# tencent-ailab/PCDMs

Measured on AMD Instinct MI355X. Metric: images/sec (50-step DDIM, 352x512 stage2), higher is better.
Workload: dtype bf16; 1 GPU; stage2 inpaint, 352x512 (canvas 704x512, latent 64x88), batch=4 per GPU, 50 DDIM steps, guidance 2.0 (UNet batch 8), 868.9M-param UNet, 258 context tokens, bf16 MFMA / fp32 accumulate; global_batch=4, parallelism=dp1, hipgraph=True, rccl_world_size=1, attention=bf16

## Files before the change

### include/pcdm.h

```cpp
#ifndef PCDM_H
#define PCDM_H
#include <stdint.h>
#ifdef __cplusplus
extern "C" {
#endif

typedef void* pcdm_stream_t;

#define PCDM_ABI_VERSION 5
int pcdm_version(void);
int pcdm_is_emulator(void);

int64_t pcdm_groupnorm_ws_floats(int B, int C);
int pcdm_groupnorm_cluster_timeouts(const float* ws, unsigned* count_out, pcdm_stream_t s);
int pcdm_groupnorm(const void* x1, int C1, const void* x2, int C2, int B, int HW, int groups, float eps,
                   const float* gamma, const float* beta, int fuse_silu, void* y, float* ws, pcdm_stream_t s);

typedef struct pcdm_gn_splitk_src {
    const float* part;
    int32_t split_k, M, N, Npad;
    const float* bias;
    const float* rowvec;
    int64_t ldrv;
    const int32_t* rowvec_step;
    int64_t rowvec_step_stride;
    const void* residual;
    int64_t ldr;
    void* pre_out;
    int32_t store_pre;
    int32_t rowvec_step_count;
    int32_t* step_error;
} pcdm_gn_splitk_src;
int pcdm_groupnorm_splitk(const pcdm_gn_splitk_src* src, const void* x2, int C2, int B, int HW, int groups, float eps,
                          const float* gamma, const float* beta, int fuse_silu, void* y, float* ws, pcdm_stream_t s);

int pcdm_layernorm(const void* x, void* y, int rows, int C, float eps, const float* gamma, const float* beta,
                   pcdm_stream_t s);

enum { PCDM_EPI_STORE = 0, PCDM_EPI_GEGLU = 1, PCDM_EPI_SPLIT_VT = 2, PCDM_EPI_NCHW_F32 = 3 };
enum { PCDM_ACT_NONE = 0, PCDM_ACT_SILU = 1, PCDM_ACT_GELU = 2 };
typedef struct pcdm_gemm_params {
    uint32_t struct_size;
    const void* a;
    const void* a2;
    int64_t lda, lda2;
    int32_t c1;
    int32_t conv;
    int32_t B, Hi, Wi, Ho, Wo, stride, upsample, cin;
    const void* w;
    int32_t M, N, K, Npad;
    const float* bias;
    const float* rowvec;
    int64_t ldrv;
    int32_t rows_per_batch;
    const void* residual;
    int64_t ldr;
    int32_t res_mod;
    int32_t epilogue;
    int32_t vt_col0;
    void* out;
    int64_t ldo;
    void* out2;
    int64_t ldo2;
    int32_t split_k;
    float* ws;
    int64_t ws_floats;
    int64_t ldw;
    int32_t no_pad_lo;
    int32_t tile;
    int32_t act;
    int32_t zero_rows;
    const float* ln_wsum;
    float ln_eps;
    int32_t defer_reduce;
    const int32_t* rowvec_step;
    int64_t rowvec_step_stride;
    int32_t dup_rows;
    const float* ln_row_stats;
    float* row_stats_out;
    int32_t rowvec_step_count;
    int32_t* step_error;
    const void* a3;
    int64_t lda3;
    uint64_t tap_lut;
    int32_t tap_group_n;
} pcdm_gemm_params;
int pcdm_gemm(const pcdm_gemm_params* p, pcdm_stream_t s);

int pcdm_flash_attn(const void* q, int64_t ldq, const void* k, int64_t ldk, const void* vt, int64_t ldvt,
                    void* o, int64_t ldo, int B, int H, int Lq, int Lk, float scale, pcdm_stream_t s);
#define PCDM_ATTN_DEFAULT_THR 8.0f
int pcdm_flash_attn_thr(const void* q, int64_t ldq, const void* k, int64_t ldk, const void* vt, int64_t ldvt,
                        void* o, int64_t ldo, int B, int H, int Lq, int Lk, float scale, float thr_log2, pcdm_stream_t s);

int pcdm_quantize_fp8(const void* x, void* y, int64_t rows, int cols, int cols_pad, int64_t ldx, int64_t ldy, float scale, pcdm_stream_t s);
int pcdm_flash_attn_fp8(const void* q, int64_t ldq, const void* k8, int64_t ldk, const void* vt8, int64_t ldvt, void* o, int64_t ldo,
                        int B, int H, int Lq, int Lk, float scale, float k_descale, float v_descale, float thr_log2, pcdm_stream_t s);

int pcdm_attn_wide(const void* q, int64_t ldq, const void* k, int64_t ldk, const void* vt, int64_t ldvt, void* o, int64_t ldo,
                   int B, int Lq, int Lk, int d, float scale, pcdm_stream_t s);

int pcdm_timestep_embedding(const int64_t* t_dev, const int32_t* step_dev, float* out, int B, int dim,
                            int flip_sin_to_cos, float shift, pcdm_stream_t s);
int pcdm_small_linear(const float* x, const void* w, const float* bias, const float* add, float* y, int B, int K,
                      int N, int act_in, int act_out, pcdm_stream_t s);
int pcdm_timestep_embedding_rows(const int64_t* t_dev, int n, float* out, int dim, int flip_sin_to_cos, float shift, pcdm_stream_t s);
int pcdm_time_class_combine(const float* emb_t, const float* cls, void* out_bf16, int n, int B, int D, pcdm_stream_t s);

int pcdm_assemble_input(const float* latents, int N, int rep, const float* mask, int mask_b, const float* masked,
                        int masked_b, void* out, int h, int w, int cpad, pcdm_stream_t s);
int pcdm_nchw_f32_to_nhwc_bf16(const float* x, void* y, int B, int C, int Cpad, int HW, pcdm_stream_t s);
int pcdm_nhwc_bf16_to_nchw_f32(const void* x, float* y, int B, int C, int HW, pcdm_stream_t s);
int pcdm_f32_to_bf16(const float* x, void* y, int64_t n, pcdm_stream_t s);

int pcdm_cfg_step(const float* eps, int cfg, float g, const float* x, const float* noise, float* x_prev,
                  float* eps_out, const float* coef, const int32_t* step_dev, int64_t n, pcdm_stream_t s);
int pcdm_unipc_step(const float* eps, int cfg, float g, float* x, float* m1, float* m2, float* last, const float* coef,
                    const int32_t* step_dev, int64_t n, pcdm_stream_t s);
int pcdm_dpmpp_step(const float* eps, int cfg, float g, float* x, float* m1, const float* noise_all, const float* coef,
                    const int32_t* step_dev, int64_t n, pcdm_stream_t s);
int pcdm_unclip_step(const float* pred, int cfg, float g, const float* x, const float* noise, float* x_prev,
                     const float* c8, int64_t n, pcdm_stream_t s);
int pcdm_unclip_step_dev(const float* pred, int cfg, float g, float* x, const float* noise_all, const float* coef,
                         const int32_t* step_dev, int64_t n, pcdm_stream_t s);
int pcdm_rescale_noise_cfg(const float* cfg_eps, const float* text_eps, float* out, int N, int64_t n,
                           float guidance_rescale, pcdm_stream_t s);
int pcdm_softmax_rows(const float* s_in, void* p_out, int rows, int cols, int64_t ld_s, int64_t ld_p, float scale,
                      pcdm_stream_t s);
int pcdm_gaussian_sample(const float* moments, const float* noise, float* out, int B, int zc, int HW, float scale,
                         pcdm_stream_t s);
int pcdm_image_to_uint8(const float* x, void* out, int B, int cstride, int HW, pcdm_stream_t s);
int pcdm_lincomb(float* y, int nin, const float* const* xs, const float* c, int64_t n, pcdm_stream_t s);
int pcdm_advance_step(int32_t* step_dev, pcdm_stream_t s);
int pcdm_pixel_shuffle2(const void* in, void* out, int B, int H, int W, int C, pcdm_stream_t s);

int64_t pcdm_metrics_ws_bytes(int N, int ref_n, int W, int H, float sigma);
int pcdm_ssim(const void* cand, int N, int Hc, int Wc, const int32_t* cand_win, const void* ref, int ref_n, int Hr, int Wr, const int32_t* ref_win,
              int channels, int is_f32, float sigma, float data_range, float* scores, int32_t* argmax, void* ws, int64_t ws_bytes, pcdm_stream_t s);
int pcdm_psnr(const void* cand, int N, int Hc, int Wc, const int32_t* cand_win, const void* ref, int ref_n, int Hr, int Wr, const int32_t* ref_win,
              int channels, int is_f32, float data_range, float* mse, float* psnr, void* ws, int64_t ws_bytes, pcdm_stream_t s);
int pcdm_select_image(const void* cand_u8, int N, int Hc, int Wc, const int32_t* win, int channels, const int32_t* index_dev, void* out, int normalized,
                      pcdm_stream_t s);

typedef struct pcdm_lpips_weights {
    const float* conv_w[5];
    const float* conv_b[5];
    const float* lin[5];
} pcdm_lpips_weights;
int pcdm_pack_lpips_conv(const float* w, const float* bias, int Cout, int Cin, int kh, int kw, float* out_w, float* out_bias, int* K_out, int* cin_out);
int pcdm_conv2d_f32(const float* x, int B, int Hi, int Wi, int Cin, const float* w_packed, const float* bias, int Cout, int kh, int kw, int stride, int pad,
                    int relu, float* out, pcdm_stream_t s);
int pcdm_maxpool3s2_f32(const float* x, int B, int Hi, int Wi, int C, float* out, pcdm_stream_t s);
int64_t pcdm_lpips_ws_bytes(int N, int ref_n, int H, int W);
int pcdm_lpips(const void* img0, int N, int H0, int W0, const int32_t* win0, const void* img1, int ref_n, int H1, int W1, const int32_t* win1, int is_f32,
               int normalize, const pcdm_lpips_weights* wts, float* out, float* layers, int32_t* argmin, void* ws, int64_t ws_bytes, pcdm_stream_t s);

typedef struct pcdm_inception_weights {
    const float* w[94];
    const float* bias[94];
} pcdm_inception_weights;
int pcdm_conv2d_f32_ex(const float* x, int B, int Hi, int Wi, int Cin, const float* w_packed, const float* bias, int Cout, int kh, int kw, int stride,
                       int pad_h, int pad_w, int relu, float* out, int out_pitch, int out_offset, pcdm_stream_t s);
int pcdm_maxpool3s2_f32_ex(const float* x, int B, int Hi, int Wi, int C, float* out, int out_pitch, int out_offset, pcdm_stream_t s);
int pcdm_avgpool3_f32(const float* x, int B, int H, int W, int C, float* out, pcdm_stream_t s);
int pcdm_global_avgpool_f32(const float* x, int B, int P, int C, float* out, pcdm_stream_t s);
int pcdm_inception_input(const void* img, int N, int Hi, int Wi, const int32_t* win, int is_f32, int resize, int normalize, float* out, pcdm_stream_t s);
int64_t pcdm_inception_ws_bytes(int B, int H, int W, int dims);
int pcdm_inception_features(const void* img, int N, int Hi, int Wi, const int32_t* win, int is_f32, int resize, int normalize, int dims,
                            const pcdm_inception_weights* wts, float* out, void* ws, int64_t ws_bytes, pcdm_stream_t s);
int pcdm_fid_accumulate(const float* feat, int B, int D, double* sum, double* gram, pcdm_stream_t s);
int pcdm_fid_finalize(const double* sum, const double* gram, int64_t n, int D, double* mu, double* sigma, pcdm_stream_t s);

int64_t pcdm_resample_ws_bytes(int Hs, int Ws, int Hd, int Wd, int channels, int ky);
int pcdm_resample_u8(const void* src, int Hs, int Ws, int channels, const int32_t* xtab, int kx, const int32_t* ytab, int ky, void* dst, int Hd, int Wd,
                     int64_t dst_pitch, int x0, int y0, void* ws, int64_t ws_bytes, pcdm_stream_t s);
int pcdm_u8_to_nchw(const void* src_u8, int Hs, int Ws, int channels, const int32_t* win, int mode, double scale, const float* mean, const float* std_,
                    float* out, pcdm_stream_t s);

int pcdm_resize_cubic_f32(const void* src, int src_is_f32, int Hs, int Ws, int channels, float* dst, int N, int Hd, int Wd, int index, int nchw,
                          float divisor, pcdm_stream_t s);
int pcdm_absdiff(const void* cand, int N, int Hc, int Wc, const int32_t* cand_win, const void* ref, int ref_n, int Hr, int Wr, const int32_t* ref_win,
                 int channels, int is_f32, float* l1, float* mae, void* ws, int64_t ws_bytes, pcdm_stream_t s);
int64_t pcdm_ssim_box_ws_bytes(int N, int ref_n, int W, int H, int win_size);
int pcdm_ssim_box(const void* cand, int N, int Hc, int Wc, const int32_t* cand_win, const void* ref, int ref_n, int Hr, int Wr, const int32_t* ref_win,
                  int channels, int is_f32, int win_size, float data_range, float* scores, void* ws, int64_t ws_bytes, pcdm_stream_t s);

int pcdm_pose_tables(int32_t* tables, int count);
int64_t pcdm_pose_ws_bytes(int M, int P);
int pcdm_pose_draw(const float* keypoints, const float* scores, int M, int P, int Hd, int Wd, int hands, int faces, const int32_t* tables, void* out,
                   void* ws, int64_t ws_bytes, pcdm_stream_t s);
int pcdm_resize_linear_u8(const void* src, int M, int Hs, int Ws, void* dst, int Hd, int Wd, pcdm_stream_t s);

typedef struct pcdm_unet pcdm_unet;
typedef struct pcdm_unet_config {
    int32_t out_channels;
    int32_t n_levels;
    int32_t block_out_channels[8];
    int32_t heads[8];
    int32_t cross_attn[8];
    int32_t layers_per_block;
    int32_t cross_attention_dim;
    int32_t norm_groups;
    float norm_eps;
    int32_t class_embed;
    int32_t flip_sin_to_cos;
    float freq_shift;
} pcdm_unet_config;
pcdm_unet* pcdm_unet_create(const pcdm_unet_config* cfg);
void pcdm_unet_destroy(pcdm_unet* u);
const char* pcdm_unet_last_error(const pcdm_unet* u);
int pcdm_unet_set_weight(pcdm_unet* u, const char* name, const void* w_bf16, const float* bias, const float* wsum, int N, int K, int Npad, int cin);
int pcdm_unet_set_vector(pcdm_unet* u, const char* name, const float* v, int n);
int pcdm_unet_set_tile(pcdm_unet* u, int ln, int M, int Npad, int K, int conv, int stride, int upsample, int epilogue, int two_source, int residual,
                       int zero_rows, int tile, int split_k);
int pcdm_unet_set_attention_fp8(pcdm_unet* u, int on);
int pcdm_unet_get_tile(const pcdm_unet* u, int ln, int M, int Npad, int K, int conv, int stride, int upsample, int epilogue, int two_source, int residual,
// ... 20 lines not shown
```

### pcdms_amd/_lib.py

```python
from __future__ import annotations

import ctypes as C
import os
from pathlib import Path
from typing import Optional

import torch

_HERE = Path(__file__).resolve().parent
LIB_PATH = Path(os.environ.get("PCDM_LIB") or _HERE / "lib" / "libpcdm.so")

_lib: Optional[C.CDLL] = None
_is_emu = False


class GemmParams(C.Structure):

    _fields_ = [
        ("struct_size", C.c_uint32),
        ("a", C.c_void_p), ("a2", C.c_void_p), ("lda", C.c_int64), ("lda2", C.c_int64),
        ("c1", C.c_int32), ("conv", C.c_int32),
        ("B", C.c_int32), ("Hi", C.c_int32), ("Wi", C.c_int32), ("Ho", C.c_int32), ("Wo", C.c_int32),
        ("stride", C.c_int32), ("upsample", C.c_int32), ("cin", C.c_int32),
        ("w", C.c_void_p),
        ("M", C.c_int32), ("N", C.c_int32), ("K", C.c_int32), ("Npad", C.c_int32),
        ("bias", C.c_void_p), ("rowvec", C.c_void_p), ("ldrv", C.c_int64), ("rows_per_batch", C.c_int32),
        ("residual", C.c_void_p), ("ldr", C.c_int64), ("res_mod", C.c_int32),
        ("epilogue", C.c_int32), ("vt_col0", C.c_int32),
        ("out", C.c_void_p), ("ldo", C.c_int64), ("out2", C.c_void_p), ("ldo2", C.c_int64),
        ("split_k", C.c_int32), ("ws", C.c_void_p), ("ws_floats", C.c_int64),
        ("ldw", C.c_int64), ("no_pad_lo", C.c_int32), ("tile", C.c_int32), ("act", C.c_int32),
        ("zero_rows", C.c_int32),
        ("ln_wsum", C.c_void_p), ("ln_eps", C.c_float), ("defer_reduce", C.c_int32),
        ("rowvec_step", C.c_void_p), ("rowvec_step_stride", C.c_int64), ("dup_rows", C.c_int32),
        ("ln_row_stats", C.c_void_p), ("row_stats_out", C.c_void_p), ("rowvec_step_count", C.c_int32), ("step_error", C.c_void_p),
        ("a3", C.c_void_p), ("lda3", C.c_int64), ("tap_lut", C.c_uint64), ("tap_group_n", C.c_int32),
    ]

    def __init__(self, *args, **kw):
        super().__init__(*args, **kw)
        self.struct_size = C.sizeof(GemmParams)


class GnSplitKSrc(C.Structure):

    _fields_ = [("part", C.c_void_p), ("split_k", C.c_int32), ("M", C.c_int32), ("N", C.c_int32), ("Npad", C.c_int32),
                ("bias", C.c_void_p), ("rowvec", C.c_void_p), ("ldrv", C.c_int64), ("rowvec_step", C.c_void_p), ("rowvec_step_stride", C.c_int64),
                ("residual", C.c_void_p), ("ldr", C.c_int64), ("pre_out", C.c_void_p), ("store_pre", C.c_int32),
                ("rowvec_step_count", C.c_int32), ("step_error", C.c_void_p)]


class UNetConfig(C.Structure):

    _fields_ = [("out_channels", C.c_int32), ("n_levels", C.c_int32), ("block_out_channels", C.c_int32 * 8), ("heads", C.c_int32 * 8),
                ("cross_attn", C.c_int32 * 8), ("layers_per_block", C.c_int32), ("cross_attention_dim", C.c_int32),
                ("norm_groups", C.c_int32), ("norm_eps", C.c_float), ("class_embed", C.c_int32), ("flip_sin_to_cos", C.c_int32),
                ("freq_shift", C.c_float)]


class LpipsWeights(C.Structure):

    _fields_ = [("conv_w", C.c_void_p * 5), ("conv_b", C.c_void_p * 5), ("lin", C.c_void_p * 5)]


class InceptionWeights(C.Structure):

    _fields_ = [("w", C.c_void_p * 94), ("bias", C.c_void_p * 94)]


_P, _I, _L, _F = C.c_void_p, C.c_int, C.c_int64, C.c_float
_W4 = C.POINTER(C.c_int32)
_SIGS = {
    "pcdm_version": ([], C.c_int),
    "pcdm_is_emulator": ([], C.c_int),
    "pcdm_groupnorm_ws_floats": ([_I, _I], _L),
    "pcdm_groupnorm_cluster_timeouts": ([_P, C.POINTER(C.c_uint), _P], C.c_int),
    "pcdm_groupnorm": ([_P, _I, _P, _I, _I, _I, _I, _F, _P, _P, _I, _P, _P, _P], C.c_int),
    "pcdm_groupnorm_splitk": ([C.POINTER(GnSplitKSrc), _P, _I, _I, _I, _I, _F, _P, _P, _I, _P, _P, _P], C.c_int),
    "pcdm_layernorm": ([_P, _P, _I, _I, _F, _P, _P, _P], C.c_int),
    "pcdm_gemm": ([C.POINTER(GemmParams), _P], C.c_int),
    "pcdm_flash_attn": ([_P, _L, _P, _L, _P, _L, _P, _L, _I, _I, _I, _I, _F, _P], C.c_int),
    "pcdm_flash_attn_thr": ([_P, _L, _P, _L, _P, _L, _P, _L, _I, _I, _I, _I, _F, _F, _P], C.c_int),
    "pcdm_quantize_fp8": ([_P, _P, _L, _I, _I, _L, _L, _F, _P], C.c_int),
    "pcdm_flash_attn_fp8": ([_P, _L, _P, _L, _P, _L, _P, _L, _I, _I, _I, _I, _F, _F, _F, _F, _P], C.c_int),
    "pcdm_attn_wide": ([_P, _L, _P, _L, _P, _L, _P, _L, _I, _I, _I, _I, _F, _P], C.c_int),
    "pcdm_timestep_embedding": ([_P, _P, _P, _I, _I, _I, _F, _P], C.c_int),
    "pcdm_timestep_embedding_rows": ([_P, _I, _P, _I, _I, _F, _P], C.c_int),
    "pcdm_time_class_combine": ([_P, _P, _P, _I, _I, _I, _P], C.c_int),
    "pcdm_small_linear": ([_P, _P, _P, _P, _P, _I, _I, _I, _I, _I, _P], C.c_int),
    "pcdm_assemble_input": ([_P, _I, _I, _P, _I, _P, _I, _P, _I, _I, _I, _P], C.c_int),
    "pcdm_nchw_f32_to_nhwc_bf16": ([_P, _P, _I, _I, _I, _I, _P], C.c_int),
    "pcdm_nhwc_bf16_to_nchw_f32": ([_P, _P, _I, _I, _I, _P], C.c_int),
    "pcdm_f32_to_bf16": ([_P, _P, _L, _P], C.c_int),
    "pcdm_cfg_step": ([_P, _I, _F, _P, _P, _P, _P, _P, _P, _L, _P], C.c_int),
    "pcdm_unipc_step": ([_P, _I, _F, _P, _P, _P, _P, _P, _P, _L, _P], C.c_int),
    "pcdm_dpmpp_step": ([_P, _I, _F, _P, _P, _P, _P, _P, _L, _P], C.c_int),
    "pcdm_unclip_step": ([_P, _I, _F, _P, _P, _P, C.POINTER(_F), _L, _P], C.c_int),
    "pcdm_unclip_step_dev": ([_P, _I, _F, _P, _P, _P, _P, _L, _P], C.c_int),
    "pcdm_lincomb": ([_P, _I, C.POINTER(_P), C.POINTER(_F), _L, _P], C.c_int),
    "pcdm_rescale_noise_cfg": ([_P, _P, _P, _I, _L, _F, _P], C.c_int),
    "pcdm_softmax_rows": ([_P, _P, _I, _I, _L, _L, _F, _P], C.c_int),
    "pcdm_gaussian_sample": ([_P, _P, _P, _I, _I, _I, _F, _P], C.c_int),
    "pcdm_image_to_uint8": ([_P, _P, _I, _I, _I, _P], C.c_int),
    "pcdm_advance_step": ([_P, _P], C.c_int),
    "pcdm_pixel_shuffle2": ([_P, _P, _I, _I, _I, _I, _P], C.c_int),
    "pcdm_metrics_ws_bytes": ([_I, _I, _I, _I, _F], _L),
    "pcdm_ssim": ([_P, _I, _I, _I, _W4, _P, _I, _I, _I, _W4, _I, _I, _F, _F, _P, _P, _P, _L, _P], C.c_int),
    "pcdm_psnr": ([_P, _I, _I, _I, _W4, _P, _I, _I, _I, _W4, _I, _I, _F, _P, _P, _P, _L, _P], C.c_int),
    "pcdm_select_image": ([_P, _I, _I, _I, _W4, _I, _P, _P, _I, _P], C.c_int),
    "pcdm_pack_lpips_conv": ([_P, _P, _I, _I, _I, _I, _P, _P, _P, _P], C.c_int),
    "pcdm_conv2d_f32": ([_P, _I, _I, _I, _I, _P, _P, _I, _I, _I, _I, _I, _I, _P, _P], C.c_int),
    "pcdm_maxpool3s2_f32": ([_P, _I, _I, _I, _I, _P, _P], C.c_int),
    "pcdm_lpips_ws_bytes": ([_I, _I, _I, _I], _L),
    "pcdm_lpips": ([_P, _I, _I, _I, _W4, _P, _I, _I, _I, _W4, _I, _I, C.POINTER(LpipsWeights), _P, _P, _P, _P, _L, _P], C.c_int),
    "pcdm_conv2d_f32_ex": ([_P, _I, _I, _I, _I, _P, _P, _I, _I, _I, _I, _I, _I, _I, _P, _I, _I, _P], C.c_int),
    "pcdm_maxpool3s2_f32_ex": ([_P, _I, _I, _I, _I, _P, _I, _I, _P], C.c_int),
    "pcdm_avgpool3_f32": ([_P, _I, _I, _I, _I, _P, _P], C.c_int),
    "pcdm_global_avgpool_f32": ([_P, _I, _I, _I, _P, _P], C.c_int),
    "pcdm_inception_input": ([_P, _I, _I, _I, _W4, _I, _I, _I, _P, _P], C.c_int),
    "pcdm_inception_ws_bytes": ([_I, _I, _I, _I], _L),
    "pcdm_inception_features": ([_P, _I, _I, _I, _W4, _I, _I, _I, _I, C.POINTER(InceptionWeights), _P, _P, _L, _P], C.c_int),
    "pcdm_fid_accumulate": ([_P, _I, _I, _P, _P, _P], C.c_int),
    "pcdm_fid_finalize": ([_P, _P, _L, _I, _P, _P, _P], C.c_int),
    "pcdm_resample_ws_bytes": ([_I, _I, _I, _I, _I, _I], _L),
    "pcdm_resample_u8": ([_P, _I, _I, _I, _P, _I, _P, _I, _P, _I, _I, _L, _I, _I, _P, _L, _P], C.c_int),
    "pcdm_u8_to_nchw": ([_P, _I, _I, _I, _W4, _I, C.c_double, C.POINTER(_F), C.POINTER(_F), _P, _P], C.c_int),
    "pcdm_resize_cubic_f32": ([_P, _I, _I, _I, _I, _P, _I, _I, _I, _I, _I, _F, _P], C.c_int),
    "pcdm_absdiff": ([_P, _I, _I, _I, _W4, _P, _I, _I, _I, _W4, _I, _I, _P, _P, _P, _L, _P], C.c_int),
    "pcdm_ssim_box_ws_bytes": ([_I, _I, _I, _I, _I], _L),
    "pcdm_ssim_box": ([_P, _I, _I, _I, _W4, _P, _I, _I, _I, _W4, _I, _I, _I, _F, _P, _P, _L, _P], C.c_int),
    "pcdm_pose_tables": ([C.POINTER(C.c_int32), _I], C.c_int),
    "pcdm_pose_ws_bytes": ([_I, _I], _L),
    "pcdm_pose_draw": ([_P, _P, _I, _I, _I, _I, _I, _I, _P, _P, _P, _L, _P], C.c_int),
    "pcdm_resize_linear_u8": ([_P, _I, _I, _I, _P, _I, _I, _P], C.c_int),
    "pcdm_unet_create":([C.POINTER(UNetConfig)], _P),
    "pcdm_unet_destroy": ([_P], None),
    "pcdm_unet_last_error": ([_P], C.c_char_p),
    "pcdm_unet_set_weight": ([_P, C.c_char_p, _P, _P, _P, _I, _I, _I, _I], C.c_int),
    "pcdm_unet_set_vector": ([_P, C.c_char_p, _P, _I], C.c_int),
    "pcdm_unet_set_tile": ([_P] + [_I] * 13, C.c_int),
    "pcdm_unet_set_attention_fp8": ([_P, _I], C.c_int),
    "pcdm_unet_get_tile": ([_P] + [_I] * 11 + [C.POINTER(C.c_int), C.POINTER(C.c_int)], C.c_int),
    "pcdm_unet_workspace_bytes": ([_P, _I, _I, _I, _I], _L),
    "pcdm_unet_workspace_init": ([_P, _I, _I, _I, _I, _P, _P], C.c_int),
    "pcdm_unet_prepare_conditioning": ([_P, _I, _I, _I, _I, _P, _P, _P, _I, _I, _P, _P], C.c_int),
    "pcdm_unet_time_table_bytes": ([_P, _I, _I], _L),
    "pcdm_unet_prepare_timesteps": ([_P, _P, _I, _P, _P, _P], C.c_int),
    "pcdm_unet_set_shared_cfg_input": ([_P, _P, _I], C.c_int),
    "pcdm_unet_forward": ([_P, _P, _P, _P, _I, _I, _I, _I, _I, _P, _P, _P], C.c_int),
    "pcdm_unet_step_overflow": ([_P, _P, C.POINTER(C.c_int), _P], C.c_int),
    "pcdm_pack_linear": ([_P, _P, _I, _I, _I, _P, _P], C.c_int),
    "pcdm_pack_conv3x3": ([_P, _P, _I, _I, _I, _P, _P, _P, _P], C.c_int),
    "pcdm_pack_geglu": ([_P, _P, _I, _I, _P, _P], C.c_int),
}
EXPORTS = tuple(_SIGS)


def _bind(lib: C.CDLL) -> C.CDLL:
    for name, (args, res) in _SIGS.items():
        fn = getattr(lib, name)
        fn.argtypes = args
        fn.restype = res
    return lib


def use_library(lib: C.CDLL) -> None:
    global _lib, _is_emu
    _lib = _bind(lib)
    _is_emu = bool(lib.pcdm_is_emulator())


def load(path: Optional[Path] = None) -> C.CDLL:
    global _lib, _is_emu
    p = Path(path) if path else LIB_PATH
    if not p.exists():
        raise RuntimeError(
            f"{p} not found: the HIP kernel library is not built.  Run `python -m pcdms_amd.build` "
            "(needs hipcc); pcdms_amd has no fallback implementation.")
    _lib = _bind(C.CDLL(str(p)))
    _is_emu = bool(_lib.pcdm_is_emulator())
    return _lib


def lib() -> C.CDLL:
    return _lib if _lib is not None else load()


# ... 4 lines not shown
```

### pcdms_amd/csrc/gemm.hip

```cpp
#include "gemm_kernel.inc"

namespace {
template <bool CONV>
int dispatch_tile(int tile, const GemmArgs& a, hipStream_t st) {
    switch (tile) {
#ifndef PCDM_DEV_NEW_TILES_ONLY
        case 1: return launch_gemm<256, 128, 4, 2, 3, CONV>(a, st);
        case 2: return launch_gemm<64, 64, 2, 2, 2, CONV>(a, st);
        case 3: return launch_gemm<256, 64, 4, 2, 2, CONV>(a, st);
        case 4: return launch_gemm<128, 128, 2, 2, 2, CONV>(a, st);
        case 5: return launch_gemm<128, 64, 2, 2, 2, CONV>(a, st);
        case 6: return launch_gemm<256, 64, 4, 2, 3, CONV>(a, st);
        case 7: return launch_gemm<128, 128, 2, 2, 3, CONV>(a, st);
        case 8: return launch_gemm<64, 64, 2, 2, 4, CONV>(a, st);
        case 9: return launch_gemm<256, 128, 4, 2, 2, CONV>(a, st);
        case 10: return launch_gemm<128, 64, 2, 2, 3, CONV>(a, st);
        case 11: return launch_gemm<256, 128, 4, 2, 3, CONV, true>(a, st);
        case 12: return launch_gemm<256, 64, 4, 2, 3, CONV, true>(a, st);
        case 13: return launch_gemm<256, 64, 4, 1, 2, CONV>(a, st);
        case 14: return launch_gemm<256, 64, 4, 1, 3, CONV>(a, st);
        case 15: return launch_gemm<128, 64, 2, 1, 2, CONV>(a, st);
        case 16: return launch_gemm<512, 64, 8, 1, 2, CONV>(a, st);
        case 17: return launch_gemm<256, 256, 2, 4, 2, CONV>(a, st);
        case 18: return launch_gemm<128, 128, 4, 2, 2, CONV>(a, st);
#endif
        case 21: return launch_gemm<192, 320, 2, 4, 2, CONV, false, 16>(a, st);
        case 22: return launch_gemm<176, 320, 2, 4, 2, CONV, false, 16>(a, st);
        case 23: return launch_gemm<176, 256, 2, 4, 2, CONV, false, 16>(a, st);
        case 26: return launch_gemm<192, 256, 2, 4, 2, CONV, false, 16>(a, st);
#ifdef PCDM_DEV_KB32
        case 27: return launch_gemm<192, 320, 2, 4, 4, CONV, false, 16, 32>(a, st);
        case 28: return launch_gemm<256, 256, 2, 4, 4, CONV, false, 16, 32>(a, st);
#endif
        default: return -1;
    }
}
}

extern "C" int pcdm_gemm(const pcdm_gemm_params* p, pcdm_stream_t s) {
    if (!p || p->struct_size != (uint32_t)sizeof(pcdm_gemm_params)) return -1;
    if (!p->a || !p->w || !p->out) return -1;
    if (p->M <= 0 || p->N <= 0 || p->K <= 0 || p->K % BK || p->Npad % 64 || p->Npad < p->N || p->N % 4) return -1;
    if (p->rows_per_batch <= 0) return -1;
    if (((uintptr_t)p->bias & 15) || (p->rowvec && (((uintptr_t)p->rowvec & 15) || (p->ldrv > 0 && p->ldrv % 4) || (p->rowvec_step && p->rowvec_step_stride % 4))))
        return -1;
    const int64_t lim = 0x7fffffffLL;
    if ((int64_t)p->Npad * (p->ldw > 0 ? p->ldw : p->K) * 2 >= lim) return -2;
    if (p->conv ? ((int64_t)p->B * p->Hi * p->Wi * p->cin * 2 + ((int64_t)p->Wi + 1) * p->cin * 2 >= lim ||
                   (p->a2 && (int64_t)p->M * p->lda2 * 2 >= lim) || (p->a3 && (int64_t)p->M * p->lda3 * 2 >= lim))
                : ((int64_t)p->M * p->lda * 2 >= lim || (p->a2 && (int64_t)p->M * p->lda2 * 2 >= lim))) return -2;
    const int64_t out_esz = p->epilogue == PCDM_EPI_NCHW_F32 ? 4 : 2;
    if ((int64_t)p->M * (p->ldo > 0 ? p->ldo : p->N) * out_esz >= lim || (p->residual && (int64_t)p->M * (p->ldr > 0 ? p->ldr : p->N) * 2 >= lim))
        return -2;
    GemmArgs a;
    a.a = (const u16*)p->a;
    a.a2 = (const u16*)p->a2;
    a.lda = p->lda;
    a.lda2 = p->lda2;
    a.c1 = p->a2 ? p->c1 : p->K;
    a.a3 = (const u16*)p->a3;
    a.lda3 = p->lda3;
    a.xinv = 0;
    a.tap_lut = 0;
    a.tap_group_n = 0;
    a.B = p->B; a.Hi = p->Hi; a.Wi = p->Wi; a.Ho = p->Ho; a.Wo = p->Wo;
    a.stride = p->stride; a.upsample = p->upsample; a.cin = p->cin;
    a.pad = p->no_pad_lo ? 0 : 1;
    a.w = (const u16*)p->w;
    a.ldw = p->ldw > 0 ? p->ldw : p->K;
    if (a.ldw < p->K || a.ldw % 8) return -1;
    a.M = p->M; a.N = p->N; a.K = p->K; a.Npad = p->Npad;
    a.bias = p->bias;
    a.rowvec = p->rowvec;
    a.rowvec_step = p->rowvec ? p->rowvec_step : nullptr;
    a.rowvec_step_stride = p->rowvec_step_stride;
    a.rowvec_step_count = a.rowvec_step ? p->rowvec_step_count : 0;
    a.step_error = a.rowvec_step ? p->step_error : nullptr;
    if (a.rowvec_step_count < 0 || ((uintptr_t)a.step_error & 3)) return -1;
    a.ldrv = p->ldrv > 0 ? (int)p->ldrv : p->N;
    a.rows_per_batch = p->rows_per_batch;
    a.residual = (const u16*)p->residual;
    a.ldr = p->ldr;
    a.res_mod = p->res_mod > 0 ? p->res_mod : p->M;
    a.epilogue = p->epilogue;
    a.vt_col0 = p->vt_col0;
    a.out = p->out;
    a.ldo = p->ldo;
    a.out2 = (u16*)p->out2;
    a.ldo2 = p->ldo2;
    a.tiles_m = a.tiles_n = 0;
    a.debug = p->tile >> 8;
    a.act = p->act;
    a.dup_rows = p->dup_rows;
    if (a.dup_rows) {
        if (a.dup_rows < 0 || !p->conv || p->epilogue != PCDM_EPI_STORE || p->act || p->split_k > 1 || (p->N & 7) || (p->ldo & 7)) return -1;
        if (p->residual && ((p->ldr & 7) || (p->res_mod > 0 && p->res_mod < p->M))) return -1;
        if (p->rowvec && (p->rows_per_batch < 32 || a.dup_rows % p->rows_per_batch)) return -1;
        if (((int64_t)p->M + a.dup_rows) * (p->ldo > 0 ? p->ldo : p->N) * 2 >= lim) return -2;
    }
    a.zero_rows = p->zero_rows;
    if (a.zero_rows < 0 || a.zero_rows > p->M || (a.zero_rows && p->conv)) return -1;
    if (a.act < 0 || a.act > PCDM_ACT_GELU || (a.act == PCDM_ACT_GELU && p->epilogue == PCDM_EPI_GEGLU)) return -1;
    a.ln_wsum = p->ln_wsum;
    a.ln_eps = p->ln_eps;
    a.split_k = p->split_k > 1 ? p->split_k : 1;
    a.defer_reduce = (p->defer_reduce && a.split_k > 1) ? 1 : 0;
    if (a.defer_reduce && (p->act || p->res_mod > 0 && p->res_mod < p->M)) return -1;
    a.ws = p->ws;
    if (a.split_k > 1) {
        if (p->epilogue != PCDM_EPI_STORE || !p->ws || a.split_k > p->K / BK || a.split_k > 64) return -1;
        if (p->ws_floats < (int64_t)a.split_k * p->M * p->Npad) return -1;
    }
    if (p->conv && p->tap_group_n > 0) {
        const int ntaps = p->cin > 0 ? p->K / p->cin : 0;
        if (p->cin <= 0 || p->cin % BK || p->K != ntaps * p->cin || ntaps < 1 || ntaps > 4 || p->stride != 1 || p->upsample || p->no_pad_lo || p->dup_rows ||
            p->a2 || p->a3 || p->Hi != p->Ho || p->Wi != p->Wo || p->N % p->tap_group_n || p->N / p->tap_group_n > 4 || p->tap_group_n % 64)
            return -1;
        uint64_t lut = 0;
        for (int g = 0; g < p->N / p->tap_group_n; ++g) {
            uint64_t grp = (p->tap_lut >> (16 * g)) & ((1ull << (4 * ntaps)) - 1);
            for (int t = 0; t < ntaps; ++t)
                if (((grp >> (4 * t)) & 15) > 8) return -1;
            if (grp == 0) {
                if (ntaps == 4) return -1;
                grp = 1ull << (4 * ntaps);
            }
            lut |= grp << (16 * g);
        }
        if (p->M != p->B * p->Ho * p->Wo) return -1;
        a.tap_lut = lut;
        a.tap_group_n = p->tap_group_n;
    } else if (p->conv) {
        const int cx = p->K - 9 * p->cin;
        if (p->cin <= 0 || p->cin % BK || cx < 0 || (p->stride != 1 && p->stride != 2)) return -1;
        if (cx == 0 ? (p->a2 || p->a3)
                    : (!p->a2 || p->stride != 1 || p->upsample || p->no_pad_lo || p->dup_rows || p->Hi != p->Ho || p->Wi != p->Wo || cx % BK ||
                       p->c1 <= 0 || p->c1 % BK || p->c1 > cx || (p->c1 < cx) != (p->a3 != nullptr) || p->lda2 < p->c1 || (p->lda2 & 7) ||
                       (p->a3 && (p->lda3 < cx - p->c1 || (p->lda3 & 7))) || (((uintptr_t)p->a2 | (uintptr_t)p->a3) & 15)))
            return -1;
        a.xinv = (uint32_t)(((1ull << 31) + (uint64_t)(p->cin / 64) - 1) / (uint64_t)(p->cin / 64));
        if (p->upsample && (p->stride != 1 || p->no_pad_lo || p->Ho < p->Hi || p->Wo < p->Wi)) return -1;
        if (p->M != p->B * p->Ho * p->Wo) return -1;
    } else {
        if (p->a3 || (p->a2 && (p->c1 % BK || p->c1 <= 0 || p->c1 >= p->K))) return -1;
    }
    if (p->epilogue == PCDM_EPI_GEGLU && (!p->bias || p->Npad % 128 || p->N * 2 > p->Npad)) return -1;
    if (p->epilogue == PCDM_EPI_SPLIT_VT && (!p->out2 || p->vt_col0 % 4)) return -1;
    hipStream_t st = (hipStream_t)s;
    int tile = p->tile & 0xff;
    if (tile >= pcdm_gemm_detail::kRowGemmTile0) {
        if ((a.debug & 4) && p->ws_floats < (int64_t)((p->M + 95) / 96) * 8 * 8 * 2) return -1;
        if (p->row_stats_out) return -1;
        return p->conv ? -1 : pcdm_gemm_detail::launch_rowgemm(tile, a, st);
    }
    a.ln_row_stats = p->ln_row_stats;
    a.row_stats_out = p->row_stats_out;
    if (a.ln_wsum) {
        if (p->conv || p->a2 || a.split_k > 1 || p->rowvec || p->residual || p->act || a.zero_rows || a.dup_rows || (p->N & 7) || (p->ldo & 7) ||
            ((uintptr_t)a.ln_wsum & 15) || p->row_stats_out)
            return -1;
        if (p->epilogue != PCDM_EPI_STORE && p->epilogue != PCDM_EPI_GEGLU && p->epilogue != PCDM_EPI_SPLIT_VT) return -1;
        if (p->epilogue == PCDM_EPI_SPLIT_VT && (p->vt_col0 % 64 || p->rows_per_batch % 32 || (p->ldo2 & 7) || p->M % 32)) return -1;
        if (p->epilogue == PCDM_EPI_GEGLU && (tile == 2 || tile == 8)) return -1;
        if (((tile == 4 || tile == 7 || tile == 18) && p->Npad % 128) || ((tile == 17 || tile == 26 || tile == 23) && p->Npad % 256)) return -1;
        if (a.ln_row_stats && ((p->K & 63) || p->K > 1280 || ((uintptr_t)a.ln_row_stats & 15))) return -1;
        return pcdm_gemm_detail::launch_gemm_ext(a.ln_row_stats ? 2 : 1, tile, a, st);
    }
    if (a.ln_row_stats) return -1;
    if (a.row_stats_out) {
        if (p->conv || a.split_k > 1 || p->act || a.dup_rows || p->epilogue != PCDM_EPI_STORE || (p->N & 31) || (p->ldo & 7) || ((uintptr_t)a.row_stats_out & 7) ||
            (p->residual && ((p->ldr & 7) || (p->res_mod > 0 && p->res_mod < p->M))) || (p->rowvec && p->rows_per_batch < 32))
            return -1;
        if ((tile == 4 || tile == 7 || tile == 18) && p->Npad % 128) return -1;
        return pcdm_gemm_detail::launch_gemm_ext(3, tile, a, st);
    }
    const bool n128 = p->Npad % 128 == 0 && (a.tap_group_n == 0 || a.tap_group_n % 128 == 0);
    const bool needs128 = tile == 1 || tile == 4 || tile == 7 || tile == 9 || tile == 11 || tile == 18;
    if (p->epilogue == PCDM_EPI_GEGLU && tile != 0 && !needs128 && tile < 13) return -1;
    if (tile == 0) {
        const int64_t t256 = (int64_t)((p->M + 255) / 256) * (p->Npad / 128);
        const int64_t t128 = (int64_t)((p->M + 127) / 128) * (p->Npad / 128);
        if (n128 && t256 >= 200) tile = 1;
        else if (n128 && (t128 >= 160 || p->epilogue == PCDM_EPI_GEGLU)) tile = 4;
        else if (!n128 && (int64_t)((p->M + 127) / 128) * (p->Npad / 64) >= 256) tile = 5;
        else tile = 2;
    } else if ((needs128 && !n128) || (tile == 17 && p->Npad % 256)) {
        return -1;
    }
    return p->conv ? dispatch_tile<true>(tile, a, st) : dispatch_tile<false>(tile, a, st);
}
```

### pcdms_amd/csrc/gemm_args.h

```cpp
#pragma once
#include "pcdm_device.h"
#include "../../include/pcdm.h"

namespace pcdm_gemm_detail {
struct GemmArgs {
    const u16* a;
    const u16* a2;
    int64_t lda, lda2;
    int c1;
    const u16* a3;
    int64_t lda3;
    uint64_t tap_lut;
    int tap_group_n;
    uint32_t xinv;
    int B, Hi, Wi, Ho, Wo, stride, upsample, cin;
    int pad;
    const u16* w;
    int64_t ldw;
    int M, N, K, Npad;
    const float* bias;
    const float* rowvec;
    const int32_t* rowvec_step;
    int64_t rowvec_step_stride;
    int rowvec_step_count;
    int32_t* step_error;
    int ldrv;
    int rows_per_batch;
    const u16* residual;
    int64_t ldr;
    int res_mod;
    int epilogue;
    int vt_col0;
    void* out;
    int64_t ldo;
    u16* out2;
    int64_t ldo2;
    int tiles_m, tiles_n;
    int split_k;
    float* ws;
    int act;
    int zero_rows;
    const float* ln_wsum;
    float ln_eps;
    const float* ln_row_stats;
    float* row_stats_out;
    int dup_rows;
    int defer_reduce;
    int debug;
};
}

namespace pcdm_gemm_detail {
__device__ __forceinline__ int bounded_step(const int32_t* step, int count, int32_t* err) {
    int st = *step;
    if (count > 0 && (st < 0 || st >= count)) {
        if (err) *err = 1;
        st = st < 0 ? 0 : count - 1;
    }
    return st;
}
__device__ __forceinline__ const float* rowvec_base(const GemmArgs& p) {
    return (p.rowvec && p.rowvec_step) ? p.rowvec + (int64_t)bounded_step(p.rowvec_step, p.rowvec_step_count, p.step_error) * p.rowvec_step_stride : p.rowvec;
}
__device__ __forceinline__ float apply_act(float v, int act) {
    return act == PCDM_ACT_SILU ? silu_f(v) : act == PCDM_ACT_GELU ? gelu_erf_f(v) : v;
}
__device__ __forceinline__ float gate_act(float g, int act) { return act == PCDM_ACT_SILU ? silu_f(g) : gelu_erf_f(g); }

constexpr int kRowGemmTile0 = 31;
int launch_rowgemm(int tile, const GemmArgs& a, hipStream_t st);
int launch_gemm_ext(int ext, int tile, const GemmArgs& a, hipStream_t st);
}
```

### pcdms_amd/csrc/gemm_kernel.inc

```
#include "gemm_args.h"

#include <type_traits>



namespace {
using pcdm_gemm_detail::GemmArgs;
using pcdm_gemm_detail::apply_act;
using pcdm_gemm_detail::gate_act;
constexpr int BK = 64;

__device__ __attribute__((aligned(32))) const unsigned int g_zero32[8] = {0, 0, 0, 0, 0, 0, 0, 0};

template <int WCOLS>
struct PassGeom {
    static constexpr int LPR = WCOLS / 8;
    static constexpr int RPI = 64 / LPR;
    static constexpr int NIT = (32 + RPI - 1) / RPI;
    static constexpr bool TAIL = NIT * RPI > 32;
};

template <int WCOLS>
__device__ __forceinline__ void lean_res_load(const GemmArgs& p, int lane, int mrow0, int ncol0, BufRsrc rs_r, u32x4 (&rv)[4]) {
    typedef PassGeom<WCOLS> G;
    constexpr uint32_t kOOB = 0x80000000u;
    const int rl = lane / G::LPR, c8 = (lane - rl * G::LPR) * 8;
    const int n = ncol0 + c8;
    const bool lane_ok = rl < G::RPI && n < p.N;
    const uint32_t vr0 = lane_ok ? (uint32_t)(((mrow0 + rl) * (int)p.ldr + n) * 2) : kOOB;
    const uint32_t sr = (uint32_t)(G::RPI * (int)p.ldr * 2);
#pragma unroll
    for (int it = 0; it < G::NIT; ++it) rv[it] = buf_load16_once(rs_r, (G::TAIL && it * G::RPI + rl >= 32) ? kOOB : vr0 + it * sr);
}

template <int WCOLS, int EPW, int RV, bool STATS = false>
__device__ __forceinline__ void lean_pass(const GemmArgs& p, float* ep, int lane, int mrow0, int ncol0, f32x4 b0, f32x4 b1,
                                          BufRsrc rs_o, BufRsrc rs_v, const u32x4 (&rv)[4], const float* rvec_w, int rv_pitch,
                                          int rv_col0, int rv_split_row) {
    static_assert(!STATS || WCOLS == 32 || WCOLS == 64, "row statistics: passes of 32 or 64 columns");
    typedef PassGeom<WCOLS> G;
    constexpr int LPR = G::LPR, RPI = G::RPI, NIT = G::NIT;
    constexpr bool TAIL = G::TAIL;
    constexpr uint32_t kOOB = 0x80000000u;
    const int rl = lane / LPR, c8 = (lane - rl * LPR) * 8;
    const int n = ncol0 + c8;
    const bool lane_ok = rl < RPI && n < p.N;
    const uint32_t vo0 = lane_ok ? (uint32_t)(((mrow0 + rl) * (int)p.ldo + n) * 2) : kOOB;
    const uint32_t so = (uint32_t)(RPI * (int)p.ldo * 2);
    f32x4 t0[2], t1[2];
    if constexpr (RV == 1) {
#pragma unroll
        for (int h = 0; h < 2; ++h) {
            t0[h] = *(const f32x4*)(rvec_w + h * rv_pitch + rv_col0 + c8);
            t1[h] = *(const f32x4*)(rvec_w + h * rv_pitch + rv_col0 + c8 + 4);
        }
    }
#pragma unroll
    for (int it = 0; it < NIT; ++it) {
        const int r = it * RPI + rl;
        const int rr = (TAIL && r >= 32) ? 0 : r;
        const f32x4 v0 = *(const f32x4*)(ep + rr * EPW + c8), v1 = *(const f32x4*)(ep + rr * EPW + c8 + 4);
        f32x4 a0 = v0 + b0, a1 = v1 + b1;
        if constexpr (RV == 1) {
            const bool hi = mrow0 + r >= rv_split_row;
            a0 += hi ? t0[1] : t0[0];
            a1 += hi ? t1[1] : t1[0];
        }
        if constexpr (RV == 2) {
            const int mb = mrow0 + it * RPI;
            const int b_lo = mb / p.rows_per_batch;
            const int bidx = b_lo + ((mb + rl) >= (b_lo + 1) * p.rows_per_batch ? 1 : 0);
            const uint32_t vv = lane_ok ? (uint32_t)((bidx * p.ldrv + n) * 4) : kOOB;
            a0 += __builtin_bit_cast(f32x4, buf_load16(rs_v, vv));
            a1 += __builtin_bit_cast(f32x4, buf_load16(rs_v, vv + 16));
        }
#pragma unroll
        for (int e = 0; e < 4; ++e) {
            a0[e] += __builtin_bit_cast(float, rv[it][e >> 1] << (e & 1 ? 0 : 16) & 0xffff0000u);
            a1[e] += __builtin_bit_cast(float, rv[it][2 + (e >> 1)] << (e & 1 ? 0 : 16) & 0xffff0000u);
        }
        u32x4 o;
        o[0] = pack2bf(a0[0], a0[1]);
        o[1] = pack2bf(a0[2], a0[3]);
        o[2] = pack2bf(a1[0], a1[1]);
        o[3] = pack2bf(a1[2], a1[3]);
        buf_store16(rs_o, (TAIL && r >= 32) ? kOOB : vo0 + it * so, o);
        if constexpr (STATS) {
            float v[8];
#pragma unroll
            for (int e = 0; e < 4; ++e) {
                v[2 * e] = __builtin_bit_cast(float, o[e] << 16);
                v[2 * e + 1] = __builtin_bit_cast(float, o[e] & 0xffff0000u);
            }
            float sv = ((v[0] + v[1]) + (v[2] + v[3])) + ((v[4] + v[5]) + (v[6] + v[7]));
            sv += __shfl_xor(sv, 1, 64);
            sv += __shfl_xor(sv, 2, 64);
            const float mu = sv * (1.0f / 32.0f);
            float qv = 0.f;
#pragma unroll
            for (int e = 0; e < 8; ++e) {
                const float d = v[e] - mu;
                qv += d * d;
            }
            qv += __shfl_xor(qv, 1, 64);
            qv += __shfl_xor(qv, 2, 64);
            const int m = mrow0 + r;
            if (((lane & 3) == 0) && lane_ok && m < p.M) {
                const f32x2 sq = {sv, qv};
                *((f32x2*)p.row_stats_out + (int64_t)m * (p.N >> 5) + (n >> 5)) = sq;
            }
        }
    }
}

template <int WCOLS, int EPW>
__device__ __forceinline__ void vt_pass(const GemmArgs& p, const float* ep, int lane, int mrow0, int ncol0, BufRsrc rs_vt,
                                        const float* bias_c ) {
    constexpr uint32_t kOOB = 0x80000000u;
    const int b = mrow0 / p.rows_per_batch, tok0 = mrow0 - b * p.rows_per_batch;
    const int cl = lane & 15, tg = lane >> 4;
    const int cv = p.N - p.vt_col0;
#pragma unroll
    for (int ii = 0; ii < WCOLS / 16; ++ii) {
        const int c = ii * 16 + cl, n = ncol0 + c;
        const bool ok = n < p.N;
        const float bias = bias_c[c];
        float v[8];
#pragma unroll
        for (int i = 0; i < 8; ++i) v[i] = ep[(8 * tg + i) * EPW + c] + bias;
        u32x4 o;
#pragma unroll
        for (int i = 0; i < 4; ++i) o[i] = pack2bf(v[2 * i], v[2 * i + 1]);
        const uint32_t vo = ok ? (uint32_t)((((int64_t)b * cv + (n - p.vt_col0)) * p.ldo2 + tok0 + 8 * tg) * 2) : kOOB;
        buf_store16(rs_vt, vo, o);
    }
}

template <int N>
__device__ __forceinline__ void wait_vm_then_barrier() {
#ifdef PCDM_EMU
    __syncthreads();
#else
    asm volatile("s_waitcnt vmcnt(%0)\n\ts_barrier" ::"n"(N) : "memory");
#endif
}

template <int N>
__device__ __forceinline__ void wait_vm_lds_then_barrier() {
#ifdef PCDM_EMU
    __syncthreads();
#else
    __builtin_amdgcn_sched_barrier(0);
    __builtin_amdgcn_s_waitcnt((N & 15) | (7 << 4) | (0 << 8) | ((N >> 4) << 14));
    __builtin_amdgcn_s_barrier();
    __builtin_amdgcn_sched_barrier(0);
#endif
}

__device__ __forceinline__ void wait_lds() {
#ifndef PCDM_EMU
    __builtin_amdgcn_s_waitcnt(15 | (7 << 4) | (0 << 8) | (3 << 14));
#endif
}

template <int N>
__device__ __forceinline__ void wait_vm() {
#ifndef PCDM_EMU
    asm volatile("s_waitcnt vmcnt(%0)" ::"n"(N) : "memory");
#endif
}
__device__ __forceinline__ void wait_lds_then_barrier() {
#ifdef PCDM_EMU
    __syncthreads();
#else
    asm volatile("s_waitcnt lgkmcnt(0)\n\ts_barrier" ::: "memory");
#endif
}

template <int BM, int BN, int WGM, int WGN, int STAGES, bool CONV, bool STAG = false, int F = 32, int KB = 64, int EXT = 0>
__global__ __launch_bounds__(WGM* WGN * 64) void gemm_kernel(const GemmArgs p) {
    constexpr bool LNF = EXT == 1 || EXT == 2, LNK = EXT == 1, LNP = EXT == 2, STATS = EXT == 3;
    static_assert(EXT == 0 || (!CONV && !STAG && KB == 64), "extended instances: linear tiles on the rotated schedule");
    static_assert(!STATS || F == 32, "row-statistics producer: 32- / 64-column epilogue passes");
    static_assert(!LNK || BM % (8 * WGM * WGN) == 0, "in-loop row statistics: 8 rows per wave instruction");
    constexpr int BK = KB;
    constexpr int NW = WGM * WGN;
    static_assert(BM % F == 0, "tile shape");
    constexpr int FMT = BM / F;
    constexpr int FM = (FMT + WGM - 1) / WGM;
    constexpr int FM_LAST = FMT - (WGM - 1) * FM;
    constexpr bool UNEVEN = FM_LAST != FM;
    constexpr int WM = FM * F, WN = BN / WGN, FN = WN / F;
    static_assert(FM_LAST >= 1 && (!UNEVEN || (F == 16 && !STAG && KB == 64 && (EXT == 0 || EXT == 2))), "uneven tiles: 16x16x32 fragments, rotated schedule, plain / folded-LayerNorm (partials) instances");
    constexpr int KS = 512 / F;
    constexpr int NKS = BK / KS;
    constexpr int CPK = KS / 8;
    constexpr int NQ = F == 32 ? 4 : 1;
    constexpr int LF = F == 32 ? 5 : 4;
    static_assert((F == 32 || F == 16) && (!STAG || F == 32), "fragment shape");
    static_assert(KB == 64 || (KB == 32 && F == 16 && STAGES == 4 && !STAG), "K-tile depth");
    typedef typename std::conditional<F == 32, f32x16, f32x4>::type acc_t;
    constexpr bool ROLES = KB == 32;
    constexpr int LPR = BK / 8;
    constexpr int RPI = 64 / LPR;
    constexpr int PW = ROLES ? (BM + BN) / (RPI * NW) : 0;
    constexpr int NWA = ROLES ? BM / (RPI * PW) : NW;
    constexpr int BMS = ROLES ? BM : (BM + 8 * NW - 1) / (8 * NW) * (8 * NW);
    constexpr int AI = ROLES ? PW : BMS / 8 / NW, BI = ROLES ? PW : BN / 8 / NW;
    constexpr int PWT = ROLES ? PW : AI + BI;
    constexpr int D = STAGES - 1;
    static_assert(ROLES || ((BM == BMS || UNEVEN) && BN % (8 * NW) == 0), "tile shape");
    static_assert(!ROLES || ((BM + BN) % (RPI * NW) == 0 && BM % (RPI * PW) == 0 && BN % (RPI * PW) == 0), "tile shape (roles)");
    static_assert(WM % 32 == 0 && WN % F == 0, "tile shape");
    PCDM_DYN_SMEM(smem);
    u16* As = (u16*)smem;
    u16* Bs = As + STAGES * BMS * BK;

    const int t = threadIdx.x, lane = t & 63;
    const int wave = __builtin_amdgcn_readfirstlane(t >> 6);
    const int wm = wave / WGN, wn = wave - wm * WGN;
#ifndef PCDM_EMU
    unsigned long long stamp[6] = {0, 0, 0, 0, 0, 0};
    const unsigned long long wall0 = (p.debug & 4) ? wall_clock64() : 0ull;
#define PCDM_STAMP(i) do { if (p.debug & 4) stamp[i] = __builtin_readcyclecounter(); } while (0)
#else
#define PCDM_STAMP(i) ((void)0)
#endif
    PCDM_STAMP(0);

    const int nwg = gridDim.x, bid = blockIdx.x;
    const int q8 = nwg >> 3, r8 = nwg & 7, xcd = bid & 7;
    const int wg = (xcd < r8 ? xcd * (q8 + 1) : r8 * (q8 + 1) + (xcd - r8) * q8) + (bid >> 3);
    const int ntiles = p.tiles_m * p.tiles_n;
    const int ksplit = wg / ntiles, tile_id = wg - ksplit * ntiles;
    const int tile_m = tile_id / p.tiles_n, tile_n = tile_id - tile_m * p.tiles_n;
    const int m0 = tile_m * BM, n0 = tile_n * BN;

    const int srow = lane / LPR, spos = lane % LPR;
    auto swz = [](int r) { return KB == 64 ? (r >> 1) & 7 : (0 - (r >> 2)) & 3; };
    const bool doA = !ROLES || wave < NWA, doB = !ROLES || wave >= NWA;
    const int wa = ROLES ? (wave < NWA ? wave : 0) : wave, wb = ROLES ? (wave >= NWA ? wave - NWA : 0) : wave;
    constexpr uint32_t kOOB = 0x80000000u;
    uint32_t a_off[AI], a_off2[AI];
    int a_mask[AI];
    int a_b[AI], a_y[AI], a_x[AI];
#pragma unroll
    for (int j = 0; j < AI; ++j) {
        const int rl = (wa * AI + j) * RPI + srow;
        int m = m0 + rl;
        const uint32_t ck = (uint32_t)(spos ^ swz(rl)) * 16u;
        const bool mvalid = m < p.M;
        if (!mvalid) m = p.M - 1;
        const bool ghost = BMS > BM && rl >= BM;
        a_off2[j] = 0; a_mask[j] = 0; a_b[j] = a_y[j] = a_x[j] = 0;
        if (ghost) {
            a_off[j] = a_off2[j] = kOOB;
        } else if (CONV) {
            const int hw = p.Ho * p.Wo;
            const int b = m / hw, rem = m - b * hw;
            const int y = rem / p.Wo, x = rem - y * p.Wo;
            a_b[j] = b; a_y[j] = y; a_x[j] = x;
            a_off[j] = (uint32_t)((((int64_t)b * p.Hi + y * p.stride) * p.Wi + x * p.stride) * p.cin * 2) + ck;
            const int Hv_ = p.upsample ? p.Ho : p.Hi, Wv_ = p.upsample ? p.Wo : p.Wi;
#pragma unroll
            for (int tp = 0; tp < 9; ++tp) {
                const int iy = y * p.stride + tp / 3 - p.pad, ix = x * p.stride + tp % 3 - p.pad;
                if (iy >= 0 && iy < Hv_ && ix >= 0 && ix < Wv_) a_mask[j] |= 1 << tp;
            }
        } else {
            a_off[j] = m < p.zero_rows ? kOOB : (uint32_t)((int64_t)m * p.lda * 2) + ck;
            a_off2[j] = m < p.zero_rows ? kOOB : (uint32_t)((int64_t)m * p.lda2 * 2) + ck;
        }
    }
    uint32_t b_off[BI];
#pragma unroll
    for (int j = 0; j < BI; ++j) {
// ... 323 lines not shown
                    mfma_block(B1());
                    PCDM_SCHED_BARRIER();
                }
            }
            const int left = nkt - 2 - kt;
            wait_landed(left < 0 ? 0 : (left < STAGES - 2 ? left : STAGES - 2));
            if (kt + STAGES < nkt && !(p.debug & 1)) issue_tile(kt + STAGES, cur);
            const int nx = cur + 1 == STAGES ? 0 : cur + 1;
            if (kt + 1 < nkt) load_frags(nx, 0, B0());
            PCDM_SCHED_BARRIER();
            mfma_block(B1());
            PCDM_SCHED_BARRIER();
            cur = nx;
        }
        };
        if constexpr (UNEVEN) {
            if (wm == WGM - 1) kloop(std::integral_constant<int, FM_LAST>());
            else kloop(std::integral_constant<int, FM>());
        } else {
            kloop(std::integral_constant<int, FM>());
        }
    }

    PCDM_STAMP(3);
    const int half = lane >> LF;
    const int prow = lane & (F - 1);
    constexpr int QS = F == 32 ? 8 : 0;
    const int mlim = UNEVEN ? (m0 + BM < p.M ? m0 + BM : p.M) : p.M;
    if (p.split_k > 1) {
#pragma unroll
        for (int j = 0; j < FM; ++j) {
            const int m = m0 + wm * WM + j * F + prow;
            if (m >= mlim) continue;
            float* wr = p.ws + ((int64_t)ksplit * p.M + m) * p.Npad + n0 + wn * WN + 4 * half;
#pragma unroll
            for (int i = 0; i < FN; ++i)
#pragma unroll
                for (int rg = 0; rg < NQ; ++rg) {
                    f32x4 v = {acc[i][j][4 * rg], acc[i][j][4 * rg + 1], acc[i][j][4 * rg + 2], acc[i][j][4 * rg + 3]};
                    *(f32x4*)(wr + i * F + QS * rg) = v;
                }
        }
        return;
    }
    constexpr bool GLU_OK = WN == 64;
    const bool geglu = p.epilogue == PCDM_EPI_GEGLU;
    const bool qk_tile = p.epilogue == PCDM_EPI_SPLIT_VT && n0 + wn * WN + WN <= p.vt_col0;
    const bool v_tile = p.epilogue == PCDM_EPI_SPLIT_VT && n0 + wn * WN >= p.vt_col0 && p.rows_per_batch % 32 == 0 && (p.ldo2 & 7) == 0 &&
                        p.act == 0 && !p.residual && !p.rowvec && p.M % 32 == 0;
    const bool lean = ((p.epilogue == PCDM_EPI_STORE && p.act == 0) || (geglu && GLU_OK) || qk_tile || v_tile) && (p.N & 7) == 0 &&
                      (p.ldo & 7) == 0 && (!p.residual || ((p.ldr & 7) == 0 && p.res_mod >= p.M)) && (!p.rowvec || p.rows_per_batch >= 32);
    __syncthreads();
    if constexpr (LNK) {
        const float inv_k = 1.0f / (float)p.K;
#pragma unroll
        for (int i = 0; i < LN_NR; ++i) {
            float sv = ln_s[i], qv = ln_q[i];
#pragma unroll
            for (int m = 1; m < 8; m <<= 1) {
                sv += __shfl_xor(sv, m, 64);
                qv += __shfl_xor(qv, m, 64);
            }
            const float ds = sv * inv_k;
            float var = qv * inv_k - ds * ds;
            var = var > 0.f ? var : 0.f;
            if ((lane & 7) == 0) {
                const int r = wave * LN_SROWS + i * 8 + (lane >> 3);
                lnstat[2 * r] = ln_p[i] + ds;
                lnstat[2 * r + 1] = 1.0f / sqrtf(var + p.ln_eps);
            }
        }
        __syncthreads();
    }
    if (lean) {
        constexpr int RB = 32 / F;
        constexpr int CGM = 64 / F;
        constexpr int CG = FN < CGM ? FN : CGM;
        constexpr int EPW = CG * F + 4;
        const bool has_res = p.residual != nullptr && !geglu, has_rv = p.rowvec != nullptr && !geglu;
        const int ncols_out = qk_tile ? p.vt_col0 : p.N;
        auto epilogue_rep = [&](auto rep_tag) {
        constexpr int REP = decltype(rep_tag)::value;
        const int64_t sh = REP ? (int64_t)p.dup_rows : 0;
        const BufRsrc rs_o = make_buf_rsrc((const char*)p.out + sh * p.ldo * 2, (uint32_t)((((int64_t)mlim - 1) * p.ldo + ncols_out) * 2));
        const BufRsrc rs_r = make_buf_rsrc(has_res ? (const void*)(p.residual + sh * p.ldr) : (const void*)p.out,
                                           has_res ? (uint32_t)((((int64_t)p.M - 1) * p.ldr + p.N) * 2) : 0u);
        const float* rowvec0 = pcdm_gemm_detail::rowvec_base(p);
        const float* rowvec_rep = (has_rv && REP) ? rowvec0 + (sh / p.rows_per_batch) * p.ldrv : rowvec0;
        const BufRsrc rs_v = make_buf_rsrc(has_rv ? (const void*)rowvec_rep : (const void*)p.out,
                                           has_rv ? (uint32_t)((((int64_t)(p.M - 1) / p.rows_per_batch) * p.ldrv + p.N) * 4) : 0u);
        const BufRsrc rs_vt = make_buf_rsrc(v_tile ? (const void*)p.out2 : (const void*)p.out,
                                            v_tile ? (uint32_t)((int64_t)(p.M / p.rows_per_batch) * (p.N - p.vt_col0) * p.ldo2 * 2) : 0u);
        float* ep = (float*)smem + wave * (32 * EPW);
        constexpr int WNP = (WN + 3) / 4 * 4;
        float* bias_w = (float*)smem + NW * (32 * EPW) + wave * (3 * WNP);
        float* rvec_w = bias_w + WNP;
        const int wrow0 = m0 + wm * WM, wcol0 = n0 + wn * WN;
        const int rv_blo = wrow0 / p.rows_per_batch;
        const bool rv_lds = has_rv && (wrow0 + WM - 1) / p.rows_per_batch <= rv_blo + 1;
        const int rv_split_row = (rv_blo + 1) * p.rows_per_batch;
        {
            if (REP) PCDM_WAVE_SYNC();
            if (lane * 4 < WN) {
                const f32x4 z4 = {0.f, 0.f, 0.f, 0.f};
                if (!REP) *(f32x4*)(bias_w + lane * 4) = p.bias ? *(const f32x4*)(p.bias + wcol0 + lane * 4) : z4;
                if constexpr (LNF) *(f32x4*)(rvec_w + lane * 4) = *(const f32x4*)(p.ln_wsum + wcol0 + lane * 4);
                if (rv_lds) {
                    const int c = wcol0 + lane * 4;
                    const int nb = (p.M - 1) / p.rows_per_batch;
#pragma unroll
                    for (int h = 0; h < 2; ++h) {
                        const int b = rv_blo + h < nb ? rv_blo + h : nb;
                        f32x4 v = z4;
#pragma unroll
                        for (int e = 0; e < 4; ++e)
                            if (c + e < p.N) v[e] = rowvec_rep[(int64_t)b * p.ldrv + c + e];
                        *(f32x4*)(rvec_w + h * WNP + lane * 4) = v;
                    }
                }
            }
            PCDM_WAVE_SYNC();
        }
        auto ln_quad = [&](f32x4 a, int col, int row) -> f32x4 {
            if constexpr (LNF) {
                const f32x4 w4 = *(const f32x4*)(rvec_w + col);
                const float mean_r = lnstat[2 * (wm * WM + row)], rstd_r = lnstat[2 * (wm * WM + row) + 1];
#pragma unroll
                for (int e = 0; e < 4; ++e) a[e] = rstd_r * (a[e] - mean_r * w4[e]);
            }
            return a;
        };
        constexpr int NCG = (FN + CG - 1) / CG, NJB = WM / 32;
        auto run_passes = [&](auto res_tag) {
        constexpr bool RES = decltype(res_tag)::value;
        u32x4 rv[RES ? NCG * NJB : 1][4];
        auto pass_cols = [&](int q) { const int i0 = (q / NJB) * CG; return geglu ? 32 : ((FN - i0) < CG ? (FN - i0) : CG) * F; };
        auto pass_ncol0 = [&](int q) { return geglu ? (n0 + wn * WN) / 2 : n0 + wn * WN + (q / NJB) * CG * F; };
        auto issue_res = [&](int q) {
            if constexpr (!RES) {
#pragma unroll
                for (int it = 0; it < 4; ++it) rv[0][it] = u32x4{0, 0, 0, 0};
                return;
            }
            const int mrow0 = m0 + wm * WM + (q % NJB) * 32, wc = pass_cols(q), nc = pass_ncol0(q);
            if (wc == 64) lean_res_load<64>(p, lane, mrow0, nc, rs_r, rv[q]);
            else if (wc == 32) lean_res_load<32>(p, lane, mrow0, nc, rs_r, rv[q]);
            else if (wc == 16) lean_res_load<16>(p, lane, mrow0, nc, rs_r, rv[q]);
            else lean_res_load<48>(p, lane, mrow0, nc, rs_r, rv[q]);
        };
        if constexpr (EARLY_RES && RES) {
            static_assert(E_NPASS == NCG * NJB, "pass geometry");
            if (early_res) {
#pragma unroll
                for (int q = 0; q < NCG * NJB; ++q)
#pragma unroll
                    for (int it = 0; it < 4; ++it) rv[q][it] = rv_early[q][it];
            } else {
#pragma unroll
                for (int q = 0; q < NCG * NJB; ++q) issue_res(q);
            }
        } else {
#pragma unroll
            for (int q = 0; q < (RES ? NCG * NJB : 1); ++q) issue_res(q);
        }
        const bool swiglu = p.act == PCDM_ACT_SILU;
        f32x4 b0 = {0.f, 0.f, 0.f, 0.f}, b1 = b0;
#pragma unroll
        for (int q = 0; q < NCG * NJB; ++q) {
            const int i0 = (q / NJB) * CG, jb = q % NJB;
            const int ng = (FN - i0) < CG ? (FN - i0) : CG;
            const int ncol0 = pass_ncol0(q), wc = pass_cols(q);
            if (jb == 0 && !geglu && !v_tile) {
                const int c8_ = (lane % (wc / 8)) * 8;
                const float* bp = bias_w + (ncol0 - wcol0) + c8_;
                b0 = *(const f32x4*)bp;
                b1 = *(const f32x4*)(bp + 4);
            }
            if (geglu) {
                if constexpr (GLU_OK) {
#pragma unroll
                    for (int jj = 0; jj < RB; ++jj)
#pragma unroll
                        for (int i = 0; i < FN / 2; ++i)
#pragma unroll
                            for (int rg = 0; rg < NQ; ++rg) {
                                const int nl = i * F + QS * rg + 4 * half;
                                const f32x4 bh = *(const f32x4*)(bias_w + nl);
                                const f32x4 bg = *(const f32x4*)(bias_w + nl + 32);
                                const acc_t& ah = acc[i][jb * RB + jj];
                                const acc_t& ag = acc[i + FN / 2][jb * RB + jj];
                                f32x4 hq = {ah[4 * rg], ah[4 * rg + 1], ah[4 * rg + 2], ah[4 * rg + 3]};
                                f32x4 gq = {ag[4 * rg], ag[4 * rg + 1], ag[4 * rg + 2], ag[4 * rg + 3]};
                                if constexpr (LNF) {
                                    hq = ln_quad(hq, nl, jb * 32 + jj * F + prow);
                                    gq = ln_quad(gq, nl + 32, jb * 32 + jj * F + prow);
                                }
                                f32x4 v;
                                if (swiglu) {
#pragma unroll
                                    for (int e = 0; e < 4; ++e) v[e] = (hq[e] + bh[e]) * silu_f(gq[e] + bg[e]);
                                } else {
                                    v = geglu_quad(hq + bh, gq + bg);
                                }
                                *(f32x4*)(ep + (jj * F + prow) * EPW + nl) = v;
                            }
                }
            } else {
#pragma unroll
                for (int jj = 0; jj < RB; ++jj)
#pragma unroll
                    for (int i = 0; i < CG; ++i) {
                        if (i0 + i >= FN) break;
#pragma unroll
                        for (int rg = 0; rg < NQ; ++rg) {
                            const acc_t& a_ = acc[i0 + i < FN ? i0 + i : 0][jb * RB + jj];
                            f32x4 v = {a_[4 * rg], a_[4 * rg + 1], a_[4 * rg + 2], a_[4 * rg + 3]};
                            if constexpr (LNF) v = ln_quad(v, (i0 + i) * F + QS * rg + 4 * half, jb * 32 + jj * F + prow);
                            *(f32x4*)(ep + (jj * F + prow) * EPW + i * F + QS * rg + 4 * half) = v;
                        }
                    }
            }
            PCDM_WAVE_SYNC();
            const int mrow0 = m0 + wm * WM + jb * 32;
            if (v_tile) {
                if (mrow0 < p.M) {
                    const float* bc = bias_w + (ncol0 - wcol0);
                    if (ng * F == 64) vt_pass<64, EPW>(p, ep, lane, mrow0, ncol0, rs_vt, bc);
                    else if (ng * F == 32) vt_pass<32, EPW>(p, ep, lane, mrow0, ncol0, rs_vt, bc);
                    else if (ng * F == 16) vt_pass<16, EPW>(p, ep, lane, mrow0, ncol0, rs_vt, bc);
                    else vt_pass<48, EPW>(p, ep, lane, mrow0, ncol0, rs_vt, bc);
                }
            } else {
                const int rc0 = ncol0 - wcol0;
#define PCDM_LEAN(W, RVK) lean_pass<W, EPW, RVK, STATS && (W == 32 || W == 64)>(p, ep, lane, mrow0, ncol0, b0, b1, rs_o, rs_v, rv[RES ? q : 0], rvec_w, WNP, rc0, rv_split_row)
#define PCDM_LEAN_W(RVK)                 \
    do {                                 \
        if (wc == 64) PCDM_LEAN(64, RVK);      \
        else if (wc == 32) PCDM_LEAN(32, RVK); \
        else if (wc == 16) PCDM_LEAN(16, RVK); \
        else PCDM_LEAN(48, RVK);               \
    } while (0)
                if (!has_rv) PCDM_LEAN_W(0);
                else if (rv_lds) PCDM_LEAN_W(1);
                else PCDM_LEAN_W(2);
#undef PCDM_LEAN_W
#undef PCDM_LEAN
            }
            PCDM_WAVE_SYNC();
        }
        };
        if (has_res) run_passes(std::true_type());
        else run_passes(std::false_type());
        };
        epilogue_rep(std::integral_constant<int, 0>());
        if constexpr (CONV) {
            if (p.dup_rows > 0) epilogue_rep(std::integral_constant<int, 1>());
        }
#ifndef PCDM_EMU
        if ((p.debug & 4) && p.ws) {
            PCDM_STAMP(4);
            asm volatile("s_waitcnt vmcnt(0)" ::: "memory");
            PCDM_STAMP(5);
            if (lane == 0) {
                unsigned long long* o = (unsigned long long*)p.ws + ((int64_t)blockIdx.x * NW + wave) * 8;
                for (int i = 0; i < 6; ++i) o[i] = stamp[i];
                o[6] = wg;
                o[7] = wall_clock64() - wall0;
            }
        }
#endif
        return;
    }
    const float* rowvec_g = pcdm_gemm_detail::rowvec_base(p);
#pragma unroll
    for (int j = 0; j < FM; ++j) {
        const int m = m0 + wm * WM + j * F + prow;
        if (m >= mlim) continue;
        const int bidx = m / p.rows_per_batch;
        const int tok = m - bidx * p.rows_per_batch;
        const int64_t rrow = p.residual ? (int64_t)(m % p.res_mod) * p.ldr : 0;
        if (p.epilogue == PCDM_EPI_GEGLU) {
            if constexpr (GLU_OK) {
#pragma unroll
                for (int i = 0; i < FN / 2; ++i)
#pragma unroll
                    for (int rg = 0; rg < NQ; ++rg) {
                        const int nl = i * F + QS * rg + 4 * half;
                        const int nh = n0 + wn * WN + nl;
                        const int ng = nh + 32;
                        const int no = (n0 + wn * WN) / 2 + nl;
                        if (no >= p.N) continue;
                        const f32x4 bh = *(const f32x4*)(p.bias + nh), bg = *(const f32x4*)(p.bias + ng);
                        u16x4 o;
#pragma unroll
                        for (int e = 0; e < 4; ++e) {
                            const float hval = acc[i][j][4 * rg + e] + bh[e];
                            const float gval = acc[i + FN / 2][j][4 * rg + e] + bg[e];
                            o[e] = f2bf(hval * gate_act(gval, p.act));
                        }
                        *(u16x4*)((u16*)p.out + (int64_t)m * p.ldo + no) = o;
                    }
            }
            continue;
        }
#pragma unroll
        for (int i = 0; i < FN; ++i) {
#pragma unroll
            for (int rg = 0; rg < NQ; ++rg) {
                const int n = n0 + wn * WN + i * F + QS * rg + 4 * half;
                if (n >= p.N) continue;
                const f32x4 bv = *(const f32x4*)(p.bias ? p.bias + n : (const float*)g_zero32);
                const f32x4 tv = *(const f32x4*)(rowvec_g ? rowvec_g + (int64_t)bidx * p.ldrv + n : (const float*)g_zero32);
                const u16x4 rv = *(const u16x4*)(p.residual ? p.residual + rrow + n : (const u16*)g_zero32);
                float v[4];
#pragma unroll
                for (int e = 0; e < 4; ++e) v[e] = acc[i][j][4 * rg + e] + bv[e] + tv[e];
                if (p.act) {
#pragma unroll
                    for (int e = 0; e < 4; ++e) v[e] = apply_act(v[e], p.act);
                }
#pragma unroll
                for (int e = 0; e < 4; ++e) v[e] += bf2f(rv[e]);
                if (p.epilogue == PCDM_EPI_NCHW_F32) {
                    float* o = (float*)p.out;
#pragma unroll
                    for (int e = 0; e < 4; ++e)
                        if (n + e < p.N) o[((int64_t)bidx * p.N + n + e) * p.rows_per_batch + tok] = v[e];
                } else if (p.epilogue == PCDM_EPI_SPLIT_VT && n >= p.vt_col0) {
                    const int cv = p.N - p.vt_col0;
#pragma unroll
                    for (int e = 0; e < 4; ++e)
                        p.out2[((int64_t)bidx * cv + (n + e - p.vt_col0)) * p.ldo2 + tok] = f2bf(v[e]);
                } else {
                    u16x4 o;
#pragma unroll
                    for (int e = 0; e < 4; ++e) o[e] = f2bf(v[e]);
                    *(u16x4*)((u16*)p.out + (int64_t)m * p.ldo + n) = o;
                }
            }
        }
    }
}

__global__ __launch_bounds__(256) void splitk_reduce_kernel(const GemmArgs p) {
    const int nq = p.N / 4;
    const int64_t i = (int64_t)blockIdx.x * blockDim.x + threadIdx.x;
    if (i >= (int64_t)p.M * nq) return;
    const int m = (int)(i / nq), n = (int)(i - (int64_t)m * nq) * 4;
    const f32x4 bv = *(const f32x4*)(p.bias ? p.bias + n : (const float*)g_zero32);
    const float* rowvec_g = pcdm_gemm_detail::rowvec_base(p);
    const f32x4 tv = *(const f32x4*)(rowvec_g ? rowvec_g + (int64_t)(m / p.rows_per_batch) * p.ldrv + n : (const float*)g_zero32);
    const u16x4 rv = *(const u16x4*)(p.residual ? p.residual + (int64_t)(m % p.res_mod) * p.ldr + n : (const u16*)g_zero32);
    f32x4 v = {0.f, 0.f, 0.f, 0.f};
    const float* wp = p.ws + (int64_t)m * p.Npad + n;
    const int64_t slab = (int64_t)p.M * p.Npad;
    int s = 0;
    for (; s + 4 <= p.split_k; s += 4) {
        const f32x4 t0 = *(const f32x4*)(wp + (s + 0) * slab), t1 = *(const f32x4*)(wp + (s + 1) * slab);
        const f32x4 t2 = *(const f32x4*)(wp + (s + 2) * slab), t3 = *(const f32x4*)(wp + (s + 3) * slab);
        v += t0;
        v += t1;
        v += t2;
        v += t3;
    }
    for (; s < p.split_k; ++s) v += *(const f32x4*)(wp + s * slab);
    v += bv;
    v += tv;
    if (p.act) {
#pragma unroll
        for (int e = 0; e < 4; ++e) v[e] = apply_act(v[e], p.act);
    }
#pragma unroll
    for (int e = 0; e < 4; ++e) v[e] += bf2f(rv[e]);
    u16x4 o;
#pragma unroll
    for (int e = 0; e < 4; ++e) o[e] = f2bf(v[e]);
    *(u16x4*)((u16*)p.out + (int64_t)m * p.ldo + n) = o;
}

template <int BM, int BN, int WGM, int WGN, int STAGES, bool CONV, bool STAG = false, int F = 32, int KB = 64, int EXT = 0>
int launch_gemm(const GemmArgs& a, hipStream_t st) {
    constexpr bool LNF = EXT == 1 || EXT == 2;
    constexpr int BK = KB;
    constexpr int BMS_ = KB == 32 ? BM : (BM + 8 * WGM * WGN - 1) / (8 * WGM * WGN) * (8 * WGM * WGN);
    constexpr bool UNEVEN_ = (BM / F) % WGM != 0;
    constexpr int smem_ops = STAGES * (BMS_ + BN) * BK * (int)sizeof(u16);
    constexpr int FN_ = BN / WGN / F, CGM_ = 64 / F;
    constexpr int WNP_ = (BN / WGN + 3) / 4 * 4;
    constexpr int smem_epi = WGM * WGN * (32 * ((FN_ < CGM_ ? FN_ : CGM_) * F + 4) + 3 * WNP_) * (int)sizeof(float);
    constexpr int smem0 = smem_ops > smem_epi ? smem_ops : smem_epi;
    constexpr int smem = smem0 + (LNF ? 2 * BMS_ * (int)sizeof(float) : 0);
    static bool attr_done = false;
    if (!attr_done) {
        (void)hipFuncSetAttribute((const void*)gemm_kernel<BM, BN, WGM, WGN, STAGES, CONV, STAG, F, KB, EXT>,
                                  hipFuncAttributeMaxDynamicSharedMemorySize, smem);
        attr_done = true;
    }
    if (a.Npad % BN) return -1;
    if (a.tap_group_n > 0 && (!CONV || a.tap_group_n % BN)) return -1;
    if (a.epilogue == PCDM_EPI_GEGLU && BN / WGN != 64) return -1;
    if (UNEVEN_ && a.epilogue == PCDM_EPI_SPLIT_VT) return -1;
    GemmArgs g = a;
    g.tiles_m = (a.M + BM - 1) / BM;
    g.tiles_n = a.Npad / BN;
    PCDM_LAUNCH(PCDM_KERNEL_NAME(gemm_kernel<BM, BN, WGM, WGN, STAGES, CONV, STAG, F, KB, EXT>), dim3(g.tiles_m * g.tiles_n * g.split_k),
                dim3(WGM * WGN * 64), smem, st, g);
    PCDM_CHECK_LAUNCH();
    if (g.split_k > 1 && !g.defer_reduce) {
        const int64_t n = (int64_t)g.M * (g.N / 4);
        PCDM_LAUNCH(splitk_reduce_kernel, dim3((unsigned)((n + 255) / 256)), dim3(256), 0, st, g);
        PCDM_CHECK_LAUNCH();
    }
    return 0;
}

}
```

### pcdms_amd/csrc/misc.hip

```cpp
#include "pcdm_device.h"
#include "../../include/pcdm.h"
#include "image_common.h"

namespace {
__global__ void timestep_embedding_kernel(const int64_t* __restrict__ t_dev, const int32_t* __restrict__ step_dev,
                                          float* __restrict__ out, int B, int dim, int flip, float shift) {
    const int i = blockIdx.x * blockDim.x + threadIdx.x;
    if (i >= B * dim) return;
    const int j = i % dim, half = dim / 2;
    const float tv = (float)t_dev[step_dev ? *step_dev : 0];
    const int kk = j < half ? j : j - half;
    const float f = expf(-9.210340371976184f * (float)kk / ((float)half - shift));
    const float a = tv * f;
    const bool is_cos = flip ? (j < half) : (j >= half);
    out[i] = is_cos ? cosf(a) : sinf(a);
}

__global__ void timestep_embedding_rows_kernel(const int64_t* __restrict__ t_dev, float* __restrict__ out, int n, int dim, int flip, float shift) {
    const int i = blockIdx.x * blockDim.x + threadIdx.x;
    if (i >= n * dim) return;
    const int j = i % dim, half = dim / 2;
    const float tv = (float)t_dev[i / dim];
    const int kk = j < half ? j : j - half;
    const float f = expf(-9.210340371976184f * (float)kk / ((float)half - shift));
// ... 247 lines not shown
    float* o = out + (int64_t)blockIdx.x * n;
    for (int64_t i = threadIdx.x; i < n; i += blockDim.x) o[i] = a[i] * f;
}

__global__ __launch_bounds__(256) void softmax_rows_kernel(const float* __restrict__ s, u16* __restrict__ p, int cols,
                                                           int64_t ld_s, int64_t ld_p, float scale_log2e) {
    __shared__ float red[4];
    const float* sr = s + (int64_t)blockIdx.x * ld_s;
    u16* pr = p + (int64_t)blockIdx.x * ld_p;
    const int t = threadIdx.x;
    float v[32];
    float mx = -1e30f;
#pragma unroll
    for (int i = 0; i < 32; ++i) {
        const int c = t + 256 * i;
        v[i] = c < cols ? sr[c] * scale_log2e : -1e30f;
        mx = fmaxf(mx, v[i]);
    }
    mx = wave_max(mx);
    if ((t & 63) == 0) red[t >> 6] = mx;
    __syncthreads();
    mx = fmaxf(fmaxf(red[0], red[1]), fmaxf(red[2], red[3]));
    __syncthreads();
    float sum = 0.f;
#pragma unroll
    for (int i = 0; i < 32; ++i) {
        v[i] = fast_exp2(v[i] - mx);
        sum += (t + 256 * i < cols) ? v[i] : 0.f;
    }
    sum = wave_sum(sum);
    if ((t & 63) == 0) red[t >> 6] = sum;
    __syncthreads();
    const float inv = 1.0f / (red[0] + red[1] + red[2] + red[3]);
#pragma unroll
    for (int i = 0; i < 32; ++i) {
        const int c = t + 256 * i;
        if (c < cols) pr[c] = f2bf(v[i] * inv);
    }
}

__global__ void gaussian_sample_kernel(const float* __restrict__ mom, const float* __restrict__ noise,
                                       float* __restrict__ out, int zc, int HW, float scale, int64_t total) {
    const int64_t i = (int64_t)blockIdx.x * blockDim.x + threadIdx.x;
    if (i >= total) return;
    const int64_t chw = (int64_t)zc * HW;
    const int64_t b = i / chw, r = i - b * chw;
    const float mean = mom[b * 2 * chw + r];
    float lv = mom[b * 2 * chw + chw + r];
    lv = fminf(fmaxf(lv, -30.0f), 20.0f);
    const float z = noise ? noise[i] : 0.f;
    out[i] = (mean + __expf(0.5f * lv) * z) * scale;
}

__global__ void image_to_uint8_kernel(const float* __restrict__ x, uint8_t* __restrict__ out, int cstride, int HW,
                                      int64_t total) {
    const int64_t i = (int64_t)blockIdx.x * blockDim.x + threadIdx.x;
    if (i >= total) return;
    const int64_t b = i / HW, pix = i - b * HW;
#pragma unroll
    for (int c = 0; c < 3; ++c) {
        float v = x[(b * cstride + c) * HW + pix] * 0.5f + 0.5f;
        v = fminf(fmaxf(v, 0.f), 1.f);
        out[i * 3 + c] = (uint8_t)rintf(v * 255.0f);
    }
}

__global__ void pixel_shuffle2_kernel(const u16* __restrict__ in, u16* __restrict__ out, int H, int W, int C8, int64_t total) {
    const int64_t i = (int64_t)blockIdx.x * blockDim.x + threadIdx.x;
    if (i >= total) return;
    const int c8 = (int)(i % C8);
    const int64_t px = i / C8;
    const int W2 = 2 * W;
    const int X = (int)(px % W2);
    const int64_t bY = px / W2;
    const int Y = (int)(bY % (2 * H));
    const int64_t b = bY / (2 * H);
    const int64_t src = (((b * H + (Y >> 1)) * W + (X >> 1)) * 4 + ((Y & 1) * 2 + (X & 1))) * C8 + c8;
    ((u32x4*)out)[i] = ((const u32x4*)in)[src];
}

__global__ void advance_step_kernel(int32_t* step) {
    if (threadIdx.x == 0 && blockIdx.x == 0) *step += 1;
}
}

extern "C" int pcdm_version(void) { return PCDM_ABI_VERSION; }
extern "C" int pcdm_is_emulator(void) {
#ifdef PCDM_EMU
    return 1;
#else
    return 0;
#endif
}

extern "C" int pcdm_timestep_embedding(const int64_t* t_dev, const int32_t* step_dev, float* out, int B, int dim,
                                       int flip_sin_to_cos, float shift, pcdm_stream_t s) {
    if (!t_dev || !out || B <= 0 || dim <= 0 || dim % 2) return -1;
    PCDM_LAUNCH(timestep_embedding_kernel, grid1d((int64_t)B * dim, 256), dim3(256), 0, (hipStream_t)s, t_dev, step_dev,
                out, B, dim, flip_sin_to_cos, shift);
    PCDM_CHECK_LAUNCH();
    return 0;
}

extern "C" int pcdm_timestep_embedding_rows(const int64_t* t_dev, int n, float* out, int dim, int flip_sin_to_cos, float shift, pcdm_stream_t s) {
    if (!t_dev || !out || n <= 0 || dim <= 0 || dim % 2) return -1;
    PCDM_LAUNCH(timestep_embedding_rows_kernel, grid1d((int64_t)n * dim, 256), dim3(256), 0, (hipStream_t)s, t_dev, out, n, dim, flip_sin_to_cos, shift);
    PCDM_CHECK_LAUNCH();
    return 0;
}

extern "C" int pcdm_time_class_combine(const float* emb_t, const float* cls, void* out_bf16, int n, int B, int D, pcdm_stream_t s) {
    if (!emb_t || !out_bf16 || n <= 0 || B <= 0 || D <= 0) return -1;
    PCDM_LAUNCH(time_class_combine_kernel, grid1d((int64_t)n * B * D, 256), dim3(256), 0, (hipStream_t)s, emb_t, cls, (u16*)out_bf16, n, B, D);
    PCDM_CHECK_LAUNCH();
    return 0;
}

extern "C" int pcdm_small_linear(const float* x, const void* w, const float* bias, const float* add, float* y, int B,
                                 int K, int N, int act_in, int act_out, pcdm_stream_t s) {
    if (!x || !w || !y || B <= 0 || B > 32 || K <= 0 || K % 8 || N <= 0) return -1;
    PCDM_LAUNCH(small_linear_kernel, dim3((N + 3) / 4), dim3(256), 0, (hipStream_t)s, x, (const u16*)w, bias, add, y,
                B, K, N, act_in, act_out);
    PCDM_CHECK_LAUNCH();
    return 0;
}

extern "C" int pcdm_assemble_input(const float* latents, int N, int rep, const float* mask, int mask_b,
                                   const float* masked, int masked_b, void* out, int h, int w, int cpad,
                                   pcdm_stream_t s) {
    if (!latents || !masked || !out || N <= 0 || rep <= 0 || cpad % 8 || cpad < 16) return -1;
    const int64_t total = (int64_t)N * rep * h * w * (cpad / 8);
    PCDM_LAUNCH(assemble_input_kernel, grid1d(total, 256), dim3(256), 0, (hipStream_t)s, latents, N, rep, mask, mask_b,
                masked, masked_b, (u16*)out, h * w, cpad);
    PCDM_CHECK_LAUNCH();
    return 0;
}

extern "C" int pcdm_nchw_f32_to_nhwc_bf16(const float* x, void* y, int B, int C, int Cpad, int HW, pcdm_stream_t s) {
    if (!x || !y || B <= 0 || C <= 0 || HW <= 0 || Cpad % 8 || Cpad < C) return -1;
    const int64_t total = (int64_t)B * HW * (Cpad / 8);
    PCDM_LAUNCH(nchw_to_nhwc_kernel, grid1d(total, 256), dim3(256), 0, (hipStream_t)s, x, (u16*)y, C, Cpad, HW, total);
    PCDM_CHECK_LAUNCH();
    return 0;
}

extern "C" int pcdm_nhwc_bf16_to_nchw_f32(const void* x, float* y, int B, int C, int HW, pcdm_stream_t s) {
    if (!x || !y || B <= 0 || C <= 0 || HW <= 0) return -1;
    const int64_t total = (int64_t)B * HW * C;
    PCDM_LAUNCH(nhwc_to_nchw_kernel, grid1d(total, 256), dim3(256), 0, (hipStream_t)s, (const u16*)x, y, C, HW, total);
    PCDM_CHECK_LAUNCH();
    return 0;
}

extern "C" int pcdm_f32_to_bf16(const float* x, void* y, int64_t n, pcdm_stream_t s) {
    if (!x || !y || n <= 0) return -1;
    PCDM_LAUNCH(f32_to_bf16_kernel, grid1d(n, 256), dim3(256), 0, (hipStream_t)s, x, (u16*)y, n);
    PCDM_CHECK_LAUNCH();
    return 0;
}

extern "C" int pcdm_cfg_step(const float* eps, int cfg, float g, const float* x, const float* noise, float* x_prev,
                             float* eps_out, const float* coef, const int32_t* step_dev, int64_t n, pcdm_stream_t s) {
    if (!eps || n <= 0 || (x_prev && (!x || !coef))) return -1;
    PCDM_LAUNCH(cfg_step_kernel, grid1d(n, 256), dim3(256), 0, (hipStream_t)s, eps, cfg, g, x, noise, x_prev, eps_out,
                coef, step_dev, n);
    PCDM_CHECK_LAUNCH();
    return 0;
}

extern "C" int pcdm_unipc_step(const float* eps, int cfg, float g, float* x, float* m1, float* m2, float* last, const float* coef,
                               const int32_t* step_dev, int64_t n, pcdm_stream_t s) {
    if (!eps || !x || !m1 || !m2 || !last || !coef || n <= 0) return -1;
    PCDM_LAUNCH(unipc_step_kernel, grid1d(n, 256), dim3(256), 0, (hipStream_t)s, eps, cfg, g, x, m1, m2, last, coef, step_dev, n);
    PCDM_CHECK_LAUNCH();
    return 0;
}

extern "C" int pcdm_dpmpp_step(const float* eps, int cfg, float g, float* x, float* m1, const float* noise_all, const float* coef,
                               const int32_t* step_dev, int64_t n, pcdm_stream_t s) {
    if (!eps || !x || !m1 || !coef || n <= 0) return -1;
    PCDM_LAUNCH(dpmpp_step_kernel, grid1d(n, 256), dim3(256), 0, (hipStream_t)s, eps, cfg, g, x, m1, noise_all, coef, step_dev, n);
    PCDM_CHECK_LAUNCH();
    return 0;
}

extern "C" int pcdm_unclip_step(const float* pred, int cfg, float g, const float* x, const float* noise, float* x_prev,
                                const float* c8, int64_t n, pcdm_stream_t s) {
    if (!pred || !x || !x_prev || !c8 || n <= 0) return -1;
    UnclipArgs a;
    for (int i = 0; i < 8; ++i) a.c[i] = c8[i];
    PCDM_LAUNCH(unclip_step_kernel, grid1d(n, 256), dim3(256), 0, (hipStream_t)s, pred, cfg, g, x, noise, x_prev, a, n);
    PCDM_CHECK_LAUNCH();
    return 0;
}

extern "C" int pcdm_unclip_step_dev(const float* pred, int cfg, float g, float* x, const float* noise_all, const float* coef,
                                    const int32_t* step_dev, int64_t n, pcdm_stream_t s) {
    if (!pred || !x || !coef || !step_dev || n <= 0) return -1;
    PCDM_LAUNCH(unclip_step_dev_kernel, grid1d(n, 256), dim3(256), 0, (hipStream_t)s, pred, cfg, g, x, noise_all, coef, step_dev, n);
    PCDM_CHECK_LAUNCH();
    return 0;
}

extern "C" int pcdm_lincomb(float* y, int nin, const float* const* xs, const float* c, int64_t n, pcdm_stream_t s) {
    if (!y || nin <= 0 || nin > 6 || !xs || !c || n <= 0) return -1;
    LinArgs a;
    for (int i = 0; i < 6; ++i) {
        a.x[i] = i < nin ? xs[i] : nullptr;
        a.c[i] = i < nin ? c[i] : 0.f;
    }
    PCDM_LAUNCH(lincomb_kernel, grid1d(n, 256), dim3(256), 0, (hipStream_t)s, y, nin, a, (const float*)nullptr, n);
    PCDM_CHECK_LAUNCH();
    return 0;
}

extern "C" int pcdm_rescale_noise_cfg(const float* cfg_eps, const float* text_eps, float* out, int N, int64_t n,
                                      float guidance_rescale, pcdm_stream_t s) {
    if (!cfg_eps || !text_eps || !out || N <= 0 || n <= 1) return -1;
    PCDM_LAUNCH(rescale_cfg_kernel, dim3(N), dim3(1024), 0, (hipStream_t)s, cfg_eps, text_eps, out, n, guidance_rescale);
    PCDM_CHECK_LAUNCH();
    return 0;
}

__global__ __launch_bounds__(256) void quantize_fp8_kernel(const u16* __restrict__ x, uint8_t* __restrict__ y, int64_t rows, int cols,
                                                           int cols_pad, int64_t ldx, int64_t ldy, float scale) {
    const int per_row = cols_pad / 8;
    const int64_t i = (int64_t)blockIdx.x * blockDim.x + threadIdx.x;
    if (i >= rows * per_row) return;
    const int64_t r = i / per_row;
    const int c = (int)(i - r * per_row) * 8;
    float v[8];
    if (c + 8 <= cols && (ldx & 7) == 0 && ((uintptr_t)x & 15) == 0) {
        const u16x8 a = *(const u16x8*)(x + r * ldx + c);
#pragma unroll
        for (int e = 0; e < 8; ++e) v[e] = bf2f(a[e]);
    } else {
#pragma unroll
        for (int e = 0; e < 8; ++e) v[e] = c + e < cols ? bf2f(x[r * ldx + c + e]) : 0.f;
    }
#pragma unroll
    for (int e = 0; e < 8; ++e) {
        const float t = v[e] * scale;
        v[e] = t > 448.f ? 448.f : (t < -448.f ? -448.f : t);
    }
    u32x2 o = {pack4_fp8(v[0], v[1], v[2], v[3]), pack4_fp8(v[4], v[5], v[6], v[7])};
    *(u32x2*)(y + r * ldy + c) = o;
}

extern "C" int pcdm_quantize_fp8(const void* x, void* y, int64_t rows, int cols, int cols_pad, int64_t ldx, int64_t ldy, float scale,
                                 pcdm_stream_t s) {
    if (!x || !y || rows <= 0 || cols <= 0 || cols_pad < cols || cols_pad % 8 || ldy % 8 || ldy < cols_pad || ldx < cols ||
        ((uintptr_t)y & 7)) return -1;
// ... 55 lines not shown
```

### pcdms_amd/csrc/unet_ctx.hip

```cpp
#include "pcdm_device.h"
#include "../../include/pcdm.h"

#include <algorithm>
#include <cstdio>
#include <cstdlib>
#include <cstring>
#include <map>
#include <string>
#include <tuple>
#include <vector>

namespace {
struct PW {
    const void* w = nullptr;
    const float* bias = nullptr;
    const float* wsum = nullptr;
    int N = 0, K = 0, Npad = 0, cin = 0;
};
struct Vec {
    const float* v = nullptr;
    int n = 0;
};
typedef std::tuple<int, int, int, int, int, int, int, int, int, int, int> TileKey;

// ... 117 lines not shown
        return it->second.v;
    }
    void chk(int r, const char* what) {
        if (r != 0 && rc == 0) {
            rc = r;
            u->err = std::string(what) + " failed";
        }
    }

    struct G {
        const void* a2 = nullptr;
        int64_t lda2 = 0;
        const void* a3 = nullptr;
        int64_t lda3 = 0;
        int c1 = 0;
        const float* rowvec = nullptr;
        int64_t ldrv = 0;
        int rows_per_batch = 0;
        const void* residual = nullptr;
        int64_t ldr = 0;
        int res_mod = 0;
        int epilogue = PCDM_EPI_STORE;
        void* out2 = nullptr;
        int64_t ldo2 = 0;
        int vt_col0 = 0;
        int conv = 0, B = 0, Hi = 0, Wi = 0, Ho = 0, Wo = 0, stride = 1, upsample = 0;
        uint64_t tap_lut = 0;
        int tap_group_n = 0;
        int zero_rows = 0;
        int64_t ldo = 0;
        const PW* ln = nullptr;
        float ln_eps = 0.f;
        int dup_rows = 0;
        const int32_t* rowvec_step = nullptr;
        int64_t rowvec_step_stride = 0;
        int rowvec_step_count = 0;
        int32_t* step_error = nullptr;
        int defer = 0;
        float* row_stats = nullptr;
    };
    bool stats_valid = false;
    pcdm_gn_splitk_src pend;
    const void* pend_out = nullptr;
    void gemm(const void* a, int64_t lda, int M, const PW* w, void* out, const G& g) {
        if (rc || !w) return;
        pcdm_gemm_params p;
        memset(&p, 0, sizeof(p));
        p.struct_size = (uint32_t)sizeof(p);
        p.a = a;
        p.lda = lda;
        p.c1 = g.c1 ? g.c1 : (g.a2 ? (int)lda : w->K);
        p.a2 = g.a2;
        p.lda2 = g.lda2;
        p.a3 = g.a3;
        p.lda3 = g.lda3;
        p.tap_lut = g.tap_lut;
        p.tap_group_n = g.tap_group_n;
        p.conv = g.conv;
        if (g.conv) {
            p.B = g.B; p.Hi = g.Hi; p.Wi = g.Wi; p.Ho = g.Ho; p.Wo = g.Wo;
            p.stride = g.stride; p.upsample = g.upsample; p.cin = w->cin;
        }
        p.w = w->w;
        p.M = M; p.N = w->N; p.K = w->K; p.Npad = w->Npad;
        p.bias = w->bias;
        p.rowvec = g.rowvec;
        p.ldrv = g.ldrv;
        p.rows_per_batch = g.rows_per_batch ? g.rows_per_batch : M;
        p.residual = g.residual;
        p.ldr = g.residual ? (g.ldr ? g.ldr : w->N) : 0;
        p.res_mod = g.res_mod;
        p.epilogue = g.epilogue;
        p.vt_col0 = g.vt_col0;
        p.out = out;
        p.ldo = g.ldo ? g.ldo : w->N;
        p.out2 = g.out2;
        p.ldo2 = g.ldo2;
        p.zero_rows = g.zero_rows;
        p.dup_rows = g.dup_rows;
        p.rowvec_step = g.rowvec ? g.rowvec_step : nullptr;
        p.rowvec_step_stride = g.rowvec_step_stride;
        p.rowvec_step_count = g.rowvec_step_count;
        p.step_error = g.step_error;
        const TileKey key{0, M, w->Npad, w->K, g.conv, g.conv ? g.stride + (g.tap_group_n ? 20 : 0) : 0, g.upsample, g.epilogue, g.a2 ? 1 : 0, g.residual ? 1 : 0, g.zero_rows ? 1 : (g.dup_rows ? 2 : 0)};
        auto it = u->tiles.find(key);
        if (it != u->tiles.end() && !(it->second.first >= 31  && (g.rowvec || (g.residual && g.res_mod < M)))) {
            p.tile = it->second.first;
            if (it->second.second > 1) {
                p.split_k = it->second.second;
                p.ws = buf<float>("splitk");
                p.ws_floats = kSplitKFloats;
                if ((int64_t)p.split_k * M * w->Npad > kSplitKFloats) { p.split_k = 0; p.tile = 0; p.ws = nullptr; p.ws_floats = 0; }
            }
        }
        if (g.row_stats) {
            const int tl = p.tile;
            stats_valid = (tl == 2 || tl == 4 || tl == 5 || tl == 6 || tl == 7 || tl == 8 || tl == 10 || tl == 18) && p.split_k <= 1 && !g.conv &&
                          g.epilogue == PCDM_EPI_STORE && w->N % 32 == 0;
            if (stats_valid) p.row_stats_out = g.row_stats;
        } else {
            stats_valid = false;
        }
        if (pend_out) { rc = -1; u->err = "a deferred split-K reduce was never consumed"; return; }
        if (g.defer && p.split_k > 1 && g.epilogue == PCDM_EPI_STORE && p.ldo == w->N && (!g.residual || g.res_mod == M || g.res_mod == 0) &&
            !getenv_off("PCDM_DEFER_SPLITK")) {
            p.defer_reduce = 1;
            memset(&pend, 0, sizeof(pend));
            pend.part = p.ws; pend.split_k = p.split_k; pend.M = M; pend.N = w->N; pend.Npad = w->Npad;
            pend.bias = p.bias; pend.rowvec = p.rowvec; pend.ldrv = g.rowvec ? (g.ldrv ? g.ldrv : w->N) : 0;
            pend.rowvec_step = p.rowvec_step; pend.rowvec_step_stride = p.rowvec_step_stride;
            pend.rowvec_step_count = p.rowvec_step_count; pend.step_error = p.step_error;
            pend.residual = p.residual; pend.ldr = p.ldr;
            pend.pre_out = out; pend.store_pre = g.defer == 1;
            pend_out = out;
        }
        chk(pcdm_gemm(&p, st), "pcdm_gemm");
    }
    bool ln_wants_stats(int M, const PW* w, const PW* w_ln, int epilogue) const {
        if (!w || !w_ln || !w_ln->wsum || w->K == 320 || w->K % 64 || w->K > 1280 || getenv_off("PCDM_LN_TILED")) return false;
        auto it = u->tiles.find(TileKey{1, M, w->Npad, w->K, 0, 0, 0, epilogue, 0, 0, 0});
        return it != u->tiles.end() && it->second.first > 0 && it->second.second == 2;
    }
    void gemm_ln(const void* a, int64_t lda, int M, const PW* w, const PW* w_ln, const float* gamma, const float* beta, float eps, void* ln_buf,
                 void* out, G g) {
        if (rc || !w) return;
        if (w_ln && w_ln->wsum && (w->K == 320 || !getenv_off("PCDM_LN_TILED"))) {
            auto it = u->tiles.find(TileKey{1, M, w->Npad, w->K, 0, 0, 0, g.epilogue, 0, 0, 0});
            if (it != u->tiles.end() && it->second.first > 0) {
                pcdm_gemm_params p;
                memset(&p, 0, sizeof(p));
        p.struct_size = (uint32_t)sizeof(p);
                p.a = a; p.lda = lda; p.c1 = w->K;
                p.w = w_ln->w; p.M = M; p.N = w_ln->N; p.K = w_ln->K; p.Npad = w_ln->Npad;
                p.bias = w_ln->bias;
                p.rows_per_batch = g.rows_per_batch ? g.rows_per_batch : M;
                p.epilogue = g.epilogue; p.vt_col0 = g.vt_col0;
                p.out = out; p.ldo = g.ldo ? g.ldo : w->N;
                p.out2 = g.out2; p.ldo2 = g.ldo2;
                p.ln_wsum = w_ln->wsum; p.ln_eps = eps;
                if (it->second.second == 2 && g.row_stats && stats_valid) p.ln_row_stats = g.row_stats;
                p.tile = it->second.first;
                const int rc_ = pcdm_gemm(&p, st);
                if (rc_ != -1) {
                    chk(rc_, "pcdm_gemm (LayerNorm folded)");
                    return;
                }
            }
        }
        chk(pcdm_layernorm(a, ln_buf, M, w->K, eps, gamma, beta, st), "pcdm_layernorm");
        g.row_stats = nullptr;
        gemm(ln_buf, w->K, M, w, out, g);
    }
    void groupnorm(const void* x1, int C1, const void* x2, int C2, int B, int HW, float eps, const float* gamma, const float* beta, int silu, void* y) {
        if (rc) return;
        if (pend_out) {
            if (pend_out != x1 || pend.N != C1) { rc = -1; u->err = "deferred split-K reduce: the next GroupNorm reads another tensor"; return; }
            pend_out = nullptr;
            chk(pcdm_groupnorm_splitk(&pend, x2, C2, B, HW, u->cfg.norm_groups, eps, gamma, beta, silu, y, buf<float>("gnws"), st), "pcdm_groupnorm_splitk");
            return;
        }
        chk(pcdm_groupnorm(x1, C1, x2, C2, B, HW, u->cfg.norm_groups, eps, gamma, beta, silu, y, buf<float>("gnws"), st), "pcdm_groupnorm");
    }
};

int64_t lp8(int64_t v) { return (v + 7) / 8 * 8; }
int64_t lp16(int64_t v) { return (v + 15) / 16 * 16; }

// ... 469 lines not shown
            g.a2 = R.buf("t0"); g.lda2 = cc;
            g.residual = x; g.ldr = cc; g.res_mod = M;
            R.gemm(R.buf("ff"), 4 * cc, M, R.pw(p + "ffo"), out, g);
            return out;
        }
        {
            Run::G g;
            g.residual = R.buf("t0"); g.ldr = cc; g.res_mod = M;
            R.gemm(R.buf("ff"), 4 * cc, M, R.pw(p + "ff2"), R.buf("t1"), g);
        }
        Run::G g;
        g.residual = x; g.ldr = cc; g.res_mod = M;
        R.gemm(R.buf("t1"), cc, M, R.pw(p + "proj_out"), out, g);
        return out;
    };

    const int HW = h * w;
    struct Skip { const void* p; int hh, ww, ch; };
    std::vector<Skip> skips;
    const void* x;
    {
        Run::G g;
        g.conv = 1; g.B = B; g.Hi = h; g.Wi = w; g.Ho = h; g.Wo = w;
        if (pose_b > 0) { g.residual = R.buf("pose"); g.ldr = C0; g.res_mod = B * HW; }
        if (shared) {
            g.B = B / 2; g.dup_rows = (B / 2) * HW;
            if (pose_b > 0) g.res_mod = g.dup_rows;
            R.gemm(x_in, 0, (B / 2) * HW, R.pw("conv_in"), R.buf("skip0"), g);
        } else
        R.gemm(x_in, 0, B * HW, R.pw("conv_in"), R.buf("skip0"), g);
        x = R.buf("skip0");
    }
    skips.push_back({x, h, w, C0});
    int hh = h, ww = w;
    for (int i = 0; i < n && !R.rc; ++i) {
        const int ci = c.block_out_channels[i];
        int cprev = i == 0 ? C0 : c.block_out_channels[i - 1];
        for (int j = 0; j < Lb; ++j) {
            const std::string nm = "d" + std::to_string(i) + "." + std::to_string(j), rp = "down_blocks." + std::to_string(i) + ".resnets." + std::to_string(j) + ".";
            if (has_cross(c, i)) {
                x = resnet(rp, x, j == 0 ? cprev : ci, nullptr, 0, hh * ww, hh, ww, "r", true, shared && i == 0 && j == 0);
                x = transformer("down_blocks." + std::to_string(i) + ".attentions." + std::to_string(j) + ".", x, ci, c.heads[i], hh * ww, nm);
            } else {
                x = resnet(rp, x, j == 0 ? cprev : ci, nullptr, 0, hh * ww, hh, ww, nm, j < Lb - 1 || i == n - 1, shared && i == 0 && j == 0);
            }
            skips.push_back({x, hh, ww, ci});
        }
        if (i != n - 1) {
            const int ho = (hh - 1) / 2 + 1, wo = (ww - 1) / 2 + 1;
            Run::G g;
            g.conv = 1; g.B = B; g.Hi = hh; g.Wi = ww; g.Ho = ho; g.Wo = wo; g.stride = 2;
            g.defer = 1;
            void* o = R.buf("ds" + std::to_string(i));
            R.gemm(x, 0, B * ho * wo, R.pw("down_blocks." + std::to_string(i) + ".downsamplers.0.conv"), o, g);
            x = o;
            hh = ho; ww = wo;
            skips.push_back({x, hh, ww, ci});
        }
    }
    const int cm = c.block_out_channels[n - 1];
    x = resnet("mid_block.resnets.0.", x, cm, nullptr, 0, hh * ww, hh, ww, "r", true);
    x = transformer("mid_block.attentions.0.", x, cm, c.heads[n - 1], hh * ww, "r2");
    x = resnet("mid_block.resnets.1.", x, cm, nullptr, 0, hh * ww, hh, ww, "r", true);
    int cx = cm;
    for (int i = 0; i < n && !R.rc; ++i) {
        const int co = c.block_out_channels[n - 1 - i];
        for (int j = 0; j < Lb + 1; ++j) {
            const Skip sk = skips.back();
            skips.pop_back();
            if (sk.hh != hh || sk.ww != ww) { u->err = "skip size mismatch"; return -1; }
            x = resnet("up_blocks." + std::to_string(i) + ".resnets." + std::to_string(j) + ".", x, cx, sk.p, sk.ch, hh * ww, hh, ww, (j + i) % 2 ? "r" : "rb",
                       has_cross(c, n - 1 - i) || j < Lb || i == n - 1);
            cx = co;
            if (has_cross(c, n - 1 - i))
                x = transformer("up_blocks." + std::to_string(i) + ".attentions." + std::to_string(j) + ".", x, co, c.heads[n - 1 - i], hh * ww, j % 2 ? "u" : "ub");
        }
        if (i != n - 1) {
            const int ho = skips.back().hh, wo = skips.back().ww;
            const std::string up4 = "up_blocks." + std::to_string(i) + ".upsamplers.0.conv4";
            if (u->w.count(up4) && ho == 2 * hh && wo == 2 * ww) {
                Run::G g4;
                g4.conv = 1; g4.B = B; g4.Hi = hh; g4.Wi = ww; g4.Ho = hh; g4.Wo = ww;
                g4.tap_lut = 0x8754764354214310ull; g4.tap_group_n = cx;
                R.gemm(x, 0, B * hh * ww, R.pw(up4), R.buf("c1"), g4);
                R.chk(pcdm_pixel_shuffle2(R.buf("c1"), R.buf("us"), B, hh, ww, cx, s), "pcdm_pixel_shuffle2");
                x = R.buf("us");
                hh = ho; ww = wo;
                continue;
            }
            Run::G g;
            g.conv = 1; g.B = B; g.Hi = hh; g.Wi = ww; g.Ho = ho; g.Wo = wo; g.upsample = 1;
            g.defer = 1;
            R.gemm(x, 0, B * ho * wo, R.pw("up_blocks." + std::to_string(i) + ".upsamplers.0.conv"), R.buf("us"), g);
            x = R.buf("us");
            hh = ho; ww = wo;
        }
    }
    R.groupnorm(x, C0, nullptr, 0, B, HW, eps, R.vec("conv_norm_out.weight"), R.vec("conv_norm_out.bias"), 1, R.buf("gn"));
    {
        Run::G g;
        g.conv = 1; g.B = B; g.Hi = h; g.Wi = w; g.Ho = h; g.Wo = w; g.rows_per_batch = HW; g.epilogue = PCDM_EPI_NCHW_F32;
        R.gemm(R.buf("gn"), 0, B * HW, R.pw("conv_out"), eps_out, g);
    }
    return R.rc;
}

namespace {
inline uint16_t host_f2bf(float f) {
    uint32_t x;
    memcpy(&x, &f, 4);
    if ((x & 0x7fffffffu) > 0x7f800000u) return (uint16_t)((x >> 16) | 0x40);
    x += 0x7fffu + ((x >> 16) & 1u);
    return (uint16_t)(x >> 16);
}
}

extern "C" int pcdm_pack_linear(const float* w, const float* bias, int N, int K, int pad_to, uint16_t* out_w, float* out_bias) {
    if (N <= 0 || K <= 0 || K % 64 || pad_to <= 0) return -1;
    const int Npad = (N + pad_to - 1) / pad_to * pad_to;
    if (out_w) {
        if (!w) return -1;
        for (int64_t n = 0; n < Npad; ++n)
            for (int64_t k = 0; k < K; ++k) out_w[n * K + k] = n < N ? host_f2bf(w[n * K + k]) : 0;
    }
    if (out_bias)
        for (int n = 0; n < Npad; ++n) out_bias[n] = (bias && n < N) ? bias[n] : 0.f;
    return Npad;
}

extern "C" int pcdm_pack_conv3x3(const float* w, const float* bias, int N, int Cin, int pad_to, uint16_t* out_w, float* out_bias, int* K_out,
                                 int* cin_out) {
    if (N <= 0 || Cin <= 0 || pad_to <= 0) return -1;
    const int Cp = (Cin + 63) / 64 * 64, K = 9 * Cp;
    const int Npad = (N + pad_to - 1) / pad_to * pad_to;
    if (K_out) *K_out = K;
    if (cin_out) *cin_out = Cp;
    if (out_w) {
        if (!w) return -1;
        memset(out_w, 0, (size_t)Npad * K * sizeof(uint16_t));
        for (int64_t n = 0; n < N; ++n)
            for (int c = 0; c < Cin; ++c)
                for (int t = 0; t < 9; ++t) out_w[n * K + t * Cp + c] = host_f2bf(w[(n * Cin + c) * 9 + t]);
    }
    if (out_bias)
        for (int n = 0; n < Npad; ++n) out_bias[n] = (bias && n < N) ? bias[n] : 0.f;
    return Npad;
}

extern "C" int pcdm_pack_geglu(const float* w, const float* bias, int D, int K, uint16_t* out_w, float* out_bias) {
    if (D <= 0 || K <= 0 || K % 64) return -1;
    const int Dp = (D + 63) / 64 * 64;
    for (int64_t r = 0; r < 2 * Dp && (out_w || out_bias); ++r) {
        const int blk = (int)(r / 64), in = (int)(r % 64);
        const int d = blk * 32 + (in & 31);
        const bool gate = in >= 32;
        const int64_t src = gate ? (int64_t)D + d : d;
        if (out_w) {
            if (!w) return -1;
            for (int64_t k = 0; k < K; ++k) out_w[r * K + k] = d < D ? host_f2bf(w[src * K + k]) : 0;
        }
        if (out_bias) out_bias[r] = (bias && d < D) ? bias[src] : 0.f;
    }
    return 2 * Dp;
}
```

### pcdms_amd/ops.py

```python
from __future__ import annotations

import ctypes as C
import json
import math
import os
from pathlib import Path
from dataclasses import dataclass
from typing import Optional, Sequence, Union

import torch

from . import _lib
from ._lib import GemmParams

EPI_STORE, EPI_GEGLU, EPI_SPLIT_VT, EPI_NCHW_F32 = 0, 1, 2, 3
ACT_NONE, ACT_SILU, ACT_GELU = 0, 1, 2
BF16 = torch.bfloat16
LAUNCH_LOG: Optional[list] = None
LAUNCH_KEYS: Optional[list] = None
LAUNCH_SPANS: Optional[list] = None
LN_REFUSED: Optional[set] = None
AUTOTUNE = True
DEFER_SPLITK = os.environ.get("PCDM_DEFER_SPLITK", "1") != "0"


def _stream(t: torch.Tensor) -> Optional[int]:
    if t.is_cuda:
        return torch.cuda.current_stream(t.device).cuda_stream
    if not _lib.is_emulator():
        raise RuntimeError("pcdms_amd ops need tensors on the MI355X (device 'cuda'); there is no CPU path")
    return None


def _ptr(t: Optional[torch.Tensor]) -> Optional[int]:
    return None if t is None else t.data_ptr()


def _chk(rc: int, name: str) -> None:
    if rc != 0:
        raise RuntimeError(f"{name} failed with code {rc}")


def _c(t: torch.Tensor, dtype) -> torch.Tensor:
    assert t.dtype == dtype and t.is_contiguous(), (t.dtype, dtype, t.is_contiguous())
    return t


ROWGEMM_TILES = (31, 32, 33, 34, 35, 36)
STATS_TILES = (2, 4, 5, 6, 7, 8, 10, 18)
_STATS_VALID: dict = {}
LN_TILED = os.environ.get("PCDM_LN_TILED", "1") != "0"
LN_TILED_TILES = (18, 4, 7, 17, 26, 8, 2)
LN_PARTIALS_TILES = (23,)
TILE_SHAPES = {1: (256, 128), 2: (64, 64), 3: (256, 64), 4: (128, 128), 5: (128, 64), 6: (256, 64), 7: (128, 128),
               8: (64, 64), 9: (256, 128), 10: (128, 64), 11: (256, 128), 12: (256, 64), 13: (256, 64), 14: (256, 64),
               15: (128, 64), 16: (512, 64), 17: (256, 256), 18: (128, 128),
               21: (192, 320), 26: (192, 256), 22: (176, 320), 23: (176, 256),
               31: (192, 128), 32: (192, 64), 33: (96, 128), 34: (192, 64), 35: (128, 64), 36: (64, 64)}
_TUNED: dict = {}
_WS: dict = {}
_WS_RETIRED: list = []
_WS_GEN: dict = {}
TUNE_ITERS = 3
TUNE_REPEATS = 1
TUNE_COLD = False
_FLUSH: dict = {}


def _launch(t: torch.Tensor, call, name: str, work: float, info: tuple, *extra, key=None) -> int:
    if LAUNCH_LOG is None or not t.is_cuda:
        return call()
    e0, e1 = torch.cuda.Event(enable_timing=True), torch.cuda.Event(enable_timing=True)
    e0.record()
    rc = call()
    if rc == 0:
        e1.record()
        LAUNCH_LOG.append((name, work, e0, e1, info, *extra))
        if LAUNCH_KEYS is not None and key is not None:
            LAUNCH_KEYS.append((len(LAUNCH_LOG) - 1, key))
    return rc


def _time_launches(fn, iters: int) -> float:
    e0, e1 = torch.cuda.Event(enable_timing=True), torch.cuda.Event(enable_timing=True)
    e0.record()
    for _ in range(iters):
        fn()
    e1.record()
    e1.synchronize()
    return e0.elapsed_time(e1)


def groupnorm_ws(B: int, C: int, device) -> torch.Tensor:
    n = _lib.lib().pcdm_groupnorm_ws_floats(B, C)
    return torch.zeros(n, dtype=torch.float32, device=device)


def groupnorm_cluster_timeouts(ws: torch.Tensor) -> int:
# ... 181 lines not shown
def pack_geglu_ln(w, bias, gamma, beta, device) -> PackedWeight:
    wf, bf = fold_layernorm(w, bias, gamma, beta)
    return _with_wsum(pack_geglu(wf, bf, device))


def gemm(a: torch.Tensor, pw: PackedWeight, out: torch.Tensor, *, a2: Optional[torch.Tensor] = None, a3: Optional[torch.Tensor] = None,
         rowvec: Optional[torch.Tensor] = None, rows_per_batch: Optional[int] = None,
         residual: Optional[torch.Tensor] = None, res_mod: int = 0, epilogue: int = EPI_STORE,
         out2: Optional[torch.Tensor] = None, vt_col0: int = 0, conv: Optional[dict] = None, tile: int = 0,
         use_bias: bool = True, split_k: int = 1, w_ld: int = 0, act: int = ACT_NONE, zero_rows: int = 0,
         ln: Optional[tuple] = None, ln_buf: Optional[torch.Tensor] = None, pw_ln: Optional[PackedWeight] = None,
         defer_reduce: Optional[bool] = None, dup_rows: int = 0, rowvec_step: Optional[torch.Tensor] = None,
         rowvec_step_stride: int = 0, row_stats: Optional[torch.Tensor] = None, rowvec_step_count: int = 0,
         step_error: Optional[torch.Tensor] = None, tap_lut: int = 0, tap_group_n: int = 0) -> Union[torch.Tensor, "DeferredGemm"]:
    if ln is not None and conv is None and a2 is None and ln_buf is not None:
        return _gemm_ln(a, pw, pw_ln, out, ln, ln_buf, rows_per_batch=rows_per_batch, epilogue=epilogue, out2=out2, vt_col0=vt_col0,
                        tile=tile, row_stats=row_stats)
    assert ln is None
    p = GemmParams()
    assert a.dtype == BF16 and a.stride(-1) == 1 and (conv is None or a.is_contiguous())
    p.a = _ptr(a)
    p.ldw = w_ld
    if conv is not None:
        p.conv = 1
        p.B, p.Hi, p.Wi, p.Ho, p.Wo = conv["B"], conv["Hi"], conv["Wi"], conv["Ho"], conv["Wo"]
        p.stride, p.upsample, p.cin = conv.get("stride", 1), conv.get("upsample", 0), pw.cin
        p.no_pad_lo = conv.get("no_pad_lo", 0)
        assert a.numel() == p.B * p.Hi * p.Wi * pw.cin, (a.shape, pw.cin)
        M = p.B * p.Ho * p.Wo
        if tap_group_n:
            assert a2 is None and a3 is None and pw.K % pw.cin == 0 and pw.K // pw.cin <= 4, (pw.K, pw.cin)
            p.tap_lut, p.tap_group_n = int(tap_lut), int(tap_group_n)
        elif a2 is not None:
            assert a2.dtype == BF16 and a2.dim() == 2 and a2.shape[0] == M and a2.stride(-1) == 1
            p.a2, p.lda2, p.c1 = _ptr(a2), a2.stride(0), a2.shape[1]
            cx = a2.shape[1]
            if a3 is not None:
                assert a3.dtype == BF16 and a3.dim() == 2 and a3.shape[0] == M and a3.stride(-1) == 1
                p.a3, p.lda3 = _ptr(a3), a3.stride(0)
                cx += a3.shape[1]
            assert pw.K == 9 * pw.cin + cx, (pw.K, pw.cin, cx)
        else:
            assert a3 is None and pw.K == 9 * pw.cin, (pw.K, pw.cin)
    else:
        M = a.shape[0]
        p.lda = a.stride(0)
        p.c1 = a.shape[1]
        assert a3 is None
        if a2 is not None:
            assert a2.dtype == BF16 and a2.stride(-1) == 1
            p.a2 = _ptr(a2)
            p.lda2 = a2.stride(0)
            assert a.shape[1] + a2.shape[1] == pw.K
        else:
            assert a.shape[1] == pw.K, (a.shape, pw.K)
    p.w = _ptr(pw.w)
    p.M, p.N, p.K, p.Npad = M, pw.N, pw.K, pw.Npad
    p.bias = _ptr(pw.bias) if (use_bias and pw.bias is not None) else None
    p.rows_per_batch = rows_per_batch or M
    if rowvec is not None:
        assert rowvec.dtype == torch.float32 and rowvec.shape[-1] == pw.N and rowvec.stride(-1) == 1
        p.rowvec = _ptr(rowvec)
        p.ldrv = rowvec.stride(0)
        if rowvec_step is not None:
            assert rowvec_step.dtype == torch.int32 and rowvec_step.device == rowvec.device
            p.rowvec_step, p.rowvec_step_stride = _ptr(rowvec_step), int(rowvec_step_stride)
            p.rowvec_step_count = int(rowvec_step_count)
            if step_error is not None:
                assert step_error.dtype == torch.int32 and step_error.device == rowvec.device
                p.step_error = _ptr(step_error)
    if residual is not None:
        _c(residual, BF16)
        p.residual = _ptr(residual)
        p.ldr = residual.stride(0) if residual.dim() == 2 else pw.N
        p.res_mod = res_mod
    p.epilogue = epilogue
    p.act = act
    p.zero_rows = zero_rows
    p.dup_rows = dup_rows
    assert not dup_rows or (conv is not None and out.shape[0] >= M + dup_rows)
    p.vt_col0 = vt_col0
    p.out = _ptr(out)
    p.ldo = out.stride(0) if (out.dim() == 2 and epilogue != EPI_NCHW_F32) else pw.N
    if out2 is not None:
        p.out2 = _ptr(out2)
        p.ldo2 = out2.shape[-1]
    stream = _stream(a)
    split = 1
    key = None
    if tile == 0 and AUTOTUNE:
        key = (M, pw.Npad, pw.K, p.conv, p.stride + (10 if p.no_pad_lo else 0) + (20 if tap_group_n else 0), p.upsample, epilogue,
               a2 is not None, residual is not None) + ((True,) if zero_rows else ((2,) if dup_rows else ()))
        tile, split = _TUNED.get(key, (0, 1))
        if tile in ROWGEMM_TILES and (rowvec is not None or act != ACT_NONE or (residual is not None and res_mod < M)):
            tile, split = 0, 1
        elif tile == 0 and a.is_cuda and not torch.cuda.is_current_stream_capturing():
            tile, split = _TUNED[key] = _autotune(p, stream, pw, epilogue, a.device, out)
    elif split_k > 1:
        split = split_k
    p.tile = tile
    if row_stats is not None:
        ok = tile in STATS_TILES and split == 1 and conv is None and epilogue == EPI_STORE and act == ACT_NONE and pw.N % 32 == 0
        _STATS_VALID[row_stats.untyped_storage().data_ptr()] = ok
        if ok:
            assert row_stats.dtype == torch.float32 and row_stats.is_contiguous() and row_stats.numel() >= M * (pw.N // 32) * 2
            p.row_stats_out = _ptr(row_stats)
    deferred = None
    if split > 1:
        ws = _splitk_ws(a.device, split * M * pw.Npad)
        p.split_k, p.ws, p.ws_floats = split, ws.data_ptr(), ws.numel()
        if defer_reduce is not None and DEFER_SPLITK and epilogue == EPI_STORE and act == ACT_NONE and (residual is None or res_mod in (0, M)) \
                and (rowvec is None or (rows_per_batch and M % rows_per_batch == 0)) and out.is_contiguous() and out.shape == (M, pw.N):
            p.defer_reduce = 1
            deferred = DeferredGemm(part=ws.data_ptr(), split_k=split, M=M, N=pw.N, Npad=pw.Npad, bias=p.bias, rowvec=p.rowvec,
                                    ldrv=p.ldrv if rowvec is not None else 0, rowvec_step=p.rowvec_step, rowvec_step_stride=p.rowvec_step_stride,
                                    rowvec_step_count=p.rowvec_step_count, step_error=p.step_error,
                                    rpb=p.rows_per_batch, residual=p.residual, ldr=p.ldr, out=out,
                                    store=bool(defer_reduce), keep=(ws, rowvec, residual, pw, rowvec_step, step_error))
    _chk(_launch(a, lambda: _lib.lib().pcdm_gemm(C.byref(p), stream), "gemm_kernel", 2.0 * M * pw.alg_nk,
                 (M, pw.N, pw.K, bool(conv), tile, split), 2.0 * (M - zero_rows) * (pw.exec_nk or pw.alg_nk), key=key), "pcdm_gemm")
    return out if deferred is None else deferred


def row_stats_valid(row_stats: Optional[torch.Tensor]) -> bool:
    return row_stats is not None and _STATS_VALID.get(row_stats.untyped_storage().data_ptr(), False)


def ln_wants_row_stats(M: int, pw: "PackedWeight", epilogue: int) -> bool:
    if not LN_TILED or pw.K == 320 or pw.K % 64 or pw.K > 1280:
        return False
    ch = _TUNED.get(("ln", M, pw.Npad, pw.K, epilogue))
    return ch is None or (len(ch) > 1 and ch[0] > 0 and ch[1] == 2)


def row_stats_reference(a: torch.Tensor) -> torch.Tensor:
    M, K = a.shape
    v = a.float().view(M, K // 32, 32)
    sm = v.sum(-1)
    return torch.stack([sm, ((v - sm.unsqueeze(-1) / 32) ** 2).sum(-1)], -1).contiguous()


def _gemm_ln(a, pw, pw_ln, out, ln, ln_buf, *, rows_per_batch, epilogue, out2, vt_col0, tile, row_stats=None):
    gamma, beta, eps = ln
    M = a.shape[0]
    assert a.dtype == BF16 and a.stride(1) == 1 and a.shape[1] == pw.K and ln_buf.shape[0] >= M
    key = ("ln", M, pw.Npad, pw.K, epilogue)
    span0 = len(LAUNCH_LOG) if (LAUNCH_SPANS is not None and LAUNCH_LOG is not None and not tile) else None
    have_stats = row_stats_valid(row_stats)
    choice = (tile, 2 if have_stats else 1) if tile else _TUNED.get(key)
    if not LN_TILED and not tile and pw.K != 320:
        pw_ln = None
    stream = _stream(a)

    def fused(t, stats=None):
        p = GemmParams()
        p.a, p.lda, p.c1 = _ptr(a), a.stride(0), a.shape[1]
        p.w, p.M, p.N, p.K, p.Npad = _ptr(pw_ln.w), M, pw_ln.N, pw_ln.K, pw_ln.Npad
        p.bias = _ptr(pw_ln.bias)
        p.rows_per_batch = rows_per_batch or M
        p.epilogue, p.vt_col0 = epilogue, vt_col0
        p.out = _ptr(out)
        p.ldo = out.stride(0)
        if out2 is not None:
            p.out2, p.ldo2 = _ptr(out2), out2.shape[-1]
        p.ln_wsum, p.ln_eps = _ptr(_c(pw_ln.wsum, torch.float32)), float(eps)
        if stats is not None:
            p.ln_row_stats = _ptr(stats)
        p.tile = t
        return _lib.lib().pcdm_gemm(C.byref(p), stream)

    def two_launches():
        n = layernorm(a, gamma, beta, eps, ln_buf[:M])
        return gemm(n, pw, out, rows_per_batch=rows_per_batch, epilogue=epilogue, out2=out2, vt_col0=vt_col0)

# ... 262 lines not shown
def cfg_step(eps: torch.Tensor, cfg: bool, g: float, x: Optional[torch.Tensor], x_prev: Optional[torch.Tensor],
             coef: Optional[torch.Tensor], step_dev: Optional[torch.Tensor] = None,
             noise: Optional[torch.Tensor] = None, eps_out: Optional[torch.Tensor] = None) -> None:
    n = eps.numel() // (2 if cfg else 1)
    _c(eps, torch.float32)
    _chk(_lib.lib().pcdm_cfg_step(_ptr(eps), int(cfg), g, _ptr(x), _ptr(noise), _ptr(x_prev), _ptr(eps_out),
                                  _ptr(coef), _ptr(step_dev), n, _stream(eps)), "pcdm_cfg_step")


def unipc_step(eps: torch.Tensor, cfg: bool, g: float, x: torch.Tensor, m1: torch.Tensor, m2: torch.Tensor, last: torch.Tensor,
               coef: torch.Tensor, step_dev: Optional[torch.Tensor] = None) -> None:
    n = x.numel()
    for t in (eps, x, m1, m2, last, coef):
        _c(t, torch.float32)
    assert eps.numel() == (2 * n if cfg else n) and m1.numel() == m2.numel() == last.numel() == n and coef.shape[-1] == 12
    _chk(_lib.lib().pcdm_unipc_step(_ptr(eps), int(cfg), float(g), _ptr(x), _ptr(m1), _ptr(m2), _ptr(last), _ptr(coef),
                                    _ptr(step_dev), n, _stream(x)), "pcdm_unipc_step")


def dpmpp_step(eps: torch.Tensor, cfg: bool, g: float, x: torch.Tensor, m1: torch.Tensor, noise_all: Optional[torch.Tensor],
               coef: torch.Tensor, step_dev: Optional[torch.Tensor] = None) -> None:
    n = x.numel()
    for t in (eps, x, m1, coef):
        _c(t, torch.float32)
    assert eps.numel() == (2 * n if cfg else n) and m1.numel() == n and coef.shape[-1] == 8
    if noise_all is not None:
        assert _c(noise_all, torch.float32).numel() == coef.shape[0] * n
    _chk(_lib.lib().pcdm_dpmpp_step(_ptr(eps), int(cfg), float(g), _ptr(x), _ptr(m1), _ptr(noise_all), _ptr(coef),
                                    _ptr(step_dev), n, _stream(x)), "pcdm_dpmpp_step")


def unclip_step(pred: torch.Tensor, cfg: bool, g: float, x: torch.Tensor, noise: Optional[torch.Tensor], out: torch.Tensor,
                coefs: Sequence[float]) -> torch.Tensor:
    _c(pred, torch.float32); _c(x, torch.float32); _c(out, torch.float32)
    n = x.numel()
    assert pred.numel() == (2 * n if cfg else n) and out.numel() == n and len(coefs) == 8
    if noise is not None:
        assert _c(noise, torch.float32).numel() == n
    carr = (C.c_float * 8)(*[float(c) for c in coefs])
    _chk(_lib.lib().pcdm_unclip_step(_ptr(pred), int(cfg), float(g), _ptr(x), _ptr(noise), _ptr(out), carr, n, _stream(x)),
         "pcdm_unclip_step")
    return out


def unclip_step_dev(pred: torch.Tensor, cfg: bool, g: float, x: torch.Tensor, noise_all: Optional[torch.Tensor], coef: torch.Tensor,
                    step_dev: torch.Tensor) -> None:
    _c(pred, torch.float32); _c(x, torch.float32); _c(coef, torch.float32)
    n = x.numel()
    assert pred.numel() == (2 * n if cfg else n) and coef.shape[-1] == 8
    if noise_all is not None:
        assert _c(noise_all, torch.float32).numel() == coef.shape[0] * n
    _chk(_lib.lib().pcdm_unclip_step_dev(_ptr(pred), int(cfg), float(g), _ptr(x), _ptr(noise_all), _ptr(coef), _ptr(step_dev), n,
                                         _stream(x)), "pcdm_unclip_step_dev")


def lincomb(out: torch.Tensor, xs: Sequence[torch.Tensor], cs: Sequence[float]) -> torch.Tensor:
    n = len(xs)
    assert 1 <= n <= 6 and len(cs) == n
    for t in xs:
        _c(t, torch.float32)
        assert t.numel() == out.numel()
    arr = (C.c_void_p * n)(*[t.data_ptr() for t in xs])
    carr = (C.c_float * n)(*[float(c) for c in cs])
    _chk(_lib.lib().pcdm_lincomb(_ptr(out), n, arr, carr, out.numel(), _stream(out)), "pcdm_lincomb")
    return out


def rescale_noise_cfg(cfg_eps: torch.Tensor, text_eps: torch.Tensor, out: torch.Tensor, guidance_rescale: float) -> torch.Tensor:
    _c(cfg_eps, torch.float32); _c(text_eps, torch.float32); _c(out, torch.float32)
    N = cfg_eps.shape[0]
    _chk(_lib.lib().pcdm_rescale_noise_cfg(_ptr(cfg_eps), _ptr(text_eps), _ptr(out), N, cfg_eps.numel() // N,
                                           float(guidance_rescale), _stream(out)), "pcdm_rescale_noise_cfg")
    return out


def softmax_rows(s: torch.Tensor, out: torch.Tensor, scale: float) -> torch.Tensor:
    assert s.dtype == torch.float32 and out.dtype == BF16 and s.stride(1) == 1 and out.stride(1) == 1
    rows, cols = s.shape
    _chk(_lib.lib().pcdm_softmax_rows(_ptr(s), _ptr(out), rows, cols, s.stride(0), out.stride(0), float(scale), _stream(s)),
         "pcdm_softmax_rows")
    return out


def advance_step(step_dev: torch.Tensor) -> None:
    _chk(_lib.lib().pcdm_advance_step(_ptr(step_dev), _stream(step_dev)), "pcdm_advance_step")


def _win(w: Sequence[int]):
    return (C.c_int32 * 4)(*[int(v) for v in w])


def _images(cand: torch.Tensor, ref: torch.Tensor) -> int:
    assert cand.dim() == 4 and ref.dim() == 4 and cand.dtype == ref.dtype and cand.dtype in (torch.uint8, torch.float32), (cand.shape, ref.shape, cand.dtype, ref.dtype)
    assert cand.is_contiguous() and ref.is_contiguous() and cand.device == ref.device
    return int(cand.dtype == torch.float32)


def metrics_ws_bytes(N: int, ref_n: int, W: int, H: int, sigma: float) -> int:
    return int(_lib.lib().pcdm_metrics_ws_bytes(N, ref_n, W, H, float(sigma)))


def ssim(cand: torch.Tensor, ref: torch.Tensor, cand_win: Sequence[int], ref_win: Sequence[int], scores: torch.Tensor, argmax: Optional[torch.Tensor],
         ws: torch.Tensor, *, sigma: float = 1.2, data_range: Optional[float] = None) -> torch.Tensor:
    f32 = _images(cand, ref)
    _c(scores, torch.float32)
    if argmax is not None:
        _c(argmax, torch.int32)
    _chk(_lib.lib().pcdm_ssim(_ptr(cand), cand.shape[0], cand.shape[1], cand.shape[2], _win(cand_win), _ptr(ref), ref.shape[0], ref.shape[1], ref.shape[2],
                              _win(ref_win), cand.shape[3], f32, float(sigma), -1.0 if data_range is None else float(data_range), _ptr(scores),
                              _ptr(argmax), _ptr(ws), ws.numel() * ws.element_size(), _stream(cand)), "pcdm_ssim")
    return scores


def psnr(cand: torch.Tensor, ref: torch.Tensor, cand_win: Sequence[int], ref_win: Sequence[int], mse: Optional[torch.Tensor], out: Optional[torch.Tensor],
         ws: torch.Tensor, *, data_range: float = 255.0) -> Optional[torch.Tensor]:
    f32 = _images(cand, ref)
    for t in (mse, out):
        if t is not None:
            _c(t, torch.float32)
    _chk(_lib.lib().pcdm_psnr(_ptr(cand), cand.shape[0], cand.shape[1], cand.shape[2], _win(cand_win), _ptr(ref), ref.shape[0], ref.shape[1], ref.shape[2],
                              _win(ref_win), cand.shape[3], f32, float(data_range), _ptr(mse), _ptr(out), _ptr(ws), ws.numel() * ws.element_size(),
                              _stream(cand)), "pcdm_psnr")
    return out


def absdiff(cand: torch.Tensor, ref: torch.Tensor, cand_win: Sequence[int], ref_win: Sequence[int], l1: Optional[torch.Tensor],
            mae: Optional[torch.Tensor], ws: torch.Tensor) -> None:
    f32 = _images(cand, ref)
    for t in (l1, mae):
        if t is not None:
            _c(t, torch.float32)
    N, W, H = cand.shape[0], int(cand_win[2]), int(cand_win[3])
    call = lambda: _lib.lib().pcdm_absdiff(_ptr(cand), N, cand.shape[1], cand.shape[2], _win(cand_win), _ptr(ref), ref.shape[0], ref.shape[1],
                                           ref.shape[2], _win(ref_win), cand.shape[3], f32, _ptr(l1), _ptr(mae), _ptr(ws),
                                           ws.numel() * ws.element_size(), _stream(cand))
    _chk(_launch(cand, call, "absdiff", 3.0 * N * W * H * 3, (N, H, W, f32)), "pcdm_absdiff")


def ssim_box_ws_bytes(N: int, ref_n: int, W: int, H: int, win_size: int) -> int:
    return int(_lib.lib().pcdm_ssim_box_ws_bytes(N, ref_n, W, H, int(win_size)))


def ssim_box(cand: torch.Tensor, ref: torch.Tensor, cand_win: Sequence[int], ref_win: Sequence[int], scores: torch.Tensor, ws: torch.Tensor, *,
             win_size: int = 51, data_range: Optional[float] = None) -> torch.Tensor:
    f32 = _images(cand, ref)
    _c(scores, torch.float32)
    N, W, H, w = cand.shape[0], int(cand_win[2]), int(cand_win[3]), int(win_size)
    call = lambda: _lib.lib().pcdm_ssim_box(_ptr(cand), N, cand.shape[1], cand.shape[2], _win(cand_win), _ptr(ref), ref.shape[0], ref.shape[1],
                                            ref.shape[2], _win(ref_win), cand.shape[3], f32, w, -1.0 if data_range is None else float(data_range),
                                            _ptr(scores), _ptr(ws), ws.numel() * ws.element_size(), _stream(cand))
    _chk(_launch(cand, call, "ssim_box", 10.0 * N * 3 * max(W - w + 1, 0) * max(H - w + 1, 0) * 2 * w, (N, H, W, w)), "pcdm_ssim_box")
    return scores


def select_image(cand: torch.Tensor, win: Sequence[int], index: torch.Tensor, out: torch.Tensor, normalized: bool) -> torch.Tensor:
    assert cand.dim() == 4
    _c(cand, torch.uint8); _c(index, torch.int32); _c(out, torch.float32 if normalized else torch.uint8)
    _chk(_lib.lib().pcdm_select_image(_ptr(cand), cand.shape[0], cand.shape[1], cand.shape[2], _win(win), cand.shape[3], _ptr(index), _ptr(out),
                                      int(normalized), _stream(cand)), "pcdm_select_image")
    return out


def pack_lpips_conv(w: torch.Tensor, bias: Optional[torch.Tensor], device) -> dict:
    assert w.dim() == 4, w.shape
    w = w.detach().to("cpu", torch.float32).contiguous()
    b = None if bias is None else bias.detach().to("cpu", torch.float32).contiguous()
# ... 224 lines not shown
```

### pcdms_amd/pipeline.py

```python
from __future__ import annotations

import inspect
from dataclasses import dataclass
from typing import Any, Callable, List, Optional, Union

import torch

from . import ops
from .schedulers import DDIMScheduler, DDPMScheduler, DPMSolverMultistepScheduler, UniPCMultistepScheduler, _step_noise
from .unet import Stage2_InapintUNet2DConditionModel


@dataclass
class Stage2_InpaintDiffusionPipelineOutput:
    images: Any
    nsfw_content_detected: Optional[List[bool]] = None
    latents: Optional[torch.Tensor] = None


def rescale_noise_cfg(noise_cfg, noise_pred_text, guidance_rescale=0.0):
    a, b = noise_cfg.float().contiguous(), noise_pred_text.float().contiguous()
    return ops.rescale_noise_cfg(a, b, torch.empty_like(a), guidance_rescale).to(noise_cfg.dtype)


def retrieve_timesteps(scheduler, num_inference_steps: Optional[int] = None, device=None, timesteps: Optional[List[int]] = None,
                       **kwargs):
    if timesteps is not None:
        if "timesteps" not in set(inspect.signature(scheduler.set_timesteps).parameters.keys()):
            raise ValueError(f"The current scheduler class {scheduler.__class__}'s `set_timesteps` does not support custom"
                             f" timestep schedules. Please check whether you are using the correct scheduler.")
        scheduler.set_timesteps(timesteps=timesteps, device=device, **kwargs)
        timesteps = scheduler.timesteps
        num_inference_steps = len(timesteps)
    else:
        scheduler.set_timesteps(num_inference_steps, device=device, **kwargs)
        timesteps = scheduler.timesteps
    return timesteps, num_inference_steps


class Stage2_InpaintDiffusionPipeline:
    use_prior_embed = True

    def __init__(self, unet: Stage2_InapintUNet2DConditionModel, scheduler, vae=None, c_schedule: bool = False):
        self.unet = unet
        self.scheduler = scheduler
        self.vae = vae
        self.vae_scale_factor = 8
        self.c_schedule = c_schedule
        self._ctx = None
        self._graph = None
        self._graph_key = None
        self._st = {}

    _unet_kwargs: dict = {}

    @classmethod
    def from_pretrained(cls, pretrained_model_name_or_path, torch_dtype=None, **kwargs):
        import json
        from pathlib import Path

        from . import schedulers as S
        from .unet import UNet2DConditionModel
        from .vae import AutoencoderKL
        root = Path(str(pretrained_model_name_or_path))
        vae = AutoencoderKL.from_pretrained(root, subfolder="vae", torch_dtype=torch_dtype) if (root / "vae").is_dir() else None
        unet = UNet2DConditionModel.from_pretrained(root, subfolder="unet", torch_dtype=torch_dtype, **cls._unet_kwargs)
        scfg = {}
        sj = root / "scheduler" / "scheduler_config.json"
        if sj.exists():
            scfg = json.loads(sj.read_text())
        sched_cls = getattr(S, str(scfg.get("_class_name", "")), None)
        if not (isinstance(sched_cls, type) and issubclass(sched_cls, S._Base)):
            sched_cls = S.DDIMScheduler
        return cls(unet, sched_cls.from_config(scfg), vae=vae)

    @property
    def device(self):
        return self.unet.device

    _execution_device = device

    def to(self, device):
        self.unet.to(device)
        if self.vae is not None and hasattr(self.vae, "to"):
            self.vae.to(device)
        return self

    def enable_xformers_memory_efficient_attention(self, attention_op=None):
        self.unet.set_use_memory_efficient_attention_xformers(True, attention_op)

    def prepare_extra_step_kwargs(self, generator, eta):
        params = set(inspect.signature(self.scheduler.step).parameters.keys())
        kw = {}
# ... 56 lines not shown
            feature_f = torch.cat([s_img_proj_f.to(**f32), pred_t_img_embed.to(**f32)], dim=1).repeat_interleave(N, 0)
            prior_embed = pred_t_img_embed.to(**f32).repeat_interleave(N, 0)
        else:
            feature_f = s_img_proj_f.to(**f32).repeat_interleave(N, 0)
            prior_embed = None
        if do_cfg:
            feature_f = torch.cat([torch.zeros_like(feature_f), feature_f], dim=0)
            if prior_embed is not None:
                prior_embed = torch.cat([torch.zeros_like(prior_embed), prior_embed], dim=0)
        feature_f = feature_f.contiguous()
        if prior_embed is not None:
            prior_embed = prior_embed.contiguous()

        self.scheduler.set_timesteps(num_inference_steps, device=device)
        timesteps = self.scheduler.timesteps
        lat = self.prepare_latents(bs * N, 4, height, width, torch.float32, device, generator, latents).contiguous()
        extra = self.prepare_extra_step_kwargs(generator, eta)

        lat = self._sample(lat, mask, masked, pose_cond, feature_f, prior_embed, timesteps, do_cfg, guidance_scale, guidance_rescale,
                           eta, extra, mode, use_graph, callback, callback_steps, zero_uncond=do_cfg,
                           shared_halves=do_cfg)

        images = self._postprocess(lat, output_type)
        if not return_dict:
            return (images, None)
        return Stage2_InpaintDiffusionPipelineOutput(images=images, nsfw_content_detected=None, latents=lat)

    def _sample(self, lat, mask, masked, pose_cond, feature_f, prior_embed, timesteps, do_cfg, guidance_scale, guidance_rescale, eta,
                extra, mode, use_graph, callback, callback_steps, zero_uncond=False, shared_halves=False):
        linear = isinstance(self.scheduler, (DDIMScheduler, DDPMScheduler)) and eta == 0.0 \
            and not isinstance(self.scheduler, DDPMScheduler)
        linear = linear or (isinstance(self.scheduler, UniPCMultistepScheduler) and self.scheduler.config.solver_order <= 2)
        linear = linear or isinstance(self.scheduler, DPMSolverMultistepScheduler)
        mode = mode or ("fused" if linear else "reference")
        if mode == "fused" and not linear:
            raise ValueError("mode='fused' needs a scheduler with one linear update per step (DDIM with eta=0, UniPC, DPM-Solver++)")

        if mode == "reference":
            self.unet.invalidate_caches()
            for i, t in enumerate(timesteps):
                x = torch.cat([lat] * 2) if do_cfg else lat
                x = self.scheduler.scale_model_input(x, t)
                B = x.shape[0]
                inp = torch.cat([x] + ([] if mask is None else [mask.expand(B, -1, -1, -1)]) + [masked.expand(B, -1, -1, -1)], dim=1)
                eps = self.unet(inp, t, class_labels=prior_embed, encoder_hidden_states=feature_f,
                                my_pose_cond=pose_cond, return_dict=False)[0]
                if do_cfg:
                    g = torch.empty_like(lat)
                    eps = eps.float().contiguous()
                    ops.cfg_step(eps, True, float(guidance_scale), None, None, None, eps_out=g)
                    if guidance_rescale > 0.0:
                        g = rescale_noise_cfg(g, eps[eps.shape[0] // 2:], guidance_rescale)
                    eps = g
                lat = self.scheduler.step(eps, t, lat, **extra, return_dict=False)[0]
                if callback is not None and i % callback_steps == 0:
                    callback(i, t, lat)
            self.unet.invalidate_caches()
        else:
            lat = self._run_fused(lat, mask, masked, pose_cond, feature_f, prior_embed, timesteps, do_cfg,
                                  float(guidance_scale), eta, use_graph, callback, callback_steps,
                                  float(guidance_rescale) if do_cfg else 0.0, zero_uncond, shared_halves and do_cfg,
                                  generator=extra.get("generator"))

        return lat

    def _postprocess(self, lat, output_type):
        if output_type == "latent" or self.vae is None:
            return lat
        z = lat / self.vae.config.scaling_factor
        if output_type == "pt":
            return (self.vae.decode(z, return_dict=False)[0] / 2 + 0.5).clamp(0, 1)
        u8 = self.vae.decode_to_uint8(z)
        if output_type == "uint8":
            return u8
        arr = u8.cpu().numpy()
        if output_type == "np":
            return arr.astype("float32") / 255.0
        from PIL import Image
        return [Image.fromarray(a) for a in arr]

    def _step_eager(self, st):
        unet = self.unet
        B, h, w = st["B"], st["h"], st["w"]
        x_in = ops.assemble_input(st["lat"], st["rep"], st["mask"], st["masked"], st["x_in"])
        if st.get("ctx") is not None:
            eps = st["ctx"].forward(x_in, st["timesteps"], st["step"], B, h, w, st["pose_b"], out=st["eps_c"])
        else:
            eps = unet._forward_nhwc(x_in, B, h, w, st["timesteps"], st["cond"], step_dev=st["step"])
        cfg, g, e = st["rep"] == 2, st["g"], eps
        if st["gr"] > 0.0:
            n = eps.shape[0] // 2
            ops.cfg_step(eps, True, st["g"], None, None, None, eps_out=st["eps_g"])
            ops.rescale_noise_cfg(st["eps_g"], eps[n:], st["eps_g"], st["gr"])
            cfg, g, e = False, 1.0, st["eps_g"]
        if st["unipc"]:
            ops.unipc_step(e, cfg, g, st["lat"], st["m1"], st["m2"], st["last"], st["coef"], st["step"])
        elif st["dpm"]:
            ops.dpmpp_step(e, cfg, g, st["lat"], st["m1"], st["noise"], st["coef"], st["step"])
        else:
            ops.cfg_step(e, cfg, g, st["lat"], st["lat"], st["coef"], st["step"])
        ops.advance_step(st["step"])

    @staticmethod
    def _zero_history(st):
        if st.get("unipc"):
            for k in ("m1", "m2", "last"):
                st[k].zero_()
        elif st.get("dpm"):
            st["m1"].zero_()

    def _run_fused(self, lat, mask, masked, pose_cond, feature_f, prior_embed, timesteps, do_cfg, g, eta, use_graph,
                   callback, callback_steps, guidance_rescale=0.0, zero_uncond=False, shared_halves=False, generator=None):
        unet, dev = self.unet, self.device
        if unet._w is None:
            unet._pack()
        n = len(timesteps)
        N, _, h, w = lat.shape
        rep = 2 if do_cfg else 1
        B = rep * N
        n0 = N if (do_cfg and zero_uncond) else 0
        unipc = isinstance(self.scheduler, UniPCMultistepScheduler)
        dpm = isinstance(self.scheduler, DPMSolverMultistepScheduler)
        sde = dpm and self.scheduler.stochastic
        kind = "unipc" if unipc else ("dpm_sde" if sde else "dpm") if dpm else "linear"
        key = (B, h, w, n, rep, n0, tuple(feature_f.shape), None if mask is None else tuple(mask.shape), tuple(masked.shape),
               None if pose_cond is None else tuple(pose_cond.shape), prior_embed is None, kind, bool(shared_halves))
        st = self._st if self._graph_key == key else {}
        if not st:
            st.update(B=B, h=h, w=w, rep=rep, unipc=unipc, dpm=dpm, noise=None,
                      lat=torch.empty_like(lat), mask=None if mask is None else torch.empty_like(mask), masked=torch.empty_like(masked),
                      eps_g=torch.empty_like(lat),
                      x_in=torch.empty(B, h, w, 64, dtype=ops.BF16, device=dev),
                      step=torch.zeros(1, dtype=torch.int32, device=dev),
                      timesteps=torch.empty(n, dtype=torch.int64, device=dev),
                      coef=torch.empty(n, 12 if unipc else 8 if dpm else 4, dtype=torch.float32, device=dev))
            if unipc:
                st.update(m1=torch.zeros_like(lat), m2=torch.zeros_like(lat), last=torch.zeros_like(lat))
            if dpm:
                st.update(m1=torch.zeros_like(lat), noise=torch.empty(n, lat.numel(), dtype=torch.float32, device=dev) if sde else None)
            self._graph = None
        st["lat"].copy_(lat)
        if mask is not None:
            st["mask"].copy_(mask)
        st["masked"].copy_(masked)
        st["timesteps"].copy_(timesteps.to(dev))
        st["cond"] = unet.prepare_conditioning(B, h, w, feature_f, prior_embed, pose_cond, zero_ctx_batches=n0, shared_cfg_input=shared_halves,
                                               timesteps=st["timesteps"])
        st["coef"].copy_(self.scheduler.coefficient_table(device=dev) if (unipc or dpm) else self.scheduler.coefficient_table(eta, device=dev))
        if sde:
            for i in range(n):
                st["noise"][i].copy_(_step_noise(lat.shape, generator, dev).reshape(-1))
        st["g"] = g
        if st.get("gr", guidance_rescale) != guidance_rescale:
            self._graph = None
        st["gr"] = guidance_rescale
        w_gen = (id(unet), getattr(unet, "_pack_gen", 0), ops.workspace_generation(dev))
        if st.get("w_gen") != w_gen:
            self._graph = None
        st["ctx"] = None
        if self.c_schedule:
            from .unet_ctx import UNetContext
            if self._ctx is None or self._ctx._pack_gen != unet._pack_gen or self._ctx.unet is not unet:
                self._ctx = UNetContext(unet)
                self._graph = None
            if st.get("c_tuned") != (id(self._ctx), w_gen) and dev.type == "cuda":
                lat0 = lat.clone()
                st["step"].zero_()
                self._zero_history(st)
                self._step_eager(st)
                st["lat"].copy_(lat0)
                st["step"].zero_()
                self._zero_history(st)
                self._ctx.sync_tiles()
                w_gen2 = (id(unet), getattr(unet, "_pack_gen", 0), ops.workspace_generation(dev))
                if w_gen2 != w_gen:
                    self._graph = None
                w_gen = w_gen2
                st["c_tuned"] = (id(self._ctx), w_gen)
            st["pose_b"] = self._ctx.prepare_conditioning(B, h, w, feature_f, prior_embed, pose_cond, zero_ctx_batches=n0,
                                                          shared_cfg_input=st["cond"].shared_halves)
            self._ctx.prepare_timesteps(st["timesteps"], B, h, w)
            st["eps_c"] = st.get("eps_c") if st.get("eps_c") is not None and st["eps_c"].shape[0] == B else \
                torch.empty(B, unet.config.out_channels, h, w, dtype=torch.float32, device=dev)
            st["ctx"] = self._ctx
        st["step"].zero_()
        self._zero_history(st)
        self._st, self._graph_key = st, key
        if use_graph and dev.type == "cuda":
            if self._graph is None or self._st.get("g_captured") != g:
                lat0 = st["lat"].clone()
                self._step_eager(st)
                torch.cuda.synchronize()
                st["lat"].copy_(lat0)
                st["step"].zero_()
                self._zero_history(st)
                graph = torch.cuda.CUDAGraph()
                with torch.cuda.graph(graph, capture_error_mode="thread_local"):
                    self._step_eager(st)
                st["lat"].copy_(lat0)
                st["step"].zero_()
                self._zero_history(st)
                self._graph = graph
                st["g_captured"] = g
                w_gen = (id(unet), getattr(unet, "_pack_gen", 0), ops.workspace_generation(dev))
            st["w_gen"] = w_gen
            for i in range(n):
                self._graph.replay()
                if callback is not None and i % callback_steps == 0:
                    callback(i, timesteps[i], st["lat"].clone())
        else:
            st["w_gen"] = w_gen
            for i in range(n):
                self._step_eager(st)
                if callback is not None and i % callback_steps == 0:
                    callback(i, timesteps[i], st["lat"])
        out = st["lat"].clone()
        if hasattr(unet, "step_overflow") and unet.step_overflow():
            raise RuntimeError("the device step counter left the time-embedding table of this sampling call (clamped on the device): "
                               "the schedule ran more steps than prepare_conditioning(timesteps=...) was given")
        return out


class Simple_Stage2_InpaintDiffusionPipeline(Stage2_InpaintDiffusionPipeline):

    use_prior_embed = False


class Stage3_RefinedDiffusionPipeline(Stage2_InpaintDiffusionPipeline):

    @torch.no_grad()
    def __call__(self, height: Optional[int] = None, width: Optional[int] = None, num_inference_steps: int = 50,
                 guidance_scale: float = 7.5, num_images_per_prompt: Optional[int] = 1, eta: float = 0.0, generator=None,
                 latents: Optional[torch.Tensor] = None, output_type: Optional[str] = "pil", return_dict: bool = True,
                 callback=None, callback_steps: int = 1, guidance_rescale: float = 0.0,
                 vae_gen_t_image: Optional[torch.Tensor] = None, s_img_proj_f: Optional[torch.Tensor] = None,
                 gen_t_img_latents: Optional[torch.Tensor] = None, mode: Optional[str] = None, use_graph: bool = True):
        device = self.device
        N = num_images_per_prompt
        f32 = dict(device=device, dtype=torch.float32)
        if gen_t_img_latents is None:
            if self.vae is None:
                raise ValueError("pass gen_t_img_latents=... (VAE encode is outside the hot path) or construct with vae=")
            gen_t_img_latents = self.vae.encode(vae_gen_t_image.to(device)).latent_dist.sample(generator=generator)
            gen_t_img_latents = gen_t_img_latents * self.vae.config.scaling_factor
        do_cfg = guidance_scale > 1.0
        feat = s_img_proj_f.to(**f32).repeat_interleave(N, 0)
        gl = gen_t_img_latents.to(**f32).repeat_interleave(N, 0)
        if do_cfg:
            feat = torch.cat([torch.zeros_like(feat), feat])
            gl = torch.cat([torch.zeros_like(gl), gl])
        feat, gl = feat.contiguous(), gl.contiguous()
        self.scheduler.set_timesteps(num_inference_steps, device=device)
        lat = self.prepare_latents(s_img_proj_f.shape[0] * N, 4, height, width, torch.float32, device, generator, latents).contiguous()
        extra = self.prepare_extra_step_kwargs(generator, eta)
        lat = self._sample(lat, None, gl, None, feat, None, self.scheduler.timesteps, do_cfg, guidance_scale, guidance_rescale, eta, extra,
                           mode, use_graph, callback, callback_steps, zero_uncond=do_cfg)
        images = self._postprocess(lat, output_type)
        if not return_dict:
            return (images, None)
        return Stage2_InpaintDiffusionPipelineOutput(images=images, nsfw_content_detected=None, latents=lat)


class PCDMsPipeline(Simple_Stage2_InpaintDiffusionPipeline):

    @torch.no_grad()
    def __call__(self, simg_mask_latents=None, mask=None, cond_pose=None, prompt=None, height: Optional[int] = None,
                 width: Optional[int] = None, num_inference_steps: int = 50, timesteps=None, guidance_scale: float = 7.5,
                 negative_prompt=None, num_images_per_prompt: Optional[int] = 1, eta: float = 0.0, generator=None,
                 latents: Optional[torch.Tensor] = None, prompt_embeds=None, negative_prompt_embeds=None, ip_adapter_image=None,
                 output_type: Optional[str] = "pil", return_dict: bool = True, cross_attention_kwargs=None,
                 guidance_rescale: float = 0.0, clip_skip=None, callback_on_step_end=None,
                 callback_on_step_end_tensor_inputs=("latents",), mode: Optional[str] = None, use_graph: bool = True, **kwargs):
        if prompt is not None or negative_prompt is not None or ip_adapter_image is not None or cross_attention_kwargs is not None \
                or clip_skip is not None:
            raise NotImplementedError("text prompts / IP-adapter / LoRA / clip_skip are not part of the PCDMs path")
        if prompt_embeds is None or simg_mask_latents is None or mask is None or cond_pose is None:
            raise ValueError("simg_mask_latents, mask, cond_pose and prompt_embeds are required")
        device = self.device
        N = num_images_per_prompt
        h, w = simg_mask_latents.shape[-2:]
        height, width = height or h * self.vae_scale_factor, width or w * self.vae_scale_factor
        if (height // self.vae_scale_factor, width // self.vae_scale_factor) != (h, w):
            raise ValueError("height / width do not match simg_mask_latents")
        f32 = dict(device=device, dtype=torch.float32)
# ... 32 lines not shown
```

### pcdms_amd/unet.py

```python
from __future__ import annotations

import os
from pathlib import Path
from types import SimpleNamespace
from typing import Any, Dict, Iterator, List, Optional, Tuple, Union

import torch

from . import ops
from ._module import Config, HipModel, default_init, read_checkpoint, read_config
from .ops import BF16, PackedWeight

SHARE_CFG_PREFIX = os.environ.get("PCDM_SHARE_CFG_PREFIX", "1") != "0"
TIME_TABLE = os.environ.get("PCDM_TIME_TABLE", "1") != "0"
FUSE_FF_OUT = os.environ.get("PCDM_FUSE_FF_OUT", "1") != "0"
FUSE_SHORTCUT = os.environ.get("PCDM_FUSE_SHORTCUT", "1") != "0"
PHASE_UPSAMPLE = os.environ.get("PCDM_PHASE_UPSAMPLE", "1") != "0"

_DEFAULT_CONFIG: Dict[str, Any] = dict(
    sample_size=None, in_channels=4, out_channels=4, center_input_sample=False, flip_sin_to_cos=True, freq_shift=0,
    down_block_types=("CrossAttnDownBlock2D", "CrossAttnDownBlock2D", "CrossAttnDownBlock2D", "DownBlock2D"),
    mid_block_type="UNetMidBlock2DCrossAttn",
    up_block_types=("UpBlock2D", "CrossAttnUpBlock2D", "CrossAttnUpBlock2D", "CrossAttnUpBlock2D"),
    only_cross_attention=False, block_out_channels=(320, 640, 1280, 1280), layers_per_block=2,
    downsample_padding=1, mid_block_scale_factor=1, act_fn="silu", norm_num_groups=32, norm_eps=1e-5,
    cross_attention_dim=1280, encoder_hid_dim=None, encoder_hid_dim_type=None, attention_head_dim=8,
    num_attention_heads=None, dual_cross_attention=False, use_linear_projection=False, class_embed_type=None,
    addition_embed_type=None, num_class_embeds=None, upcast_attention=False, resnet_time_scale_shift="default",
    resnet_skip_time_act=False, resnet_out_scale_factor=1.0, time_embedding_type="positional",
    time_embedding_dim=None, time_embedding_act_fn=None, timestep_post_act=None, time_cond_proj_dim=None,
    conv_in_kernel=3, conv_out_kernel=3, projection_class_embeddings_input_dim=None,
    class_embeddings_concat=False, mid_block_only_cross_attention=None, cross_attention_norm=None,
    addition_embed_type_num_heads=64,
)

SD21_BASE_UNET_CONFIG: Dict[str, Any] = dict(
    sample_size=64, in_channels=4, out_channels=4, block_out_channels=(320, 640, 1280, 1280), layers_per_block=2,
    attention_head_dim=(5, 10, 20, 20), cross_attention_dim=1024, use_linear_projection=True,
    norm_num_groups=32, norm_eps=1e-5, flip_sin_to_cos=True, freq_shift=0, act_fn="silu",
    _diffusers_version="0.24.0",
)

_REQUIRED = dict(center_input_sample=False, mid_block_type="UNetMidBlock2DCrossAttn", only_cross_attention=False,
                 act_fn="silu", encoder_hid_dim=None, encoder_hid_dim_type=None, dual_cross_attention=False,
                 addition_embed_type=None, num_class_embeds=None, resnet_time_scale_shift="default",
                 resnet_skip_time_act=False, time_embedding_type="positional", time_embedding_act_fn=None,
                 timestep_post_act=None, time_cond_proj_dim=None, conv_in_kernel=3, conv_out_kernel=3,
                 class_embeddings_concat=False, cross_attention_norm=None, downsample_padding=1)


class UNet2DConditionOutput:

    def __init__(self, sample: torch.Tensor):
        self.sample = sample

    def __getitem__(self, i):
        return (self.sample,)[i]

    def to_tuple(self):
        return (self.sample,)


def _as_tuple(v, n):
    return tuple(v) if isinstance(v, (list, tuple)) else (v,) * n


class Conditioning:

    __slots__ = ("gen", "B", "h", "w", "L", "n0", "cls_emb", "pose_nhwc", "kv", "shared_halves", "temb_all", "temb_steps", "step_error")

    def __init__(self, gen: int, B: int, h: int, w: int, L: int):
        self.gen, self.B, self.h, self.w, self.L = gen, B, h, w, L
        self.n0 = 0
        self.shared_halves = False
        self.temb_all: Optional[torch.Tensor] = None
        self.temb_steps: Optional[torch.Tensor] = None
        self.step_error: Optional[torch.Tensor] = None
        self.cls_emb: Optional[torch.Tensor] = None
        self.pose_nhwc: Optional[torch.Tensor] = None
        self.kv: Dict[str, Tuple[torch.Tensor, torch.Tensor]] = {}


class Stage2_InapintUNet2DConditionModel(HipModel):

    _pose_required = True

    def __init__(self, **kwargs):
        super().__init__()
        cfg = dict(_DEFAULT_CONFIG)
        unknown = [k for k in kwargs if k not in cfg and not k.startswith("_")]
        if unknown:
            raise TypeError(f"unexpected config keys: {unknown}")
        cfg.update(kwargs)
        for k, v in _REQUIRED.items():
            if cfg[k] != v and not (k == "only_cross_attention" and not any(_as_tuple(cfg[k], 1))):
                raise NotImplementedError(f"config {k}={cfg[k]!r} is outside the stage-2 hot path (supported: {v!r})")
        if cfg["class_embed_type"] not in (None, "projection"):
            raise NotImplementedError(f"class_embed_type={cfg['class_embed_type']!r}")
        if cfg["class_embed_type"] == "projection" and cfg["projection_class_embeddings_input_dim"] is None:
            raise ValueError("`class_embed_type`: 'projection' requires `projection_class_embeddings_input_dim` be set")
# ... 426 lines not shown
            t1 = ops.gemm(at, a["o1"], self._buf("t1", (M, c)), residual=t0, res_mod=M, row_stats=want(a.get("q2_ln"), M - r0, ops.EPI_STORE))
            k2, vt2 = kv[p]
            at2 = self._buf("at", (M, c))
            q2 = ops.gemm(t1[r0:], a["q2"], self._buf("q2", (M, c))[r0:], ln=(a["ln2"][0], a["ln2"][1], 1e-5),
                          ln_buf=self._buf("ln", (M, c))[r0:], pw_ln=a.get("q2_ln"), row_stats=None if rs is None else rs[r0:])
            (ops.flash_attn_fp8 if self._attn_fp8 else ops.flash_attn)(q2, k2, vt2, at2[r0:], B - nzero, H, HW_, L)
            if taps is not None:
                tap(p + "t1", t1), tap(p + "q2", q2), tap(p + "at2", at2[r0:])
            t2 = ops.gemm(at2, a["o2"], self._buf("t0", (M, c)), residual=t1, res_mod=M, zero_rows=r0,
                          row_stats=want(a.get("ff1_ln"), M, ops.EPI_GEGLU))
            ff = ops.gemm(t2, a["ff1"], self._buf("ff", (M, 4 * c)), epilogue=ops.EPI_GEGLU, ln=(a["ln3"][0], a["ln3"][1], 1e-5),
                          ln_buf=self._buf("ln", (M, c)), pw_ln=a.get("ff1_ln"), row_stats=rs)
            if taps is not None:
                tap(p + "t2", t2), tap(p + "ff", ff)
            if "ffo" in a:
                o = ops.gemm(ff, a["ffo"], self._buf(name, (M, c)), a2=t2, residual=x, res_mod=M)
            else:
                t3 = ops.gemm(ff, a["ff2"], self._buf("t1", (M, c)), residual=t2, res_mod=M)
                o = ops.gemm(t3, a["proj_out"], self._buf(name, (M, c)), residual=x, res_mod=M)
                if taps is not None:
                    tap(p + "t3", t3)
            if taps is not None:
                tap(p + "out", o)
            return o

        HW = h * w
        shared = cond.shared_halves
        if shared:
            Mh = (B // 2) * HW
            x = ops.gemm(x_in[: B // 2], W["conv_in"], self._buf("skip0", (B * HW, boc[0])), conv=dict(B=B // 2, Hi=h, Wi=w, Ho=h, Wo=w),
                         residual=None if pose_nhwc is None else pose_nhwc.view(-1, boc[0])[:Mh], res_mod=0 if pose_nhwc is None else Mh,
                         dup_rows=Mh)
        else:
            x = ops.gemm(x_in, W["conv_in"], self._buf("skip0", (B * HW, boc[0])), conv=dict(B=B, Hi=h, Wi=w, Ho=h, Wo=w),
                         residual=None if pose_nhwc is None else pose_nhwc.view(-1, boc[0]),
                         res_mod=0 if pose_nhwc is None else pose_nhwc.shape[0] * HW)
        if taps is not None:
            tap("conv_in.out", x)
        skips: List[Tuple[torch.Tensor, int, int]] = [(x, h, w)]
        hh, ww = h, w
        L_ = self._layers[0]

        def skip_of(t):
            return t.out if isinstance(t, ops.DeferredGemm) else t
        for i, typ in enumerate(cfg.down_block_types):
            for j in range(L_):
                nm = f"d{i}.{j}"
                first = shared and i == 0 and j == 0
                if typ == "CrossAttnDownBlock2D":
                    x = resnet(f"down_blocks.{i}.resnets.{j}.", x, None, hh * ww, hh, ww, "r", gn_next=True, shared=first)
                    x = transformer(f"down_blocks.{i}.attentions.{j}.", x, hh * ww, nm)
                else:
                    x = resnet(f"down_blocks.{i}.resnets.{j}.", x, None, hh * ww, hh, ww, nm, gn_next=j < L_ - 1 or i == nlev - 1, shared=first)
                skips.append((skip_of(x), hh, ww))
            if i != nlev - 1:
                ho, wo = (hh - 1) // 2 + 1, (ww - 1) // 2 + 1
                x = ops.gemm(x.view(B, hh, ww, boc[i]), W[f"down_blocks.{i}.downsamplers.0.conv."],
                             self._buf(f"ds{i}", (B * ho * wo, boc[i])),
                             conv=dict(B=B, Hi=hh, Wi=ww, Ho=ho, Wo=wo, stride=2), defer_reduce=True)
                if taps is not None:
                    tap(f"down_blocks.{i}.downsamplers.0.out", x)
                hh, ww = ho, wo
                skips.append((skip_of(x), hh, ww))
        all_skips = list(skips) if taps is not None else None
        x = resnet("mid_block.resnets.0.", x, None, hh * ww, hh, ww, "r", gn_next=True)
        x = transformer("mid_block.attentions.0.", x, hh * ww, "r2")
        x = resnet("mid_block.resnets.1.", x, None, hh * ww, hh, ww, "r", gn_next=True)
        rev = list(reversed(boc))
        for i, typ in enumerate(cfg.up_block_types):
            for j in range(L_ + 1):
                sk, sh, sw = skips.pop()
                assert (sh, sw) == (hh, ww)
                cross = typ == "CrossAttnUpBlock2D"
                x = resnet(f"up_blocks.{i}.resnets.{j}.", x, sk, hh * ww, hh, ww, "r" if (j + i) % 2 else "rb",
                           gn_next=cross or j < L_ or i == nlev - 1)
                if cross:
                    x = transformer(f"up_blocks.{i}.attentions.{j}.", x, hh * ww, "u" if j % 2 else "ub")
                    if taps is not None:
                        taps[f"up{i}.{j}"] = x.clone()
            if i != nlev - 1:
                ho, wo = skips[-1][1], skips[-1][2]
                w4 = W.get(f"up_blocks.{i}.upsamplers.0.conv4.")
                if w4 is not None and (ho, wo) == (2 * hh, 2 * ww):
                    ph = ops.gemm(x.view(B, hh, ww, rev[i]), w4, self._buf("usp", (B * hh * ww, 4 * rev[i])),
                                  conv=dict(B=B, Hi=hh, Wi=ww, Ho=hh, Wo=ww), tap_lut=ops.UPSAMPLE_TAP_LUT, tap_group_n=rev[i])
                    x = ops.pixel_shuffle2(ph, self._buf("us", (B * ho * wo, rev[i])), B, hh, ww, rev[i])
                    if taps is not None:
                        tap(f"up_blocks.{i}.upsamplers.0.ph", ph), tap(f"up_blocks.{i}.upsamplers.0.out", x)
                    hh, ww = ho, wo
                    continue
                x = ops.gemm(x.view(B, hh, ww, rev[i]), W[f"up_blocks.{i}.upsamplers.0.conv."],
                             self._buf("us", (B * ho * wo, rev[i])),
                             conv=dict(B=B, Hi=hh, Wi=ww, Ho=ho, Wo=wo, upsample=1), defer_reduce=True)
                if taps is not None:
                    tap(f"up_blocks.{i}.upsamplers.0.out", x)
                hh, ww = ho, wo
        ws = self._buf("gnws", (int(ops._lib.lib().pcdm_groupnorm_ws_floats(B, 4096)),), torch.float32, zero=True)
        n = ops.groupnorm(x, None, B, HW, G, eps, W["norm_out"][0], W["norm_out"][1], True, self._buf("gn", (B * HW, boc[0])), ws)
        out = self._buf("eps", (B, cfg.out_channels, h, w), torch.float32)
        ops.gemm(n, W["conv_out"], out, conv=dict(B=B, Hi=h, Wi=w, Ho=h, Wo=w), rows_per_batch=HW,
                 epilogue=ops.EPI_NCHW_F32)
        if taps is not None:
            tap_stored()
            tap("norm_out", n), tap("eps", out)
            names = ["conv_in"]
            for i in range(nlev):
                names += [f"down{i}.{j}" for j in range(L_)] + ([f"ds{i}"] if i != nlev - 1 else [])
            for nm_, (t_, _, _) in zip(names, all_skips):
                taps[nm_] = t_.clone()
        return out


def _resnets(m: Stage2_InapintUNet2DConditionModel) -> Iterator[Tuple[str, int, int, int]]:
    boc, L = m._boc, m._layers[0]
    out = boc[0]
    for i in range(len(boc)):
        cin, out = out, boc[i]
        for j in range(L):
            yield f"down_blocks.{i}.resnets.{j}.", (cin if j == 0 else out), out, i
    yield "mid_block.resnets.0.", boc[-1], boc[-1], len(boc) - 1
    yield "mid_block.resnets.1.", boc[-1], boc[-1], len(boc) - 1
    rev = list(reversed(boc))
    out = rev[0]
    for i in range(len(boc)):
        prev, out = out, rev[i]
        inc = rev[min(i + 1, len(boc) - 1)]
        for j in range(L + 1):
            skip = inc if j == L else out
            rin = prev if j == 0 else out
            yield f"up_blocks.{i}.resnets.{j}.", rin + skip, out, len(boc) - 1 - i


def _transformers(m: Stage2_InapintUNet2DConditionModel) -> Iterator[Tuple[str, int, int]]:
    boc, L = m._boc, m._layers[0]
    for i, typ in enumerate(m.config.down_block_types):
        if typ == "CrossAttnDownBlock2D":
            for j in range(L):
                yield f"down_blocks.{i}.attentions.{j}.", boc[i], m._heads[i]
        elif typ != "DownBlock2D":
            raise NotImplementedError(typ)
    yield "mid_block.attentions.0.", boc[-1], m._heads[-1]
    rev, rh = list(reversed(boc)), list(reversed(m._heads))
    for i, typ in enumerate(m.config.up_block_types):
        if typ == "CrossAttnUpBlock2D":
            for j in range(L + 1):
                yield f"up_blocks.{i}.attentions.{j}.", rev[i], rh[i]
        elif typ != "UpBlock2D":
            raise NotImplementedError(typ)


def _param_shapes(m: Stage2_InapintUNet2DConditionModel) -> Iterator[Tuple[str, Tuple[int, ...]]]:
    cfg, boc = m.config, m._boc
    temb, ctx = boc[0] * 4, cfg.cross_attention_dim
    yield "conv_in.weight", (boc[0], cfg.in_channels, 3, 3)
    yield "conv_in.bias", (boc[0],)
    for nm, din in (("time_embedding", boc[0]),) + ((("class_embedding", cfg.projection_class_embeddings_input_dim),)
                                                    if cfg.class_embed_type == "projection" else ()):
        yield f"{nm}.linear_1.weight", (temb, din)
        yield f"{nm}.linear_1.bias", (temb,)
        yield f"{nm}.linear_2.weight", (temb, temb)
        yield f"{nm}.linear_2.bias", (temb,)
    for p, cin, cout, _ in _resnets(m):
        yield p + "norm1.weight", (cin,)
        yield p + "norm1.bias", (cin,)
        yield p + "conv1.weight", (cout, cin, 3, 3)
        yield p + "conv1.bias", (cout,)
        yield p + "time_emb_proj.weight", (cout, temb)
        yield p + "time_emb_proj.bias", (cout,)
        yield p + "norm2.weight", (cout,)
# ... 49 lines not shown
```

Measured before the change: 6.398 images/s.

## Fuse pixel-shuffle into upsample GEMM store and fuse DDIM step with input assembly

Adds a SHUFFLE2 epilogue so the phase-decomposed upsample convolution writes its outputs directly at their pixel-shuffled positions. This removes the separate pixel_shuffle2 kernel and its intermediate buffer round-trip. It also adds a step_tail kernel that fuses the CFG/DDIM update, the step advance and the next step's UNet input assembly, cutting small kernel launches per step. The trade-off is scattered row stores in the GEMM epilogue and extra index arithmetic per lane.

```diff
diff --git a/include/pcdm.h b/include/pcdm.h
--- a/include/pcdm.h
+++ b/include/pcdm.h
@@ -37,7 +37,7 @@
 int pcdm_layernorm(const void* x, void* y, int rows, int C, float eps, const float* gamma, const float* beta,
                    pcdm_stream_t s);
 
-enum { PCDM_EPI_STORE = 0, PCDM_EPI_GEGLU = 1, PCDM_EPI_SPLIT_VT = 2, PCDM_EPI_NCHW_F32 = 3 };
+enum { PCDM_EPI_STORE = 0, PCDM_EPI_GEGLU = 1, PCDM_EPI_SPLIT_VT = 2, PCDM_EPI_NCHW_F32 = 3, PCDM_EPI_SHUFFLE2 = 4 };
 enum { PCDM_ACT_NONE = 0, PCDM_ACT_SILU = 1, PCDM_ACT_GELU = 2 };
 typedef struct pcdm_gemm_params {
     uint32_t struct_size;
@@ -132,6 +132,8 @@
 int pcdm_image_to_uint8(const float* x, void* out, int B, int cstride, int HW, pcdm_stream_t s);
 int pcdm_lincomb(float* y, int nin, const float* const* xs, const float* c, int64_t n, pcdm_stream_t s);
 int pcdm_advance_step(int32_t* step_dev, pcdm_stream_t s);
+int pcdm_step_tail(const float* eps, int cfg, float g, float* lat, const float* coef, int32_t* step_dev, int32_t* ticket, void* x_in,
+                   int N, int rep, int HW, int cpad, pcdm_stream_t s);
 int pcdm_pixel_shuffle2(const void* in, void* out, int B, int H, int W, int C, pcdm_stream_t s);
 
 int64_t pcdm_metrics_ws_bytes(int N, int ref_n, int W, int H, float sigma);
diff --git a/pcdms_amd/_lib.py b/pcdms_amd/_lib.py
--- a/pcdms_amd/_lib.py
+++ b/pcdms_amd/_lib.py
@@ -103,6 +103,7 @@
     "pcdm_gaussian_sample": ([_P, _P, _P, _I, _I, _I, _F, _P], C.c_int),
     "pcdm_image_to_uint8": ([_P, _P, _I, _I, _I, _P], C.c_int),
     "pcdm_advance_step": ([_P, _P], C.c_int),
+    "pcdm_step_tail": ([_P, _I, _F, _P, _P, _P, _P, _P, _I, _I, _I, _I, _P], C.c_int),
     "pcdm_pixel_shuffle2": ([_P, _P, _I, _I, _I, _I, _P], C.c_int),
     "pcdm_metrics_ws_bytes": ([_I, _I, _I, _I, _F], _L),
     "pcdm_ssim": ([_P, _I, _I, _I, _W4, _P, _I, _I, _I, _W4, _I, _I, _F, _F, _P, _P, _P, _L, _P], C.c_int),
diff --git a/pcdms_amd/csrc/gemm.hip b/pcdms_amd/csrc/gemm.hip
--- a/pcdms_amd/csrc/gemm.hip
+++ b/pcdms_amd/csrc/gemm.hip
@@ -1,36 +1,36 @@
 #include "gemm_kernel.inc"
 
 namespace {
-template <bool CONV>
+template <bool CONV, int EXT = 0>
 int dispatch_tile(int tile, const GemmArgs& a, hipStream_t st) {
     switch (tile) {
 #ifndef PCDM_DEV_NEW_TILES_ONLY
-        case 1: return launch_gemm<256, 128, 4, 2, 3, CONV>(a, st);
-        case 2: return launch_gemm<64, 64, 2, 2, 2, CONV>(a, st);
-        case 3: return launch_gemm<256, 64, 4, 2, 2, CONV>(a, st);
-        case 4: return launch_gemm<128, 128, 2, 2, 2, CONV>(a, st);
-        case 5: return launch_gemm<128, 64, 2, 2, 2, CONV>(a, st);
-        case 6: return launch_gemm<256, 64, 4, 2, 3, CONV>(a, st);
-        case 7: return launch_gemm<128, 128, 2, 2, 3, CONV>(a, st);
-        case 8: return launch_gemm<64, 64, 2, 2, 4, CONV>(a, st);
-        case 9: return launch_gemm<256, 128, 4, 2, 2, CONV>(a, st);
-        case 10: return launch_gemm<128, 64, 2, 2, 3, CONV>(a, st);
-        case 11: return launch_gemm<256, 128, 4, 2, 3, CONV, true>(a, st);
-        case 12: return launch_gemm<256, 64, 4, 2, 3, CONV, true>(a, st);
-        case 13: return launch_gemm<256, 64, 4, 1, 2, CONV>(a, st);
-        case 14: return launch_gemm<256, 64, 4, 1, 3, CONV>(a, st);
-        case 15: return launch_gemm<128, 64, 2, 1, 2, CONV>(a, st);
-        case 16: return launch_gemm<512, 64, 8, 1, 2, CONV>(a, st);
-        case 17: return launch_gemm<256, 256, 2, 4, 2, CONV>(a, st);
-        case 18: return launch_gemm<128, 128, 4, 2, 2, CONV>(a, st);
+        case 1: return launch_gemm<256, 128, 4, 2, 3, CONV, false, 32, 64, EXT>(a, st);
+        case 2: return launch_gemm<64, 64, 2, 2, 2, CONV, false, 32, 64, EXT>(a, st);
+        case 3: return launch_gemm<256, 64, 4, 2, 2, CONV, false, 32, 64, EXT>(a, st);
+        case 4: return launch_gemm<128, 128, 2, 2, 2, CONV, false, 32, 64, EXT>(a, st);
+        case 5: return launch_gemm<128, 64, 2, 2, 2, CONV, false, 32, 64, EXT>(a, st);
+        case 6: return launch_gemm<256, 64, 4, 2, 3, CONV, false, 32, 64, EXT>(a, st);
+        case 7: return launch_gemm<128, 128, 2, 2, 3, CONV, false, 32, 64, EXT>(a, st);
+        case 8: return launch_gemm<64, 64, 2, 2, 4, CONV, false, 32, 64, EXT>(a, st);
+        case 9: return launch_gemm<256, 128, 4, 2, 2, CONV, false, 32, 64, EXT>(a, st);
+        case 10: return launch_gemm<128, 64, 2, 2, 3, CONV, false, 32, 64, EXT>(a, st);
+        case 11: return launch_gemm<256, 128, 4, 2, 3, CONV, true, 32, 64, EXT>(a, st);
+        case 12: return launch_gemm<256, 64, 4, 2, 3, CONV, true, 32, 64, EXT>(a, st);
+        case 13: return launch_gemm<256, 64, 4, 1, 2, CONV, false, 32, 64, EXT>(a, st);
+        case 14: return launch_gemm<256, 64, 4, 1, 3, CONV, false, 32, 64, EXT>(a, st);
+        case 15: return launch_gemm<128, 64, 2, 1, 2, CONV, false, 32, 64, EXT>(a, st);
+        case 16: return launch_gemm<512, 64, 8, 1, 2, CONV, false, 32, 64, EXT>(a, st);
+        case 17: return launch_gemm<256, 256, 2, 4, 2, CONV, false, 32, 64, EXT>(a, st);
+        case 18: return launch_gemm<128, 128, 4, 2, 2, CONV, false, 32, 64, EXT>(a, st);
 #endif
-        case 21: return launch_gemm<192, 320, 2, 4, 2, CONV, false, 16>(a, st);
-        case 22: return launch_gemm<176, 320, 2, 4, 2, CONV, false, 16>(a, st);
-        case 23: return launch_gemm<176, 256, 2, 4, 2, CONV, false, 16>(a, st);
-        case 26: return launch_gemm<192, 256, 2, 4, 2, CONV, false, 16>(a, st);
+        case 21: return launch_gemm<192, 320, 2, 4, 2, CONV, false, 16, 64, EXT>(a, st);
+        case 22: return launch_gemm<176, 320, 2, 4, 2, CONV, false, 16, 64, EXT>(a, st);
+        case 23: return launch_gemm<176, 256, 2, 4, 2, CONV, false, 16, 64, EXT>(a, st);
+        case 26: return launch_gemm<192, 256, 2, 4, 2, CONV, false, 16, 64, EXT>(a, st);
 #ifdef PCDM_DEV_KB32
-        case 27: return launch_gemm<192, 320, 2, 4, 4, CONV, false, 16, 32>(a, st);
-        case 28: return launch_gemm<256, 256, 2, 4, 4, CONV, false, 16, 32>(a, st);
+        case 27: return launch_gemm<192, 320, 2, 4, 4, CONV, false, 16, 32, EXT>(a, st);
+        case 28: return launch_gemm<256, 256, 2, 4, 4, CONV, false, 16, 32, EXT>(a, st);
 #endif
         default: return -1;
     }
@@ -50,7 +50,12 @@
                    (p->a2 && (int64_t)p->M * p->lda2 * 2 >= lim) || (p->a3 && (int64_t)p->M * p->lda3 * 2 >= lim))
                 : ((int64_t)p->M * p->lda * 2 >= lim || (p->a2 && (int64_t)p->M * p->lda2 * 2 >= lim))) return -2;
     const int64_t out_esz = p->epilogue == PCDM_EPI_NCHW_F32 ? 4 : 2;
-    if ((int64_t)p->M * (p->ldo > 0 ? p->ldo : p->N) * out_esz >= lim || (p->residual && (int64_t)p->M * (p->ldr > 0 ? p->ldr : p->N) * 2 >= lim))
+    const bool shuffle2 = p->epilogue == PCDM_EPI_SHUFFLE2;
+    if (shuffle2 && (!p->conv || p->tap_group_n <= 0 || p->N != 4 * p->tap_group_n || (p->ldo > 0 && p->ldo < p->tap_group_n) || p->act || p->defer_reduce ||
+                     p->row_stats_out || p->ln_wsum || p->ln_row_stats || (p->tile & 0xff) >= pcdm_gemm_detail::kRowGemmTile0))
+        return -1;
+    const int64_t out_rows = shuffle2 ? 4 * (int64_t)p->M : p->M, out_cols = shuffle2 ? p->tap_group_n : p->N;
+    if (out_rows * (p->ldo > 0 ? p->ldo : out_cols) * out_esz >= lim || (p->residual && (int64_t)p->M * (p->ldr > 0 ? p->ldr : p->N) * 2 >= lim))
         return -2;
     GemmArgs a;
     a.a = (const u16*)p->a;
@@ -82,10 +87,11 @@
     a.residual = (const u16*)p->residual;
     a.ldr = p->ldr;
     a.res_mod = p->res_mod > 0 ? p->res_mod : p->M;
-    a.epilogue = p->epilogue;
+    a.epilogue = shuffle2 ? (int)PCDM_EPI_STORE : p->epilogue;
+    a.shuffle2 = shuffle2 ? 1 : 0;
     a.vt_col0 = p->vt_col0;
     a.out = p->out;
-    a.ldo = p->ldo;
+    a.ldo = (shuffle2 && p->ldo <= 0) ? p->tap_group_n : p->ldo;
     a.out2 = (u16*)p->out2;
     a.ldo2 = p->ldo2;
     a.tiles_m = a.tiles_n = 0;
@@ -108,7 +114,7 @@
     if (a.defer_reduce && (p->act || p->res_mod > 0 && p->res_mod < p->M)) return -1;
     a.ws = p->ws;
     if (a.split_k > 1) {
-        if (p->epilogue != PCDM_EPI_STORE || !p->ws || a.split_k > p->K / BK || a.split_k > 64) return -1;
+        if (a.epilogue != PCDM_EPI_STORE || !p->ws || a.split_k > p->K / BK || a.split_k > 64) return -1;
         if (p->ws_floats < (int64_t)a.split_k * p->M * p->Npad) return -1;
     }
     if (p->conv && p->tap_group_n > 0) {
@@ -187,5 +193,6 @@
     } else if ((needs128 && !n128) || (tile == 17 && p->Npad % 256)) {
         return -1;
     }
+    if (a.shuffle2) return dispatch_tile<true, 4>(tile, a, st);
     return p->conv ? dispatch_tile<true>(tile, a, st) : dispatch_tile<false>(tile, a, st);
 }
diff --git a/pcdms_amd/csrc/gemm_args.h b/pcdms_amd/csrc/gemm_args.h
--- a/pcdms_amd/csrc/gemm_args.h
+++ b/pcdms_amd/csrc/gemm_args.h
@@ -47,6 +47,7 @@
     int dup_rows;
     int defer_reduce;
     int debug;
+    int shuffle2;
 };
 }
 
@@ -62,6 +63,15 @@
 __device__ __forceinline__ const float* rowvec_base(const GemmArgs& p) {
     return (p.rowvec && p.rowvec_step) ? p.rowvec + (int64_t)bounded_step(p.rowvec_step, p.rowvec_step_count, p.step_error) * p.rowvec_step_stride : p.rowvec;
 }
+__device__ __forceinline__ int shuffle2_phase(const GemmArgs& p, int n) {
+    return (n >= p.tap_group_n ? 1 : 0) + (n >= 2 * p.tap_group_n ? 1 : 0) + (n >= 3 * p.tap_group_n ? 1 : 0);
+}
+__device__ __forceinline__ int shuffle2_row(const GemmArgs& p, int m, int phase) {
+    const unsigned hw = (unsigned)(p.Hi * p.Wi);
+    const unsigned b = (unsigned)m / hw, rem = (unsigned)m - b * hw;
+    const unsigned y = rem / (unsigned)p.Wi, x = rem - y * (unsigned)p.Wi;
+    return (int)(((b * 2u * p.Hi + 2u * y + (unsigned)(phase >> 1)) * 2u * p.Wi) + 2u * x + (unsigned)(phase & 1));
+}
 __device__ __forceinline__ float apply_act(float v, int act) {
     return act == PCDM_ACT_SILU ? silu_f(v) : act == PCDM_ACT_GELU ? gelu_erf_f(v) : v;
 }
diff --git a/pcdms_amd/csrc/gemm_kernel.inc b/pcdms_amd/csrc/gemm_kernel.inc
--- a/pcdms_amd/csrc/gemm_kernel.inc
+++ b/pcdms_amd/csrc/gemm_kernel.inc
@@ -33,10 +33,10 @@
     for (int it = 0; it < G::NIT; ++it) rv[it] = buf_load16_once(rs_r, (G::TAIL && it * G::RPI + rl >= 32) ? kOOB : vr0 + it * sr);
 }
 
-template <int WCOLS, int EPW, int RV, bool STATS = false>
+template <int WCOLS, int EPW, int RV, bool STATS = false, bool SHUF = false>
 __device__ __forceinline__ void lean_pass(const GemmArgs& p, float* ep, int lane, int mrow0, int ncol0, f32x4 b0, f32x4 b1,
                                           BufRsrc rs_o, BufRsrc rs_v, const u32x4 (&rv)[4], const float* rvec_w, int rv_pitch,
-                                          int rv_col0, int rv_split_row) {
+                                          int rv_col0, int rv_split_row, int srow_lane = 0, int scol = 0) {
     static_assert(!STATS || WCOLS == 32 || WCOLS == 64, "row statistics: passes of 32 or 64 columns");
     typedef PassGeom<WCOLS> G;
     constexpr int LPR = G::LPR, RPI = G::RPI, NIT = G::NIT;
@@ -84,7 +84,12 @@
         o[1] = pack2bf(a0[2], a0[3]);
         o[2] = pack2bf(a1[0], a1[1]);
         o[3] = pack2bf(a1[2], a1[3]);
-        buf_store16(rs_o, (TAIL && r >= 32) ? kOOB : vo0 + it * so, o);
+        uint32_t vo = (TAIL && r >= 32) ? kOOB : vo0 + it * so;
+        if constexpr (SHUF) {
+            const int sr = __shfl(srow_lane, r & 31, 64);
+            vo = (lane_ok && !(TAIL && r >= 32) && sr >= 0) ? (uint32_t)((sr * (int)p.ldo + n - scol) * 2) : kOOB;
+        }
+        buf_store16(rs_o, vo, o);
         if constexpr (STATS) {
             float v[8];
 #pragma unroll
@@ -179,8 +184,8 @@
 
 template <int BM, int BN, int WGM, int WGN, int STAGES, bool CONV, bool STAG = false, int F = 32, int KB = 64, int EXT = 0>
 __global__ __launch_bounds__(WGM* WGN * 64) void gemm_kernel(const GemmArgs p) {
-    constexpr bool LNF = EXT == 1 || EXT == 2, LNK = EXT == 1, LNP = EXT == 2, STATS = EXT == 3;
-    static_assert(EXT == 0 || (!CONV && !STAG && KB == 64), "extended instances: linear tiles on the rotated schedule");
+    constexpr bool LNF = EXT == 1 || EXT == 2, LNK = EXT == 1, LNP = EXT == 2, STATS = EXT == 3, SHUF = EXT == 4;
+    static_assert(EXT == 0 || (SHUF && CONV) || (!SHUF && !CONV && !STAG && KB == 64), "extended instances: linear tiles on the rotated schedule; the shuffled store: convolutions");
     static_assert(!STATS || F == 32, "row-statistics producer: 32- / 64-column epilogue passes");
     static_assert(!LNK || BM % (8 * WGM * WGN) == 0, "in-loop row statistics: 8 rows per wave instruction");
     constexpr int BK = KB;
@@ -191,7 +196,7 @@
     constexpr int FM_LAST = FMT - (WGM - 1) * FM;
     constexpr bool UNEVEN = FM_LAST != FM;
     constexpr int WM = FM * F, WN = BN / WGN, FN = WN / F;
-    static_assert(FM_LAST >= 1 && (!UNEVEN || (F == 16 && !STAG && KB == 64 && (EXT == 0 || EXT == 2))), "uneven tiles: 16x16x32 fragments, rotated schedule, plain / folded-LayerNorm (partials) instances");
+    static_assert(FM_LAST >= 1 && (!UNEVEN || (F == 16 && !STAG && KB == 64 && (EXT == 0 || EXT == 2 || EXT == 4))), "uneven tiles: 16x16x32 fragments, rotated schedule, plain / folded-LayerNorm (partials) instances");
     constexpr int KS = 512 / F;
     constexpr int NKS = BK / KS;
     constexpr int CPK = KS / 8;
@@ -681,7 +686,9 @@
         auto epilogue_rep = [&](auto rep_tag) {
         constexpr int REP = decltype(rep_tag)::value;
         const int64_t sh = REP ? (int64_t)p.dup_rows : 0;
-        const BufRsrc rs_o = make_buf_rsrc((const char*)p.out + sh * p.ldo * 2, (uint32_t)((((int64_t)mlim - 1) * p.ldo + ncols_out) * 2));
+        const BufRsrc rs_o = make_buf_rsrc((const char*)p.out + sh * p.ldo * 2,
+                                           SHUF ? (uint32_t)((((int64_t)4 * p.M - 1) * p.ldo + p.tap_group_n) * 2)
+                                                : (uint32_t)((((int64_t)mlim - 1) * p.ldo + ncols_out) * 2));
         const BufRsrc rs_r = make_buf_rsrc(has_res ? (const void*)(p.residual + sh * p.ldr) : (const void*)p.out,
                                            has_res ? (uint32_t)((((int64_t)p.M - 1) * p.ldr + p.N) * 2) : 0u);
         const float* rowvec0 = pcdm_gemm_detail::rowvec_base(p);
@@ -821,6 +828,12 @@
             }
             PCDM_WAVE_SYNC();
             const int mrow0 = m0 + wm * WM + jb * 32;
+            int srow_lane = 0, scol = 0;
+            if constexpr (SHUF) {
+                const int sph = pcdm_gemm_detail::shuffle2_phase(p, ncol0), mr = mrow0 + (lane & 31);
+                srow_lane = mr < mlim ? pcdm_gemm_detail::shuffle2_row(p, mr, sph) : -1;
+                scol = sph * p.tap_group_n;
+            }
             if (v_tile) {
                 if (mrow0 < p.M) {
                     const float* bc = bias_w + (ncol0 - wcol0);
@@ -831,7 +844,7 @@
                 }
             } else {
                 const int rc0 = ncol0 - wcol0;
-#define PCDM_LEAN(W, RVK) lean_pass<W, EPW, RVK, STATS && (W == 32 || W == 64)>(p, ep, lane, mrow0, ncol0, b0, b1, rs_o, rs_v, rv[RES ? q : 0], rvec_w, WNP, rc0, rv_split_row)
+#define PCDM_LEAN(W, RVK) lean_pass<W, EPW, RVK, STATS && (W == 32 || W == 64), SHUF>(p, ep, lane, mrow0, ncol0, b0, b1, rs_o, rs_v, rv[RES ? q : 0], rvec_w, WNP, rc0, rv_split_row, srow_lane, scol)
 #define PCDM_LEAN_W(RVK)                 \
     do {                                 \
         if (wc == 64) PCDM_LEAN(64, RVK);      \
@@ -878,6 +891,8 @@
         const int bidx = m / p.rows_per_batch;
         const int tok = m - bidx * p.rows_per_batch;
         const int64_t rrow = p.residual ? (int64_t)(m % p.res_mod) * p.ldr : 0;
+        const int sph = SHUF ? pcdm_gemm_detail::shuffle2_phase(p, n0) : 0;
+        const int srow = SHUF ? pcdm_gemm_detail::shuffle2_row(p, m, sph) : 0;
         if (p.epilogue == PCDM_EPI_GEGLU) {
             if constexpr (GLU_OK) {
 #pragma unroll
@@ -934,7 +949,9 @@
                     u16x4 o;
 #pragma unroll
                     for (int e = 0; e < 4; ++e) o[e] = f2bf(v[e]);
-                    *(u16x4*)((u16*)p.out + (int64_t)m * p.ldo + n) = o;
+                    int64_t oo = (int64_t)m * p.ldo + n;
+                    if constexpr (SHUF) oo = (int64_t)srow * p.ldo + n - sph * p.tap_group_n;
+                    *(u16x4*)((u16*)p.out + oo) = o;
                 }
             }
         }
@@ -974,7 +991,12 @@
     u16x4 o;
 #pragma unroll
     for (int e = 0; e < 4; ++e) o[e] = f2bf(v[e]);
-    *(u16x4*)((u16*)p.out + (int64_t)m * p.ldo + n) = o;
+    int64_t oo = (int64_t)m * p.ldo + n;
+    if (p.shuffle2) {
+        const int ph = pcdm_gemm_detail::shuffle2_phase(p, n);
+        oo = (int64_t)pcdm_gemm_detail::shuffle2_row(p, m, ph) * p.ldo + n - ph * p.tap_group_n;
+    }
+    *(u16x4*)((u16*)p.out + oo) = o;
 }
 
 template <int BM, int BN, int WGM, int WGN, int STAGES, bool CONV, bool STAG = false, int F = 32, int KB = 64, int EXT = 0>
diff --git a/pcdms_amd/csrc/misc.hip b/pcdms_amd/csrc/misc.hip
--- a/pcdms_amd/csrc/misc.hip
+++ b/pcdms_amd/csrc/misc.hip
@@ -353,6 +353,36 @@
 __global__ void advance_step_kernel(int32_t* step) {
     if (threadIdx.x == 0 && blockIdx.x == 0) *step += 1;
 }
+
+__global__ __launch_bounds__(256) void step_tail_kernel(const float* __restrict__ eps, int cfg, float g, float* __restrict__ lat,
+                                                        const float* __restrict__ coef, int32_t* step_dev, int32_t* ticket,
+                                                        u16* __restrict__ x_in, int N, int rep, int HW, int cpad) {
+    const int st = *step_dev;
+    const int64_t t = (int64_t)blockIdx.x * blockDim.x + threadIdx.x;
+    if (t < (int64_t)N * HW) {
+        const float* cf = coef + 4 * st;
+        const int b = (int)(t / HW), pix = (int)(t - (int64_t)b * HW);
+        const int64_t n = (int64_t)N * 4 * HW;
+        u16x4 o;
+#pragma unroll
+        for (int c = 0; c < 4; ++c) {
+            const int64_t i = ((int64_t)b * 4 + c) * HW + pix;
+            float e = eps[i];
+            if (cfg) e = e + g * (eps[n + i] - e);
+            const float v = cf[0] * lat[i] + cf[1] * e;
+            lat[i] = v;
+            o[c] = f2bf(v);
+        }
+        for (int r = 0; r < rep; ++r) *(u16x4*)(x_in + (((int64_t)r * N + b) * HW + pix) * cpad) = o;
+    }
+    __syncthreads();
+    if (threadIdx.x == 0) {
+        if (atomicAdd(ticket, (int32_t)1) == (int32_t)gridDim.x - 1) {
+            *step_dev = st + 1;
+            *ticket = 0;
+        }
+    }
+}
 }
 
 extern "C" int pcdm_version(void) { return PCDM_ABI_VERSION; }
@@ -439,6 +469,16 @@
     return 0;
 }
 
+extern "C" int pcdm_step_tail(const float* eps, int cfg, float g, float* lat, const float* coef, int32_t* step_dev, int32_t* ticket, void* x_in,
+                              int N, int rep, int HW, int cpad, pcdm_stream_t s) {
+    if (!eps || !lat || !coef || !step_dev || !ticket || !x_in || N <= 0 || rep <= 0 || HW <= 0 || cpad % 8 || cpad < 8) return -1;
+    if ((const void*)ticket == (const void*)step_dev || (cfg && rep != 2)) return -1;
+    PCDM_LAUNCH(step_tail_kernel, grid1d((int64_t)N * HW, 256), dim3(256), 0, (hipStream_t)s, eps, cfg, g, lat, coef, step_dev, ticket, (u16*)x_in,
+                N, rep, HW, cpad);
+    PCDM_CHECK_LAUNCH();
+    return 0;
+}
+
 extern "C" int pcdm_unipc_step(const float* eps, int cfg, float g, float* x, float* m1, float* m2, float* last, const float* coef,
                                const int32_t* step_dev, int64_t n, pcdm_stream_t s) {
     if (!eps || !x || !m1 || !m2 || !last || !coef || n <= 0) return -1;
diff --git a/pcdms_amd/csrc/unet_ctx.hip b/pcdms_amd/csrc/unet_ctx.hip
--- a/pcdms_amd/csrc/unet_ctx.hip
+++ b/pcdms_amd/csrc/unet_ctx.hip
@@ -223,7 +223,8 @@
         p.rowvec_step_stride = g.rowvec_step_stride;
         p.rowvec_step_count = g.rowvec_step_count;
         p.step_error = g.step_error;
-        const TileKey key{0, M, w->Npad, w->K, g.conv, g.conv ? g.stride + (g.tap_group_n ? 20 : 0) : 0, g.upsample, g.epilogue, g.a2 ? 1 : 0, g.residual ? 1 : 0, g.zero_rows ? 1 : (g.dup_rows ? 2 : 0)};
+        const int key_epi = g.epilogue == PCDM_EPI_SHUFFLE2 ? (int)PCDM_EPI_STORE : g.epilogue;
+        const TileKey key{0, M, w->Npad, w->K, g.conv, g.conv ? g.stride + (g.tap_group_n ? 20 : 0) : 0, g.upsample, key_epi, g.a2 ? 1 : 0, g.residual ? 1 : 0, g.zero_rows ? 1 : (g.dup_rows ? 2 : 0)};
         auto it = u->tiles.find(key);
         if (it != u->tiles.end() && !(it->second.first >= 31  && (g.rowvec || (g.residual && g.res_mod < M)))) {
             p.tile = it->second.first;
@@ -859,8 +860,13 @@
                 Run::G g4;
                 g4.conv = 1; g4.B = B; g4.Hi = hh; g4.Wi = ww; g4.Ho = hh; g4.Wo = ww;
                 g4.tap_lut = 0x8754764354214310ull; g4.tap_group_n = cx;
-                R.gemm(x, 0, B * hh * ww, R.pw(up4), R.buf("c1"), g4);
-                R.chk(pcdm_pixel_shuffle2(R.buf("c1"), R.buf("us"), B, hh, ww, cx, s), "pcdm_pixel_shuffle2");
+                if (!getenv_off("PCDM_SHUFFLE_STORE")) {
+                    g4.epilogue = PCDM_EPI_SHUFFLE2; g4.ldo = cx;
+                    R.gemm(x, 0, B * hh * ww, R.pw(up4), R.buf("us"), g4);
+                } else {
+                    R.gemm(x, 0, B * hh * ww, R.pw(up4), R.buf("c1"), g4);
+                    R.chk(pcdm_pixel_shuffle2(R.buf("c1"), R.buf("us"), B, hh, ww, cx, s), "pcdm_pixel_shuffle2");
+                }
                 x = R.buf("us");
                 hh = ho; ww = wo;
                 continue;
diff --git a/pcdms_amd/ops.py b/pcdms_amd/ops.py
--- a/pcdms_amd/ops.py
+++ b/pcdms_amd/ops.py
@@ -13,7 +13,7 @@
 from . import _lib
 from ._lib import GemmParams
 
-EPI_STORE, EPI_GEGLU, EPI_SPLIT_VT, EPI_NCHW_F32 = 0, 1, 2, 3
+EPI_STORE, EPI_GEGLU, EPI_SPLIT_VT, EPI_NCHW_F32, EPI_SHUFFLE2 = 0, 1, 2, 3, 4
 ACT_NONE, ACT_SILU, ACT_GELU = 0, 1, 2
 BF16 = torch.bfloat16
 LAUNCH_LOG: Optional[list] = None
@@ -361,6 +361,8 @@
     p.vt_col0 = vt_col0
     p.out = _ptr(out)
     p.ldo = out.stride(0) if (out.dim() == 2 and epilogue != EPI_NCHW_F32) else pw.N
+    if epilogue == EPI_SHUFFLE2 and tap_group_n:
+        assert pw.N == 4 * tap_group_n and out.dim() == 2 and out.shape == (4 * M, tap_group_n), (out.shape, M, tap_group_n)
     if out2 is not None:
         p.out2 = _ptr(out2)
         p.ldo2 = out2.shape[-1]
@@ -368,7 +370,8 @@
     split = 1
     key = None
     if tile == 0 and AUTOTUNE:
-        key = (M, pw.Npad, pw.K, p.conv, p.stride + (10 if p.no_pad_lo else 0) + (20 if tap_group_n else 0), p.upsample, epilogue,
+        key = (M, pw.Npad, pw.K, p.conv, p.stride + (10 if p.no_pad_lo else 0) + (20 if tap_group_n else 0), p.upsample,
+               EPI_STORE if epilogue == EPI_SHUFFLE2 else epilogue,
                a2 is not None, residual is not None) + ((True,) if zero_rows else ((2,) if dup_rows else ()))
         tile, split = _TUNED.get(key, (0, 1))
         if tile in ROWGEMM_TILES and (rowvec is not None or act != ACT_NONE or (residual is not None and res_mod < M)):
@@ -797,6 +800,16 @@
     return out
 
 
+def step_tail(eps: torch.Tensor, cfg: bool, g: float, lat: torch.Tensor, coef: torch.Tensor, step_dev: torch.Tensor, ticket: torch.Tensor,
+              x_in: torch.Tensor, rep: int) -> None:
+    N, _, h, w = lat.shape
+    _c(eps, torch.float32); _c(lat, torch.float32); _c(coef, torch.float32); _c(x_in, BF16)
+    assert eps.numel() == (2 if cfg else 1) * lat.numel() and lat.shape[1] == 4 and x_in.shape[0] == rep * N and x_in.numel() == rep * N * h * w * x_in.shape[-1]
+    assert step_dev.dtype == torch.int32 and ticket.dtype == torch.int32 and ticket.numel() == 1
+    _chk(_lib.lib().pcdm_step_tail(_ptr(eps), int(cfg), g, _ptr(lat), _ptr(coef), _ptr(step_dev), _ptr(ticket), _ptr(x_in), N, rep, h * w,
+                                   x_in.shape[-1], _stream(lat)), "pcdm_step_tail")
+
+
 def advance_step(step_dev: torch.Tensor) -> None:
     _chk(_lib.lib().pcdm_advance_step(_ptr(step_dev), _stream(step_dev)), "pcdm_advance_step")
 
diff --git a/pcdms_amd/pipeline.py b/pcdms_amd/pipeline.py
--- a/pcdms_amd/pipeline.py
+++ b/pcdms_amd/pipeline.py
@@ -1,6 +1,7 @@
 from __future__ import annotations
 
 import inspect
+import os
 from dataclasses import dataclass
 from typing import Any, Callable, List, Optional, Union
 
@@ -9,6 +10,9 @@
 from . import ops
 from .schedulers import DDIMScheduler, DDPMScheduler, DPMSolverMultistepScheduler, UniPCMultistepScheduler, _step_noise
 from .unet import Stage2_InapintUNet2DConditionModel
+
+
+STEP_TAIL = os.environ.get("PCDM_STEP_TAIL", "1") != "0"
 
 
 @dataclass
@@ -231,7 +235,8 @@
     def _step_eager(self, st):
         unet = self.unet
         B, h, w = st["B"], st["h"], st["w"]
-        x_in = ops.assemble_input(st["lat"], st["rep"], st["mask"], st["masked"], st["x_in"])
+        tail = st.get("tail", False)
+        x_in = st["x_in"] if tail else ops.assemble_input(st["lat"], st["rep"], st["mask"], st["masked"], st["x_in"])
         if st.get("ctx") is not None:
             eps = st["ctx"].forward(x_in, st["timesteps"], st["step"], B, h, w, st["pose_b"], out=st["eps_c"])
         else:
@@ -246,9 +251,17 @@
             ops.unipc_step(e, cfg, g, st["lat"], st["m1"], st["m2"], st["last"], st["coef"], st["step"])
         elif st["dpm"]:
             ops.dpmpp_step(e, cfg, g, st["lat"], st["m1"], st["noise"], st["coef"], st["step"])
+        elif tail:
+            ops.step_tail(e, cfg, g, st["lat"], st["coef"], st["step"], st["ticket"], st["x_in"], st["rep"])
+            return
         else:
             ops.cfg_step(e, cfg, g, st["lat"], st["lat"], st["coef"], st["step"])
         ops.advance_step(st["step"])
+
+    @staticmethod
+    def _prime_input(st):
+        if st.get("tail"):
+            ops.assemble_input(st["lat"], st["rep"], st["mask"], st["masked"], st["x_in"])
 
     @staticmethod
     def _zero_history(st):
@@ -281,6 +294,7 @@
                       eps_g=torch.empty_like(lat),
                       x_in=torch.empty(B, h, w, 64, dtype=ops.BF16, device=dev),
                       step=torch.zeros(1, dtype=torch.int32, device=dev),
+                      ticket=torch.zeros(1, dtype=torch.int32, device=dev),
                       timesteps=torch.empty(n, dtype=torch.int64, device=dev),
                       coef=torch.empty(n, 12 if unipc else 8 if dpm else 4, dtype=torch.float32, device=dev))
             if unipc:
@@ -303,6 +317,10 @@
         if st.get("gr", guidance_rescale) != guidance_rescale:
             self._graph = None
         st["gr"] = guidance_rescale
+        tail = STEP_TAIL and kind == "linear" and guidance_rescale == 0.0 and callback is None
+        if st.get("tail", tail) != tail:
+            self._graph = None
+        st["tail"] = tail
         w_gen = (id(unet), getattr(unet, "_pack_gen", 0), ops.workspace_generation(dev))
         if st.get("w_gen") != w_gen:
             self._graph = None
@@ -316,6 +334,7 @@
                 lat0 = lat.clone()
                 st["step"].zero_()
                 self._zero_history(st)
+                self._prime_input(st)
                 self._step_eager(st)
                 st["lat"].copy_(lat0)
                 st["step"].zero_()
@@ -334,6 +353,7 @@
             st["ctx"] = self._ctx
         st["step"].zero_()
         self._zero_history(st)
+        self._prime_input(st)
         self._st, self._graph_key = st, key
         if use_graph and dev.type == "cuda":
             if self._graph is None or self._st.get("g_captured") != g:
@@ -343,12 +363,14 @@
                 st["lat"].copy_(lat0)
                 st["step"].zero_()
                 self._zero_history(st)
+                self._prime_input(st)
                 graph = torch.cuda.CUDAGraph()
                 with torch.cuda.graph(graph, capture_error_mode="thread_local"):
                     self._step_eager(st)
                 st["lat"].copy_(lat0)
                 st["step"].zero_()
                 self._zero_history(st)
+                self._prime_input(st)
                 self._graph = graph
                 st["g_captured"] = g
                 w_gen = (id(unet), getattr(unet, "_pack_gen", 0), ops.workspace_generation(dev))
diff --git a/pcdms_amd/unet.py b/pcdms_amd/unet.py
--- a/pcdms_amd/unet.py
+++ b/pcdms_amd/unet.py
@@ -16,6 +16,7 @@
 FUSE_FF_OUT = os.environ.get("PCDM_FUSE_FF_OUT", "1") != "0"
 FUSE_SHORTCUT = os.environ.get("PCDM_FUSE_SHORTCUT", "1") != "0"
 PHASE_UPSAMPLE = os.environ.get("PCDM_PHASE_UPSAMPLE", "1") != "0"
+SHUFFLE_STORE = os.environ.get("PCDM_SHUFFLE_STORE", "1") != "0"
 
 _DEFAULT_CONFIG: Dict[str, Any] = dict(
     sample_size=None, in_channels=4, out_channels=4, center_input_sample=False, flip_sin_to_cos=True, freq_shift=0,
@@ -608,9 +609,15 @@
                 ho, wo = skips[-1][1], skips[-1][2]
                 w4 = W.get(f"up_blocks.{i}.upsamplers.0.conv4.")
                 if w4 is not None and (ho, wo) == (2 * hh, 2 * ww):
-                    ph = ops.gemm(x.view(B, hh, ww, rev[i]), w4, self._buf("usp", (B * hh * ww, 4 * rev[i])),
-                                  conv=dict(B=B, Hi=hh, Wi=ww, Ho=hh, Wo=ww), tap_lut=ops.UPSAMPLE_TAP_LUT, tap_group_n=rev[i])
-                    x = ops.pixel_shuffle2(ph, self._buf("us", (B * ho * wo, rev[i])), B, hh, ww, rev[i])
+                    if SHUFFLE_STORE:
+                        x = ops.gemm(x.view(B, hh, ww, rev[i]), w4, self._buf("us", (B * ho * wo, rev[i])), epilogue=ops.EPI_SHUFFLE2,
+                                     conv=dict(B=B, Hi=hh, Wi=ww, Ho=hh, Wo=ww), tap_lut=ops.UPSAMPLE_TAP_LUT, tap_group_n=rev[i])
+                        if taps is not None:
+                            ph = x.view(B, hh, 2, ww, 2, rev[i]).permute(0, 1, 3, 2, 4, 5).reshape(B * hh * ww, 4 * rev[i])
+                    else:
+                        ph = ops.gemm(x.view(B, hh, ww, rev[i]), w4, self._buf("usp", (B * hh * ww, 4 * rev[i])),
+                                      conv=dict(B=B, Hi=hh, Wi=ww, Ho=hh, Wo=ww), tap_lut=ops.UPSAMPLE_TAP_LUT, tap_group_n=rev[i])
+                        x = ops.pixel_shuffle2(ph, self._buf("us", (B * ho * wo, rev[i])), B, hh, ww, rev[i])
                     if taps is not None:
                         tap(f"up_blocks.{i}.upsamplers.0.ph", ph), tap(f"up_blocks.{i}.upsamplers.0.out", x)
                     hh, ww = ho, wo
```

Measured after the change: 6.410 images/s, median of 6. No clear change (+0.2%).
